# rostin79s/TFHE-AES

Measured on AMD Instinct MI355X. Metric: AES-128 CTR blocks/sec (FHE), higher is better.
Workload: dtype u64+f64; 1 GPU; configs[2]: 128 CTR blocks per GPU, Server::aes_encrypt 10 rounds (1280 bit-CBS/block), counters pre-incremented client-side; params=PARAM_OPT, blocks_per_gpu=128, total_blocks=128

## Files before the change

include/fheaes.h:

```cpp
#ifndef FHEAES_H
#define FHEAES_H

#include <stddef.h>
#include <stdint.h>

#ifdef __cplusplus
extern "C" {
#endif

#define FHEAES_OK 0
#define FHEAES_ERR_INVALID -1
#define FHEAES_ERR_NOKEYS -2
#define FHEAES_ERR_DEVICE -3
#define FHEAES_ERR_NOMEM -4

#define FHEAES_HOST 0
#define FHEAES_DEVICE 1

typedef struct fheaes_params {
    uint32_t lwe_dimension;
    uint32_t glwe_dimension;
    uint32_t polynomial_size;
    uint32_t pbs_base_log;
    uint32_t pbs_level;
// ... 77 lines not shown
int fheaes_aes_xts_decrypt_bits(fheaes_ctx *ctx, const uint64_t *dec_round_keys1, const uint64_t *round_keys2, uint32_t key_bits,
                                const uint64_t *tweaks_hi_lo, uint64_t n_units, uint64_t blocks_per_unit, uint64_t first_block,
                                const uint64_t *ct_hi_lo, uint64_t n_blocks, uint64_t *state_out, int memspace);
int fheaes_aes_xts_decrypt_packed(fheaes_ctx *ctx, const uint64_t *packed_dec_round_keys1, const uint64_t *packed_round_keys2, uint32_t key_bits,
                                  const uint64_t *tweaks_hi_lo, uint64_t n_units, uint64_t blocks_per_unit, uint64_t first_block,
                                  const uint64_t *ct_hi_lo, uint64_t n_blocks, uint64_t *state_out, int memspace);
int fheaes_xts_tweaks(fheaes_ctx *ctx, const uint64_t *anchor, uint64_t n_units, uint32_t first_offset, uint32_t n_offsets, uint64_t *out,
                      int memspace);
int fheaes_xts_tweak_row(uint32_t offset, uint32_t bit, uint32_t *sources_out , uint32_t *n_sources);
int fheaes_aes_xts_plan(uint64_t n_units, uint64_t blocks_per_unit, uint64_t first_block, uint64_t n_blocks, uint32_t key_bits,
                        uint64_t *segments, uint64_t *tweak_refresh_bytes, uint64_t *cipher_bytes, uint32_t *max_terms);

#define FHEAES_MAX_KEYS 65536
int fheaes_aes_key_expansion_batch(fheaes_ctx *ctx, const uint64_t *keys, uint32_t key_bits, uint64_t n_keys, uint64_t *round_keys, int memspace);
int fheaes_aes_decryption_round_keys_batch(fheaes_ctx *ctx, const uint64_t *round_keys, uint32_t key_bits, uint64_t n_keys,
                                           uint64_t *dec_round_keys, int memspace);
int fheaes_aes_encrypt_keyed(fheaes_ctx *ctx, const uint64_t *round_keys, uint32_t key_bits, uint64_t n_keys, const uint32_t *key_of_block,
                             uint64_t *state, uint64_t n_blocks, int memspace);
int fheaes_aes_decrypt_keyed(fheaes_ctx *ctx, const uint64_t *round_keys, uint32_t key_bits, uint64_t n_keys, const uint32_t *key_of_block,
                             uint64_t *state, uint64_t n_blocks, int memspace);
int fheaes_aes_decrypt_equivalent_keyed(fheaes_ctx *ctx, const uint64_t *dec_round_keys, uint32_t key_bits, uint64_t n_keys,
                                        const uint32_t *key_of_block, uint64_t *state, uint64_t n_blocks, int memspace);
int fheaes_aes_public_keyed(fheaes_ctx *ctx, const uint64_t *round_keys, uint32_t key_bits, uint64_t n_keys, const uint32_t *key_of_block,
                            const uint64_t *blocks_hi_lo, const uint64_t *data_hi_lo, uint64_t n_blocks, uint64_t *state_out, int memspace);
int fheaes_aes_public_plan_keyed(const uint64_t *blocks_hi_lo, const uint32_t *key_of_block, uint64_t n_blocks, uint64_t n_keys,
                                 uint32_t key_bits, uint64_t *unique_bytes_per_round);
int fheaes_aes_decrypt_public_keyed(fheaes_ctx *ctx, const uint64_t *dec_round_keys, uint32_t key_bits, uint64_t n_keys,
                                    const uint32_t *key_of_block, const uint64_t *blocks_hi_lo, const uint64_t *data_hi_lo, uint64_t n_blocks,
                                    uint64_t *state_out, int memspace);
int fheaes_aes_decrypt_public_plan_keyed(const uint64_t *blocks_hi_lo, const uint32_t *key_of_block, uint64_t n_blocks, uint64_t n_keys,
                                         uint32_t key_bits, uint64_t *unique_bytes_per_round);

size_t fheaes_packed_words(const fheaes_ctx *ctx, uint64_t m);
int fheaes_pack_bits(fheaes_ctx *ctx, const uint64_t *lwe_in, uint64_t m, uint64_t *glwe_out, int memspace);
int fheaes_unpack_bits(fheaes_ctx *ctx, const uint64_t *glwe_in, uint64_t m, uint64_t *lwe_out, int memspace);

int fheaes_expand_lwe_seeded(fheaes_ctx *ctx, const uint32_t *mask_key, uint64_t first_index, const uint64_t *bodies, uint64_t m,
                             uint64_t *lwe_out, int memspace);

size_t fheaes_packed_words_mod(const fheaes_ctx *ctx, uint64_t m, uint32_t width);
int fheaes_packed_mod_switch(fheaes_ctx *ctx, const uint64_t *glwe_in, uint64_t n_glwe, uint32_t width, uint64_t *out, int memspace);
int fheaes_pack_bits_mod(fheaes_ctx *ctx, const uint64_t *lwe_in, uint64_t m, uint32_t width, uint64_t *out, int memspace);
int fheaes_unpack_bits_mod(fheaes_ctx *ctx, const uint64_t *in, uint64_t m, uint32_t width, uint64_t *lwe_out, int memspace);

uint32_t fheaes_round_keys_packed_glwes(uint32_t key_bits);
int fheaes_pack_round_keys(fheaes_ctx *ctx, const uint64_t *round_keys, uint32_t key_bits, uint64_t n_keys, uint64_t *packed_out, int memspace);
int fheaes_unpack_round_keys(fheaes_ctx *ctx, const uint64_t *packed, uint32_t key_bits, uint64_t first_key, uint64_t n_keys,
                             uint64_t *round_keys_out, int memspace);
int fheaes_aes_encrypt_keyed_packed(fheaes_ctx *ctx, const uint64_t *packed_round_keys, uint32_t key_bits, uint64_t n_keys,
                                    const uint32_t *key_of_block, uint64_t *state, uint64_t n_blocks, int memspace);
int fheaes_aes_decrypt_keyed_packed(fheaes_ctx *ctx, const uint64_t *packed_round_keys, uint32_t key_bits, uint64_t n_keys,
                                    const uint32_t *key_of_block, uint64_t *state, uint64_t n_blocks, int memspace);
int fheaes_aes_decrypt_equivalent_keyed_packed(fheaes_ctx *ctx, const uint64_t *packed_dec_round_keys, uint32_t key_bits, uint64_t n_keys,
                                               const uint32_t *key_of_block, uint64_t *state, uint64_t n_blocks, int memspace);
int fheaes_aes_public_keyed_packed(fheaes_ctx *ctx, const uint64_t *packed_round_keys, uint32_t key_bits, uint64_t n_keys,
                                   const uint32_t *key_of_block, const uint64_t *blocks_hi_lo, const uint64_t *data_hi_lo, uint64_t n_blocks,
                                   uint64_t *state_out, int memspace);
int fheaes_aes_decrypt_public_keyed_packed(fheaes_ctx *ctx, const uint64_t *packed_dec_round_keys, uint32_t key_bits, uint64_t n_keys,
                                           const uint32_t *key_of_block, const uint64_t *blocks_hi_lo, const uint64_t *data_hi_lo,
                                           uint64_t n_blocks, uint64_t *state_out, int memspace);

#define FHEAES_MAC_MAX_STREAMS (1u << 20)
#define FHEAES_MAC_MAX_STREAM_BLOCKS (1u << 16)
#define FHEAES_MAC_NONE 0xFFFFFFFFu
int fheaes_aes_cbc_mac_keyed(fheaes_ctx *ctx, const uint64_t *round_keys, uint32_t key_bits, uint64_t n_keys, uint64_t n_streams,
                             const uint32_t *key_of_stream, const uint32_t *stream_blocks, const uint8_t *clear, const uint64_t *enc,
                             const uint8_t *enc_bytes, const uint64_t *init, uint64_t *mac_out, int memspace);
int fheaes_aes_cbc_mac_keyed_packed(fheaes_ctx *ctx, const uint64_t *packed_round_keys, uint32_t key_bits, uint64_t n_keys, uint64_t n_streams,
                                    const uint32_t *key_of_stream, const uint32_t *stream_blocks, const uint8_t *clear, const uint64_t *enc,
                                    const uint8_t *enc_bytes, const uint64_t *init, uint64_t *mac_out, int memspace);
int fheaes_aes_ccm_open_keyed(fheaes_ctx *ctx, const uint64_t *round_keys, uint32_t key_bits, uint64_t n_keys, uint64_t n_streams,
                              const uint32_t *key_of_stream, const uint32_t *head_blocks, const uint64_t *head_hi_lo, const uint64_t *ctr0_hi_lo,
                              const uint64_t *payload_bytes, const uint8_t *ciphertext, const uint8_t *tags, const uint32_t *tag_bytes,
                              uint64_t *plaintext_out, uint64_t *valid_out, int memspace);
int fheaes_aes_ccm_open_keyed_packed(fheaes_ctx *ctx, const uint64_t *packed_round_keys, uint32_t key_bits, uint64_t n_keys, uint64_t n_streams,
                                     const uint32_t *key_of_stream, const uint32_t *head_blocks, const uint64_t *head_hi_lo,
                                     const uint64_t *ctr0_hi_lo, const uint64_t *payload_bytes, const uint8_t *ciphertext, const uint8_t *tags,
                                     const uint32_t *tag_bytes, uint64_t *plaintext_out, uint64_t *valid_out, int memspace);
int fheaes_mac_link(fheaes_ctx *ctx, uint64_t *state, uint64_t n_slots, int first, const uint64_t *init, const uint64_t *enc, uint64_t n_enc,
                    const uint32_t *src_block, const uint8_t *enc_bytes, const uint8_t *clear, int memspace);
int fheaes_xts_whiten(fheaes_ctx *ctx, uint64_t *dst, const uint64_t *src, const uint64_t *tweaks, uint64_t n_tweaks, const uint32_t *tweak_of_block,
                      const uint8_t *clear, uint64_t n_blocks, int memspace);
int fheaes_aes_mac_plan(const uint32_t *stream_blocks, const uint32_t *payload_blocks, uint64_t n_streams, uint64_t *steps, uint64_t *n_active_out,
                        uint64_t n_active_cap, uint64_t *public_blocks, uint64_t *chained_blocks);

int fheaes_cmac_subkey_row(uint32_t which, uint32_t bit, uint32_t *sources_out, uint32_t *n_sources);
int fheaes_cmac_double(fheaes_ctx *ctx, const uint64_t *l, uint64_t n_keys, uint64_t *out, int memspace);
int fheaes_aes_cmac_subkeys_keyed(fheaes_ctx *ctx, const uint64_t *round_keys, uint32_t key_bits, uint64_t n_keys, uint64_t *subkeys_out,
                                  int memspace);
int fheaes_aes_cmac_subkeys_keyed_packed(fheaes_ctx *ctx, const uint64_t *packed_round_keys, uint32_t key_bits, uint64_t n_keys,
                                         uint64_t *subkeys_out, int memspace);
int fheaes_aes_cmac_keyed(fheaes_ctx *ctx, const uint64_t *round_keys, uint32_t key_bits, uint64_t n_keys, const uint64_t *subkeys,
                          uint64_t n_streams, const uint32_t *key_of_stream, const uint64_t *message_bytes, const uint8_t *data,
                          const uint8_t *tags, const uint32_t *tag_bytes, uint64_t *mac_out, uint64_t *valid_out, int memspace);
int fheaes_aes_cmac_keyed_packed(fheaes_ctx *ctx, const uint64_t *packed_round_keys, uint32_t key_bits, uint64_t n_keys, const uint64_t *subkeys,
                                 uint64_t n_streams, const uint32_t *key_of_stream, const uint64_t *message_bytes, const uint8_t *data,
                                 const uint8_t *tags, const uint32_t *tag_bytes, uint64_t *mac_out, uint64_t *valid_out, int memspace);
int fheaes_aes_cmac_plan(const uint64_t *message_bytes, uint64_t n_streams, uint64_t *steps, uint64_t *chained_blocks, uint64_t *padded_streams);

#define FHEAES_KW_MIN_SEMIBLOCKS 2
#define FHEAES_KW_MAX_SEMIBLOCKS 8
#define FHEAES_KW_MAX_KEYS 4096
int fheaes_aes_kw_unwrap_keyed(fheaes_ctx *ctx, const uint64_t *dec_round_keys, uint32_t key_bits, uint64_t n_keks, uint64_t n_keys,
                               const uint32_t *kek_of_key, uint32_t semiblocks, const uint8_t *wrapped, uint64_t *keys_out, uint64_t *valid_out,
                               int memspace);
int fheaes_aes_kw_unwrap_keyed_packed(fheaes_ctx *ctx, const uint64_t *packed_dec_round_keys, uint32_t key_bits, uint64_t n_keks, uint64_t n_keys,
                                      const uint32_t *kek_of_key, uint32_t semiblocks, const uint8_t *wrapped, uint64_t *keys_out,
                                      uint64_t *valid_out, int memspace);
int fheaes_kw_link(fheaes_ctx *ctx, uint64_t *state, uint64_t *regs, uint64_t n_keys, uint32_t semiblocks, uint32_t step, const uint8_t *wrapped,
                   int memspace);
int fheaes_aes_kw_plan(uint32_t key_bits, uint32_t semiblocks, uint64_t n_keys, uint64_t *steps, uint64_t *cipher_blocks, uint64_t *byte_wopbs);

#define FHEAES_GATE_LWE 0
#define FHEAES_GATE_GLWE 1
int fheaes_gate_ggsw(fheaes_ctx *ctx, const double *ggsw_fourier, uint64_t n_gates, const uint64_t *bits_of_gate, const uint64_t *in, uint64_t m,
                     int form, uint64_t *out, int memspace);
int fheaes_gate_bits(fheaes_ctx *ctx, const uint64_t *gates_lwe, uint64_t n_gates, const uint64_t *bits_of_gate, const uint64_t *lwe_in, uint64_t m,
                     uint64_t *lwe_out, int memspace);
int fheaes_gate_packed(fheaes_ctx *ctx, const uint64_t *gates_lwe, uint64_t n_gates, const uint64_t *glwes_of_gate, const uint64_t *glwe_in,
                       uint64_t n_glwe, uint64_t *glwe_out, int memspace);
int fheaes_gate_plan(const uint64_t *bits_of_gate, uint64_t n_gates, uint32_t k, uint64_t *workgroups, uint32_t *instances_per_workgroup);

#define FHEAES_AUDIT_MAX_ROWS 256
#define FHEAES_AUDIT_RECORDS 16
int fheaes_audit_set(fheaes_ctx *ctx, uint32_t rows, uint64_t min_bits, uint64_t seed);
int fheaes_audit_rows(uint64_t seed, uint64_t launch, uint64_t m, uint32_t rows, uint64_t *rows_out);
int fheaes_audit_read(fheaes_ctx *ctx, uint64_t *launches, uint64_t *rows_checked, uint64_t *rows_wrong, uint64_t *records_out, uint64_t record_cap,
                      uint64_t *record_n);
int fheaes_audit_debug(fheaes_ctx *ctx, uint64_t row, uint32_t word, uint64_t xor_mask);

#define FHEAES_STAGE_KEYSWITCH 0
#define FHEAES_STAGE_BLIND_ROTATE 1
#define FHEAES_STAGE_PFPKS 2
#define FHEAES_STAGE_GGSW_FFT 3
#define FHEAES_STAGE_VERTICAL_PACKING 4
#define FHEAES_STAGE_LINEAR 5
#define FHEAES_STAGE_COUNT 6
int fheaes_profile_enable(fheaes_ctx *ctx, int on);
int fheaes_profile_reset(fheaes_ctx *ctx);
int fheaes_profile_read(fheaes_ctx *ctx, int stage, double *total_ms, uint64_t *launches, uint64_t *units);

int fheaes_get_twiddles(double *psi_out);
int fheaes_read_bsk_fourier(fheaes_ctx *ctx, uint32_t i, double *out);
int fheaes_k2_launch_plan(uint64_t m, uint32_t cu_count, uint32_t k, int *form, uint64_t *units_main, uint32_t *r_main,
                          uint64_t *units_tail, uint32_t *r_tail);
int fheaes_k2_launch_plan_forms(uint64_t m, uint32_t cu_count, uint32_t k, int allow_pair, int *form, uint64_t *units_main, uint32_t *r_main,
                                uint64_t *units_tail, uint32_t *r_tail);
int fheaes_k2_context_plan(fheaes_ctx *ctx, uint64_t m, int *form, uint64_t *units_main, uint32_t *r_main, uint64_t *units_tail,
                           uint32_t *r_tail, char *kernel, size_t kernel_cap);
int fheaes_k2_set_parking(fheaes_ctx *ctx, int claimed);
int fheaes_k2_set_forms(fheaes_ctx *ctx, int allow_pair, int allow_home);
int fheaes_aes_window_plan(uint64_t n_blocks, uint32_t steps, uint32_t cu_count, uint32_t k, uint64_t *window_blocks, uint64_t *launches,
                           uint64_t *generations, uint64_t *generations_by_round);
int fheaes_aes_context_window(fheaes_ctx *ctx, uint64_t n_blocks, uint32_t steps, uint64_t *window_blocks);
#define FHEAES_AES_WINDOW_OFF 0xFFFFFFFFu
int fheaes_aes_set_window(fheaes_ctx *ctx, uint32_t window_blocks);
#define FHEAES_K2_PARK_SLOTS 1024
int fheaes_k2_park_debug(fheaes_ctx *ctx, const uint32_t *initial_owner, int record);
int fheaes_k2_park_read(fheaes_ctx *ctx, uint64_t *fallbacks, uint64_t *violations, uint32_t *owner_out, uint32_t *record_out,
                        uint64_t record_cap, uint64_t *record_n);
#define FHEAES_WS_BUFFERS 17
#define FHEAES_WS_F64 0
#define FHEAES_WS_WORDS 1
#define FHEAES_WS_TABLES 2
#define FHEAES_WS_PATTERN_F64_HALF 0x7FF87FF8u
#define FHEAES_WS_PATTERN_WORDS 0xA5
#define FHEAES_WS_PATTERN_TABLES 1u
#define FHEAES_WS_POISON_FILL 0
#define FHEAES_WS_POISON_RELEASE 1
int fheaes_workspace_info(fheaes_ctx *ctx, uint32_t index, char *name_out, size_t name_cap, uint64_t *bytes_out, int *class_out,
                          uint64_t *first_word_out, uint64_t *last_word_out);
int fheaes_workspace_poison(fheaes_ctx *ctx, int mode, uint64_t *bytes_out);
int fheaes_alloc_debug(fheaes_ctx *ctx, uint64_t fail_nth, uint64_t *seen_out);
const char *fheaes_version(void);

#ifdef __cplusplus
}
#endif
#endif
```

tfhe_aes_amd/_native.py:

```python
from __future__ import annotations

import ctypes
import os
import re
from pathlib import Path

import numpy as np

from . import _build
from .params import CParams, WopbsParameters

HOST, DEVICE = 0, 1
MAC_NONE = 0xFFFFFFFF
KW_MIN_SEMIBLOCKS, KW_MAX_SEMIBLOCKS, KW_MAX_KEYS = 2, 8, 4096
AES_WINDOW_OFF = 0xFFFFFFFF
GATE_LWE, GATE_GLWE = 0, 1
K2_PARK_SLOTS = 1024
AUDIT_MAX_ROWS, AUDIT_RECORDS = 256, 16
WS_BUFFERS = 17
WS_CLASSES = ("f64", "words", "tables")
WS_POISON_FILL, WS_POISON_RELEASE = 0, 1
STAGES = ("keyswitch", "blind_rotate", "pfpks", "ggsw_fft", "vertical_packing", "linear")

_u64p = ctypes.POINTER(ctypes.c_uint64)
_dp = ctypes.POINTER(ctypes.c_double)
_u32p = ctypes.POINTER(ctypes.c_uint32)
_u8p = ctypes.POINTER(ctypes.c_uint8)
_ctx = ctypes.c_void_p
_c = ctypes

SIGNATURES = {
    "fheaes_create": (_c.c_int, [_c.POINTER(CParams), _c.c_int, _c.POINTER(_ctx)]),
    "fheaes_destroy": (None, [_ctx]),
    "fheaes_last_error": (_c.c_char_p, [_ctx]),
    "fheaes_key_words": (_c.c_size_t, [_ctx, _c.c_int]),
    "fheaes_upload_keys": (_c.c_int, [_ctx, _c.c_void_p, _c.c_void_p, _c.c_void_p, _c.c_int]),
    "fheaes_key_body_words": (_c.c_size_t, [_ctx, _c.c_int]),
    "fheaes_upload_keys_seeded": (_c.c_int, [_ctx, _c.POINTER(_c.c_uint32), _c.c_void_p, _c.c_void_p, _c.c_void_p, _c.c_int]),
    "fheaes_clone_keys": (_c.c_int, [_ctx, _ctx]),
    "fheaes_clone_info": (_c.c_int, [_ctx, _c.POINTER(_c.c_int), _u64p, _dp]),
    "fheaes_noise_level_seen": (_c.c_int, [_ctx, _c.POINTER(_c.c_uint32), _c.POINTER(_c.c_uint32)]),
    "fheaes_set_stream": (_c.c_int, [_ctx, _c.c_void_p]),
    "fheaes_synchronize": (_c.c_int, [_ctx]),
    "fheaes_reserve": (_c.c_int, [_ctx, _c.c_uint64]),
    "fheaes_keyswitch_batch": (_c.c_int, [_ctx, _c.c_void_p, _c.c_uint64, _c.c_void_p, _c.c_int]),
    "fheaes_cbs_pbs_batch": (_c.c_int, [_ctx, _c.c_void_p, _c.c_uint64, _c.c_uint32, _c.c_void_p, _c.c_int]),
    "fheaes_pfpks_batch": (_c.c_int, [_ctx, _c.c_void_p, _c.c_uint64, _c.c_void_p, _c.c_int]),
    "fheaes_forward_fourier_batch": (_c.c_int, [_ctx, _c.c_void_p, _c.c_uint64, _c.c_void_p, _c.c_int]),
    "fheaes_vertical_packing_batch": (_c.c_int, [_ctx, _c.c_void_p, _c.c_uint64, _c.c_uint32, _c.c_void_p, _c.c_uint32,
                                                 _c.c_int, _c.c_void_p, _c.c_int]),
    "fheaes_inv_mix_columns_batch": (_c.c_int, [_ctx, _c.c_void_p, _c.c_uint64, _c.c_void_p, _c.c_int]),
    "fheaes_wopbs_batch": (_c.c_int, [_ctx, _c.c_void_p, _c.c_uint64, _c.c_uint32, _c.c_void_p, _c.c_uint32, _c.c_int,
                                      _c.c_void_p, _c.c_int]),
    "fheaes_gen_lut": (_c.c_int, [_c.c_uint32, _u64p, _u64p]),
    "fheaes_sbox": (_c.c_int, [_ctx, _c.c_void_p, _c.c_uint64, _c.c_int, _c.c_int]),
    "fheaes_many_sbox": (_c.c_int, [_ctx, _c.c_void_p, _c.c_uint64, _c.c_int, _c.c_void_p, _c.c_int]),
    "fheaes_aes_key_expansion": (_c.c_int, [_ctx, _c.c_void_p, _c.c_void_p, _c.c_int]),
    "fheaes_aes_encrypt": (_c.c_int, [_ctx, _c.c_void_p, _c.c_void_p, _c.c_uint64, _c.c_int]),
    "fheaes_aes_decrypt": (_c.c_int, [_ctx, _c.c_void_p, _c.c_void_p, _c.c_uint64, _c.c_int]),
    "fheaes_aes_decryption_round_keys": (_c.c_int, [_ctx, _c.c_void_p, _c.c_void_p, _c.c_int]),
    "fheaes_aes_decrypt_equivalent": (_c.c_int, [_ctx, _c.c_void_p, _c.c_void_p, _c.c_uint64, _c.c_int]),
    "fheaes_aes_key_expansion_bits": (_c.c_int, [_ctx, _c.c_void_p, _c.c_uint32, _c.c_void_p, _c.c_int]),
    "fheaes_aes_encrypt_bits": (_c.c_int, [_ctx, _c.c_void_p, _c.c_uint32, _c.c_void_p, _c.c_uint64, _c.c_int]),
    "fheaes_aes_decrypt_bits": (_c.c_int, [_ctx, _c.c_void_p, _c.c_uint32, _c.c_void_p, _c.c_uint64, _c.c_int]),
    "fheaes_aes_decryption_round_keys_bits": (_c.c_int, [_ctx, _c.c_void_p, _c.c_uint32, _c.c_void_p, _c.c_int]),
    "fheaes_aes_decrypt_equivalent_bits": (_c.c_int, [_ctx, _c.c_void_p, _c.c_uint32, _c.c_void_p, _c.c_uint64, _c.c_int]),
    "fheaes_add_scalar": (_c.c_int, [_ctx, _c.c_void_p, _c.c_uint64, _u64p, _c.c_int]),
    "fheaes_aes_encrypt_public_bits": (_c.c_int, [_ctx, _c.c_void_p, _c.c_uint32, _u64p, _c.c_uint64, _c.c_void_p, _c.c_int]),
    "fheaes_aes_ctr_bits": (_c.c_int, [_ctx, _c.c_void_p, _c.c_uint32, _u64p, _c.c_uint64, _u64p, _c.c_uint64, _c.c_void_p, _c.c_int]),
    "fheaes_aes_public_plan": (_c.c_int, [_u64p, _c.c_uint64, _c.c_uint32, _u64p]),
    "fheaes_aes_ctr32_bits": (_c.c_int, [_ctx, _c.c_void_p, _c.c_uint32, _u64p, _c.c_uint64, _u64p, _c.c_uint64, _c.c_void_p, _c.c_int]),
    "fheaes_aes_decrypt_public_bits": (_c.c_int, [_ctx, _c.c_void_p, _c.c_uint32, _u64p, _u64p, _c.c_uint64, _c.c_void_p, _c.c_int]),
    "fheaes_aes_cbc_decrypt_bits": (_c.c_int, [_ctx, _c.c_void_p, _c.c_uint32, _u64p, _u64p, _c.c_uint64, _c.c_void_p, _c.c_int]),
    "fheaes_aes_xts_decrypt_bits": (_c.c_int, [_ctx, _c.c_void_p, _c.c_void_p, _c.c_uint32, _u64p, _c.c_uint64, _c.c_uint64, _c.c_uint64, _u64p, _c.c_uint64,
                                               _c.c_void_p, _c.c_int]),
    "fheaes_aes_xts_decrypt_packed": (_c.c_int, [_ctx, _c.c_void_p, _c.c_void_p, _c.c_uint32, _u64p, _c.c_uint64, _c.c_uint64, _c.c_uint64, _u64p, _c.c_uint64,
                                                 _c.c_void_p, _c.c_int]),
    "fheaes_xts_tweaks": (_c.c_int, [_ctx, _c.c_void_p, _c.c_uint64, _c.c_uint32, _c.c_uint32, _c.c_void_p, _c.c_int]),
    "fheaes_xts_tweak_row": (_c.c_int, [_c.c_uint32, _c.c_uint32, _u32p, _u32p]),
    "fheaes_aes_xts_plan": (_c.c_int, [_c.c_uint64, _c.c_uint64, _c.c_uint64, _c.c_uint64, _c.c_uint32, _u64p, _u64p, _u64p, _u32p]),
    "fheaes_aes_key_expansion_batch": (_c.c_int, [_ctx, _c.c_void_p, _c.c_uint32, _c.c_uint64, _c.c_void_p, _c.c_int]),
    "fheaes_aes_decryption_round_keys_batch": (_c.c_int, [_ctx, _c.c_void_p, _c.c_uint32, _c.c_uint64, _c.c_void_p, _c.c_int]),
    "fheaes_aes_encrypt_keyed": (_c.c_int, [_ctx, _c.c_void_p, _c.c_uint32, _c.c_uint64, _u32p, _c.c_void_p, _c.c_uint64, _c.c_int]),
    "fheaes_aes_decrypt_keyed": (_c.c_int, [_ctx, _c.c_void_p, _c.c_uint32, _c.c_uint64, _u32p, _c.c_void_p, _c.c_uint64, _c.c_int]),
    "fheaes_aes_decrypt_equivalent_keyed": (_c.c_int, [_ctx, _c.c_void_p, _c.c_uint32, _c.c_uint64, _u32p, _c.c_void_p, _c.c_uint64, _c.c_int]),
    "fheaes_aes_public_keyed": (_c.c_int, [_ctx, _c.c_void_p, _c.c_uint32, _c.c_uint64, _u32p, _u64p, _u64p, _c.c_uint64, _c.c_void_p, _c.c_int]),
    "fheaes_aes_public_plan_keyed": (_c.c_int, [_u64p, _u32p, _c.c_uint64, _c.c_uint64, _c.c_uint32, _u64p]),
    "fheaes_aes_decrypt_public_keyed": (_c.c_int, [_ctx, _c.c_void_p, _c.c_uint32, _c.c_uint64, _u32p, _u64p, _u64p, _c.c_uint64, _c.c_void_p, _c.c_int]),
    "fheaes_aes_decrypt_public_plan_keyed": (_c.c_int, [_u64p, _u32p, _c.c_uint64, _c.c_uint64, _c.c_uint32, _u64p]),
    "fheaes_packed_words": (_c.c_size_t, [_ctx, _c.c_uint64]),
    "fheaes_pack_bits": (_c.c_int, [_ctx, _c.c_void_p, _c.c_uint64, _c.c_void_p, _c.c_int]),
    "fheaes_unpack_bits": (_c.c_int, [_ctx, _c.c_void_p, _c.c_uint64, _c.c_void_p, _c.c_int]),
    "fheaes_expand_lwe_seeded": (_c.c_int, [_ctx, _u32p, _c.c_uint64, _c.c_void_p, _c.c_uint64, _c.c_void_p, _c.c_int]),
    "fheaes_packed_words_mod": (_c.c_size_t, [_ctx, _c.c_uint64, _c.c_uint32]),
    "fheaes_packed_mod_switch": (_c.c_int, [_ctx, _c.c_void_p, _c.c_uint64, _c.c_uint32, _c.c_void_p, _c.c_int]),
    "fheaes_pack_bits_mod": (_c.c_int, [_ctx, _c.c_void_p, _c.c_uint64, _c.c_uint32, _c.c_void_p, _c.c_int]),
    "fheaes_unpack_bits_mod": (_c.c_int, [_ctx, _c.c_void_p, _c.c_uint64, _c.c_uint32, _c.c_void_p, _c.c_int]),
    "fheaes_round_keys_packed_glwes": (_c.c_uint32, [_c.c_uint32]),
    "fheaes_pack_round_keys": (_c.c_int, [_ctx, _c.c_void_p, _c.c_uint32, _c.c_uint64, _c.c_void_p, _c.c_int]),
    "fheaes_unpack_round_keys": (_c.c_int, [_ctx, _c.c_void_p, _c.c_uint32, _c.c_uint64, _c.c_uint64, _c.c_void_p, _c.c_int]),
    "fheaes_aes_encrypt_keyed_packed": (_c.c_int, [_ctx, _c.c_void_p, _c.c_uint32, _c.c_uint64, _u32p, _c.c_void_p, _c.c_uint64, _c.c_int]),
    "fheaes_aes_decrypt_keyed_packed": (_c.c_int, [_ctx, _c.c_void_p, _c.c_uint32, _c.c_uint64, _u32p, _c.c_void_p, _c.c_uint64, _c.c_int]),
    "fheaes_aes_decrypt_equivalent_keyed_packed": (_c.c_int, [_ctx, _c.c_void_p, _c.c_uint32, _c.c_uint64, _u32p, _c.c_void_p, _c.c_uint64, _c.c_int]),
    "fheaes_aes_public_keyed_packed": (_c.c_int, [_ctx, _c.c_void_p, _c.c_uint32, _c.c_uint64, _u32p, _u64p, _u64p, _c.c_uint64, _c.c_void_p, _c.c_int]),
    "fheaes_aes_decrypt_public_keyed_packed": (_c.c_int, [_ctx, _c.c_void_p, _c.c_uint32, _c.c_uint64, _u32p, _u64p, _u64p, _c.c_uint64, _c.c_void_p,
                                                          _c.c_int]),
    "fheaes_aes_cbc_mac_keyed": (_c.c_int, [_ctx, _c.c_void_p, _c.c_uint32, _c.c_uint64, _c.c_uint64, _u32p, _u32p, _u8p, _c.c_void_p, _u8p, _c.c_void_p,
                                            _c.c_void_p, _c.c_int]),
    "fheaes_aes_cbc_mac_keyed_packed": (_c.c_int, [_ctx, _c.c_void_p, _c.c_uint32, _c.c_uint64, _c.c_uint64, _u32p, _u32p, _u8p, _c.c_void_p, _u8p,
                                                   _c.c_void_p, _c.c_void_p, _c.c_int]),
    "fheaes_aes_ccm_open_keyed": (_c.c_int, [_ctx, _c.c_void_p, _c.c_uint32, _c.c_uint64, _c.c_uint64, _u32p, _u32p, _u64p, _u64p, _u64p, _u8p, _u8p, _u32p,
                                             _c.c_void_p, _c.c_void_p, _c.c_int]),
    "fheaes_aes_ccm_open_keyed_packed": (_c.c_int, [_ctx, _c.c_void_p, _c.c_uint32, _c.c_uint64, _c.c_uint64, _u32p, _u32p, _u64p, _u64p, _u64p, _u8p, _u8p,
                                                    _u32p, _c.c_void_p, _c.c_void_p, _c.c_int]),
    "fheaes_mac_link": (_c.c_int, [_ctx, _c.c_void_p, _c.c_uint64, _c.c_int, _c.c_void_p, _c.c_void_p, _c.c_uint64, _u32p, _u8p, _u8p, _c.c_int]),
    "fheaes_xts_whiten": (_c.c_int, [_ctx, _c.c_void_p, _c.c_void_p, _c.c_void_p, _c.c_uint64, _u32p, _u8p, _c.c_uint64, _c.c_int]),
    "fheaes_aes_mac_plan": (_c.c_int, [_u32p, _u32p, _c.c_uint64, _u64p, _u64p, _c.c_uint64, _u64p, _u64p]),
    "fheaes_cmac_subkey_row": (_c.c_int, [_c.c_uint32, _c.c_uint32, _u32p, _u32p]),
    "fheaes_cmac_double": (_c.c_int, [_ctx, _c.c_void_p, _c.c_uint64, _c.c_void_p, _c.c_int]),
    "fheaes_aes_cmac_subkeys_keyed": (_c.c_int, [_ctx, _c.c_void_p, _c.c_uint32, _c.c_uint64, _c.c_void_p, _c.c_int]),
    "fheaes_aes_cmac_subkeys_keyed_packed": (_c.c_int, [_ctx, _c.c_void_p, _c.c_uint32, _c.c_uint64, _c.c_void_p, _c.c_int]),
    "fheaes_aes_cmac_keyed": (_c.c_int, [_ctx, _c.c_void_p, _c.c_uint32, _c.c_uint64, _c.c_void_p, _c.c_uint64, _u32p, _u64p, _u8p, _u8p, _u32p, _c.c_void_p,
                                         _c.c_void_p, _c.c_int]),
    "fheaes_aes_cmac_keyed_packed": (_c.c_int, [_ctx, _c.c_void_p, _c.c_uint32, _c.c_uint64, _c.c_void_p, _c.c_uint64, _u32p, _u64p, _u8p, _u8p, _u32p,
                                                _c.c_void_p, _c.c_void_p, _c.c_int]),
    "fheaes_aes_cmac_plan": (_c.c_int, [_u64p, _c.c_uint64, _u64p, _u64p, _u64p]),
    "fheaes_aes_kw_unwrap_keyed": (_c.c_int, [_ctx, _c.c_void_p, _c.c_uint32, _c.c_uint64, _c.c_uint64, _u32p, _c.c_uint32, _u8p, _c.c_void_p, _c.c_void_p,
                                              _c.c_int]),
    "fheaes_aes_kw_unwrap_keyed_packed": (_c.c_int, [_ctx, _c.c_void_p, _c.c_uint32, _c.c_uint64, _c.c_uint64, _u32p, _c.c_uint32, _u8p, _c.c_void_p,
                                                     _c.c_void_p, _c.c_int]),
    "fheaes_kw_link": (_c.c_int, [_ctx, _c.c_void_p, _c.c_void_p, _c.c_uint64, _c.c_uint32, _c.c_uint32, _u8p, _c.c_int]),
    "fheaes_aes_kw_plan": (_c.c_int, [_c.c_uint32, _c.c_uint32, _c.c_uint64, _u64p, _u64p, _u64p]),
    "fheaes_gate_ggsw": (_c.c_int, [_ctx, _c.c_void_p, _c.c_uint64, _u64p, _c.c_void_p, _c.c_uint64, _c.c_int, _c.c_void_p, _c.c_int]),
    "fheaes_gate_bits": (_c.c_int, [_ctx, _c.c_void_p, _c.c_uint64, _u64p, _c.c_void_p, _c.c_uint64, _c.c_void_p, _c.c_int]),
    "fheaes_gate_packed": (_c.c_int, [_ctx, _c.c_void_p, _c.c_uint64, _u64p, _c.c_void_p, _c.c_uint64, _c.c_void_p, _c.c_int]),
    "fheaes_gate_plan": (_c.c_int, [_u64p, _c.c_uint64, _c.c_uint32, _u64p, _u32p]),
    "fheaes_profile_enable": (_c.c_int, [_ctx, _c.c_int]),
    "fheaes_profile_reset": (_c.c_int, [_ctx]),
    "fheaes_profile_read": (_c.c_int, [_ctx, _c.c_int, _dp, _u64p, _u64p]),
    "fheaes_get_twiddles": (_c.c_int, [_dp]),
    "fheaes_read_bsk_fourier": (_c.c_int, [_ctx, _c.c_uint32, _dp]),
    "fheaes_k2_launch_plan": (_c.c_int, [_c.c_uint64, _c.c_uint32, _c.c_uint32, _c.POINTER(_c.c_int), _c.POINTER(_c.c_uint64), _c.POINTER(_c.c_uint32),
                                       _c.POINTER(_c.c_uint64), _c.POINTER(_c.c_uint32)]),
    "fheaes_k2_launch_plan_forms": (_c.c_int, [_c.c_uint64, _c.c_uint32, _c.c_uint32, _c.c_int, _c.POINTER(_c.c_int), _c.POINTER(_c.c_uint64),
                                             _c.POINTER(_c.c_uint32), _c.POINTER(_c.c_uint64), _c.POINTER(_c.c_uint32)]),
    "fheaes_k2_context_plan": (_c.c_int, [_ctx, _c.c_uint64, _c.POINTER(_c.c_int), _c.POINTER(_c.c_uint64), _c.POINTER(_c.c_uint32),
                                        _c.POINTER(_c.c_uint64), _c.POINTER(_c.c_uint32), _c.c_char_p, _c.c_size_t]),
    "fheaes_k2_set_parking": (_c.c_int, [_ctx, _c.c_int]),
    "fheaes_k2_set_forms": (_c.c_int, [_ctx, _c.c_int, _c.c_int]),
    "fheaes_aes_window_plan": (_c.c_int, [_c.c_uint64, _c.c_uint32, _c.c_uint32, _c.c_uint32, _u64p, _u64p, _u64p, _u64p]),
    "fheaes_aes_context_window": (_c.c_int, [_ctx, _c.c_uint64, _c.c_uint32, _u64p]),
    "fheaes_aes_set_window": (_c.c_int, [_ctx, _c.c_uint32]),
    "fheaes_k2_park_debug": (_c.c_int, [_ctx, _c.POINTER(_c.c_uint32), _c.c_int]),
    "fheaes_k2_park_read": (_c.c_int, [_ctx, _u64p, _u64p, _c.POINTER(_c.c_uint32), _c.POINTER(_c.c_uint32), _c.c_uint64, _u64p]),
    "fheaes_audit_set": (_c.c_int, [_ctx, _c.c_uint32, _c.c_uint64, _c.c_uint64]),
    "fheaes_audit_rows": (_c.c_int, [_c.c_uint64, _c.c_uint64, _c.c_uint64, _c.c_uint32, _u64p]),
    "fheaes_audit_read": (_c.c_int, [_ctx, _u64p, _u64p, _u64p, _u64p, _c.c_uint64, _u64p]),
    "fheaes_audit_debug": (_c.c_int, [_ctx, _c.c_uint64, _c.c_uint32, _c.c_uint64]),
    "fheaes_workspace_info": (_c.c_int, [_ctx, _c.c_uint32, _c.c_char_p, _c.c_size_t, _u64p, _c.POINTER(_c.c_int), _u64p, _u64p]),
    "fheaes_workspace_poison": (_c.c_int, [_ctx, _c.c_int, _u64p]),
    "fheaes_alloc_debug": (_c.c_int, [_ctx, _c.c_uint64, _u64p]),
    "fheaes_version": (_c.c_char_p, []),
}

_libs = {}


def header_symbols() -> list[str]:
    text = (_build.ROOT / "include" / "fheaes.h").read_text()
    text = re.sub(r"/\*.*?\*/", "", text, flags=re.S)
    return sorted(set(re.findall(r"\b(fheaes_[a-z0-9_]+)\s*\(", text)))


def load_library(build: bool = True, path=None, partial: bool = False):
    if path is None:
        path = _build.build_engine() if build else _build.ENGINE_SO
    path = Path(path).resolve()
    if path in _libs:
        return _libs[path]
    try:
        import torch
    except ImportError:
        pass
    if not path.exists():
        raise RuntimeError("%s is missing: run __graft_entry__.build() (hipcc --offload-arch=gfx950)" % path.name)
    lib = ctypes.CDLL(str(path))
    for name, (res, args) in SIGNATURES.items():
        if partial and not hasattr(lib, name):
            continue
        fn = getattr(lib, name)
        fn.restype, fn.argtypes = res, args
    _libs[path] = lib
    return lib


class FheAesError(RuntimeError):
    def __init__(self, code: int, message: str):
        super().__init__("fheaes error %d: %s" % (code, message))
        self.code = code


def _ptr(x):
    if x is None:
        return None, None
    if isinstance(x, np.ndarray):
        assert x.flags["C_CONTIGUOUS"], "array must be C-contiguous"
        return x.ctypes.data, HOST
    if hasattr(x, "data_ptr"):
        assert x.is_contiguous()
        return x.data_ptr(), (DEVICE if x.is_cuda else HOST)
    raise TypeError("expected numpy array or torch tensor, got %r" % type(x))


class Engine:

    def __init__(self, params: WopbsParameters, device: int = 0, allow_dev_build: bool = False, library=None):
        self.params = params
        self._lib = load_library() if library is None else load_library(path=library, partial=True)
        self._h = _ctx()
        version = (self._lib.fheaes_version() or b"").decode()
        if version.endswith(" dev") and not (allow_dev_build or os.environ.get("FHEAES_ALLOW_DEV_BUILD") == "1"):
            raise RuntimeError("libfheaes.so is a developer build (%r): rebuild it with tfhe_aes_amd._build.build_engine(force=True), or pass "
                               "allow_dev_build=True / FHEAES_ALLOW_DEV_BUILD=1 if that is what you mean to run" % version)
        cp = params.c_struct()
        rc = self._lib.fheaes_create(ctypes.byref(cp), device, ctypes.byref(self._h))
        if rc != 0:
            raise FheAesError(rc, (self._lib.fheaes_last_error(None) or b"").decode())

    def close(self):
        if getattr(self, "_h", None):
            self._lib.fheaes_destroy(self._h)
            self._h = None

    def __del__(self):
        try:
            self.close()
        except Exception:
            pass

    def _check(self, rc: int):
        if rc != 0:
            raise FheAesError(rc, (self._lib.fheaes_last_error(self._h) or b"").decode())

    def _space(self, *arrays):
        spaces = {s for _, s in map(_ptr, arrays) if s is not None}
        if len(spaces) != 1:
            raise ValueError("all arrays of one call must live in the same memory space")
        return spaces.pop()

    def key_words(self, which: int) -> int:
        return self._lib.fheaes_key_words(self._h, which)

    def upload_keys(self, ksk, bsk, pfpksk):
        sp = self._space(ksk, bsk, pfpksk)
        for which, a in enumerate((ksk, bsk, pfpksk)):
            n = a.size if isinstance(a, np.ndarray) else a.numel()
            if n != self.key_words(which):
                raise ValueError("key %d has %d words, expected %d" % (which, n, self.key_words(which)))
        self._check(self._lib.fheaes_upload_keys(self._h, _ptr(ksk)[0], _ptr(bsk)[0], _ptr(pfpksk)[0], sp))

    def upload_keys_seeded(self, mask_key, ksk_body, bsk_body, pfpksk_body):
        mk = np.ascontiguousarray(np.asarray(mask_key, dtype=np.uint32).reshape(8))
        sp = self._space(ksk_body, bsk_body, pfpksk_body)
        for which, a in enumerate((ksk_body, bsk_body, pfpksk_body)):
            n = a.size if isinstance(a, np.ndarray) else a.numel()
            if n != self._lib.fheaes_key_body_words(self._h, which):
                raise ValueError("key body %d has %d words, expected %d" % (which, n, self._lib.fheaes_key_body_words(self._h, which)))
        self._check(self._lib.fheaes_upload_keys_seeded(self._h, mk.ctypes.data_as(_c.POINTER(_c.c_uint32)), _ptr(ksk_body)[0], _ptr(bsk_body)[0],
                                                        _ptr(pfpksk_body)[0], sp))

    def clone_keys_from(self, other: "Engine"):
        self._check(self._lib.fheaes_clone_keys(self._h, other._h))

    def clone_info(self) -> dict:
        path, nbytes, secs = ctypes.c_int(), ctypes.c_uint64(), ctypes.c_double()
        self._check(self._lib.fheaes_clone_info(self._h, ctypes.byref(path), ctypes.byref(nbytes), ctypes.byref(secs)))
        return {"path": ("none", "same_device", "peer", "staged")[path.value], "bytes": nbytes.value, "seconds": secs.value}

    def noise_level_seen(self) -> tuple[int, int]:
        seen, limit = ctypes.c_uint32(), ctypes.c_uint32()
        self._check(self._lib.fheaes_noise_level_seen(self._h, ctypes.byref(seen), ctypes.byref(limit)))
        return seen.value, limit.value

    def set_stream(self, stream_handle: int | None):
        self._check(self._lib.fheaes_set_stream(self._h, stream_handle))

    def synchronize(self):
        self._check(self._lib.fheaes_synchronize(self._h))

    def reserve(self, max_bits: int):
        self._check(self._lib.fheaes_reserve(self._h, max_bits))

    def keyswitch_batch(self, lwe_in, lwe_out, m: int):
        self._check(self._lib.fheaes_keyswitch_batch(self._h, _ptr(lwe_in)[0], m, _ptr(lwe_out)[0], self._space(lwe_in, lwe_out)))

    def cbs_pbs_batch(self, lwe_small, lwe_out, m: int, level: int = 1):
        self._check(self._lib.fheaes_cbs_pbs_batch(self._h, _ptr(lwe_small)[0], m, level, _ptr(lwe_out)[0], self._space(lwe_small, lwe_out)))

    def pfpks_batch(self, lwe_in, ggsw_out, m: int):
        self._check(self._lib.fheaes_pfpks_batch(self._h, _ptr(lwe_in)[0], m, _ptr(ggsw_out)[0], self._space(lwe_in, ggsw_out)))

    def forward_fourier_batch(self, polys_in, fourier_out, polys: int):
        self._check(self._lib.fheaes_forward_fourier_batch(self._h, _ptr(polys_in)[0], polys, _ptr(fourier_out)[0], self._space(polys_in, fourier_out)))
# ... 382 lines not shown
    out = np.zeros((len(values), 2), dtype=np.uint64)
    for i, v in enumerate(values):
        if isinstance(v, (bytes, bytearray)):
            if len(v) != 16:
                raise ValueError("an AES block has 16 bytes, got %d" % len(v))
            v = int.from_bytes(v, "big")
        v = int(v)
        if not 0 <= v < 1 << 128:
            raise ValueError("a block is a 128-bit value")
        out[i, 0], out[i, 1] = v >> 64, v & (2 ** 64 - 1)
    return out


def key_indices(key_of_block, n_blocks: int) -> np.ndarray:
    idx = [int(k) for k in key_of_block]
    if len(idx) != n_blocks:
        raise ValueError("one key index per block expected: %d for %d blocks" % (len(idx), n_blocks))
    if any(not 0 <= k < 1 << 32 for k in idx):
        raise ValueError("a key index is a uint32")
    out = np.zeros(max(n_blocks, 1), dtype=np.uint32)
    out[:n_blocks] = idx
    return out


def wrapped_bytes(wrapped, semiblocks: int) -> np.ndarray:
    size = 8 * (semiblocks + 1)
    if not isinstance(wrapped, np.ndarray):
        wrapped = [bytes(w) for w in wrapped]
        if any(len(w) != size for w in wrapped):
            raise ValueError("a wrapped key of %d semiblocks has %d bytes" % (semiblocks, size))
        wrapped = np.frombuffer(b"".join(wrapped), dtype=np.uint8)
    return np.ascontiguousarray(np.asarray(wrapped, dtype=np.uint8).reshape(-1, size))


def aes_public_plan_keyed(blocks, key_of_block, n_keys: int, key_bits: int = 128) -> list[int]:
    cnt = u128_pairs(blocks)
    kob = key_indices(key_of_block, len(cnt))
    out = np.zeros(14, dtype=np.uint64)
    rc = load_library().fheaes_aes_public_plan_keyed(cnt.ctypes.data_as(_u64p), kob.ctypes.data_as(_u32p), len(cnt), n_keys, key_bits, out.ctypes.data_as(_u64p))
    if rc != 0:
        raise FheAesError(rc, "fheaes_aes_public_plan_keyed: key_bits must be 128, 192 or 256, n_keys in 1..65536 and every key index below n_keys")
    return [int(x) for x in out[:{128: 10, 192: 12, 256: 14}[key_bits]]]


def aes_decrypt_public_plan_keyed(blocks, key_of_block, n_keys: int, key_bits: int = 128) -> list[int]:
    cnt = u128_pairs(blocks)
    kob = key_indices(key_of_block, len(cnt)) if key_of_block is not None else None
    out = np.zeros(14, dtype=np.uint64)
    rc = load_library().fheaes_aes_decrypt_public_plan_keyed(cnt.ctypes.data_as(_u64p), kob.ctypes.data_as(_u32p) if kob is not None else None, len(cnt),
                                                             n_keys, key_bits, out.ctypes.data_as(_u64p))
    if rc != 0:
        raise FheAesError(rc, "fheaes_aes_decrypt_public_plan_keyed: key_bits must be 128, 192 or 256, n_keys in 1..65536 and every key index below n_keys")
    return [int(x) for x in out[:{128: 10, 192: 12, 256: 14}[key_bits]]]


def aes_decrypt_public_plan(blocks, key_bits: int = 128) -> list[int]:
    return aes_decrypt_public_plan_keyed(blocks, None, 1, key_bits)


def xts_tweak_row(offset: int, bit: int) -> list[int]:
    src, n = (_c.c_uint32 * 4)(), _c.c_uint32()
    rc = load_library().fheaes_xts_tweak_row(offset, bit, src, _c.byref(n))
    if rc != 0:
        raise FheAesError(rc, "fheaes_xts_tweak_row: offset must be at most 121 and bit below 128")
    return [int(x) for x in src[:n.value]]


def aes_xts_plan(n_units: int, blocks_per_unit: int, first_block: int, n_blocks: int, key_bits: int = 128) -> dict:
    seg, ref, cip, terms = _c.c_uint64(), _c.c_uint64(), _c.c_uint64(), _c.c_uint32()
    rc = load_library().fheaes_aes_xts_plan(n_units, blocks_per_unit, first_block, n_blocks, key_bits, _c.byref(seg), _c.byref(ref), _c.byref(cip), _c.byref(terms))
    if rc != 0:
        raise FheAesError(rc, "fheaes_aes_xts_plan: key_bits must be 128 or 256, blocks_per_unit in 1..2^20, and n_units cover the blocks")
    return {"segments": seg.value, "tweak_refresh_bytes": ref.value, "cipher_bytes": cip.value, "max_terms": terms.value}


def aes_mac_plan(stream_blocks, payload_blocks=None) -> dict:
    sb = np.ascontiguousarray(np.asarray(stream_blocks, dtype=np.uint32).reshape(-1))
    pb = None if payload_blocks is None else np.ascontiguousarray(np.asarray(payload_blocks, dtype=np.uint32).reshape(-1))
    if pb is not None and len(pb) != len(sb):
        raise ValueError("one payload block count per stream expected")
    cap = int(sb.max()) if len(sb) else 0
    act = np.zeros(max(cap, 1), dtype=np.uint64)
    steps, pub, chained = _c.c_uint64(), _c.c_uint64(), _c.c_uint64()
    rc = load_library().fheaes_aes_mac_plan(sb.ctypes.data_as(_u32p), pb.ctypes.data_as(_u32p) if pb is not None else None, len(sb), _c.byref(steps),
                                            act.ctypes.data_as(_u64p), len(act), _c.byref(pub), _c.byref(chained))
    if rc != 0:
        raise FheAesError(rc, "fheaes_aes_mac_plan: at most 2^20 streams of at most 2^16 blocks, payload blocks within them")
    return {"steps": steps.value, "n_active": [int(x) for x in act[:steps.value]], "chained_blocks": chained.value, "public_blocks": pub.value}


def cmac_subkey_row(which: int, bit: int) -> list[int]:
    src, n = (_c.c_uint32 * 3)(), _c.c_uint32()
    rc = load_library().fheaes_cmac_subkey_row(which, bit, src, _c.byref(n))
    if rc != 0:
        raise FheAesError(rc, "fheaes_cmac_subkey_row: which must be 0 or 1 and bit below 128")
    return [int(x) for x in src[:n.value]]


def aes_cmac_plan(message_bytes) -> dict:
    mb = np.ascontiguousarray(np.asarray(message_bytes, dtype=np.uint64).reshape(-1))
    steps, chained, padded = _c.c_uint64(), _c.c_uint64(), _c.c_uint64()
    rc = load_library().fheaes_aes_cmac_plan(mb.ctypes.data_as(_u64p), len(mb), _c.byref(steps), _c.byref(chained), _c.byref(padded))
    if rc != 0:
        raise FheAesError(rc, "fheaes_aes_cmac_plan: at most 2^20 streams of at most 16 * 2^16 bytes")
    return {"steps": steps.value, "chained_blocks": chained.value, "padded_streams": padded.value}


def aes_kw_plan(key_bits: int, semiblocks: int, n_keys: int) -> dict:
    steps, blocks, wopbs = _c.c_uint64(), _c.c_uint64(), _c.c_uint64()
    rc = load_library().fheaes_aes_kw_plan(key_bits, semiblocks, n_keys, _c.byref(steps), _c.byref(blocks), _c.byref(wopbs))
    if rc != 0:
        raise FheAesError(rc, "fheaes_aes_kw_plan: key_bits 128 / 192 / 256, %d..%d semiblocks, at most %d keys" % (KW_MIN_SEMIBLOCKS, KW_MAX_SEMIBLOCKS, KW_MAX_KEYS))
    return {"steps": steps.value, "cipher_blocks": blocks.value, "byte_wopbs": wopbs.value}


def gate_plan(runs, k: int) -> dict:
    r = np.ascontiguousarray(np.asarray(runs, dtype=np.uint64).reshape(-1))
    wgs, per = _c.c_uint64(), _c.c_uint32()
    rc = load_library().fheaes_gate_plan(r.ctypes.data_as(_u64p), r.size, k, _c.byref(wgs), _c.byref(per))
    if rc != 0:
        raise FheAesError(rc, "fheaes_gate_plan: k must be 4 or 1")
    return {"workgroups": wgs.value, "instances_per_workgroup": per.value}


def audit_rows(seed: int, launch: int, m: int, rows: int) -> list[int]:
    out = np.zeros(max(min(int(rows), int(m)), 1), dtype=np.uint64)
    rc = load_library().fheaes_audit_rows(int(seed) & (2 ** 64 - 1), int(launch), int(m), int(rows), out.ctypes.data_as(_u64p))
    if rc != 0:
        raise FheAesError(rc, "fheaes_audit_rows: m at least 1 and rows in 1..%d" % AUDIT_MAX_ROWS)
    return [int(x) for x in out]


def round_keys_packed_glwes(key_bits: int) -> int:
    return int(load_library().fheaes_round_keys_packed_glwes(int(key_bits)))


def aes_public_plan(blocks, key_bits: int = 128) -> list[int]:
    cnt = u128_pairs(blocks)
    out = np.zeros(14, dtype=np.uint64)
    rc = load_library().fheaes_aes_public_plan(cnt.ctypes.data_as(_u64p), len(cnt), key_bits, out.ctypes.data_as(_u64p))
    if rc != 0:
        raise FheAesError(rc, "fheaes_aes_public_plan: key_bits must be 128, 192 or 256")
    return [int(x) for x in out[:{128: 10, 192: 12, 256: 14}[key_bits]]]


def aes_window_plan(n_blocks: int, steps: int, cu_count: int = 256, k: int = 4) -> dict:
    w, la, g, gr = _c.c_uint64(), _c.c_uint64(), _c.c_uint64(), _c.c_uint64()
    rc = load_library().fheaes_aes_window_plan(n_blocks, steps, cu_count, k, _c.byref(w), _c.byref(la), _c.byref(g), _c.byref(gr))
    if rc != 0:
        raise FheAesError(rc, "fheaes_aes_window_plan: n_blocks, steps and cu_count must be at least 1")
    return {"window": w.value, "launches": la.value, "generations": g.value, "generations_by_round": gr.value}


def get_twiddles() -> np.ndarray:
    out = np.empty((512, 2), dtype=np.float64)
    rc = load_library().fheaes_get_twiddles(out.ctypes.data_as(_dp))
    if rc != 0:
        raise FheAesError(rc, "fheaes_get_twiddles")
    return out


def gen_lut(nb_block: int, f_table) -> np.ndarray:
    f = np.ascontiguousarray(f_table, dtype=np.uint64)
    if f.size != 1 << nb_block:
        raise ValueError("f_table must have 2^nb_block entries")
    out = np.empty((nb_block, max(512, 1 << nb_block)), dtype=np.uint64)
    rc = load_library().fheaes_gen_lut(nb_block, f.ctypes.data_as(_u64p), out.ctypes.data_as(_u64p))
    if rc != 0:
        raise FheAesError(rc, "fheaes_gen_lut")
    return out
```

tfhe_aes_amd/csrc/aes_schedule.h:

```cpp
#pragma once

static int many_sbox_dev(fheaes_ctx *c, const uint64_t *bytes, uint64_t n_bytes, int set, uint64_t *out)
{
    return wopbs_dev(c, bytes, n_bytes, 8, c->lutset_d[set], (uint32_t)c->lutset_n[set], 0, out);
}

static int aes_rounds(uint32_t key_bits) { return key_bits == 128 ? 10 : key_bits == 192 ? 12 : key_bits == 256 ? 14 : 0; }

static int check_key_bits(fheaes_ctx *c, uint32_t key_bits)
{
    if (!aes_rounds(key_bits)) return c->fail(FHEAES_ERR_INVALID, "key_bits must be 128, 192 or 256, got %u", key_bits);
    return FHEAES_OK;
}

struct AesStep { int set; uint32_t n_luts; GatherTable table; int key_round; };
struct AesSchedule {
    int first_key_round = 0;
    uint32_t max_luts = 0;
    std::vector<AesStep> steps;
    void add(int set, uint32_t n_luts, const GatherTable &t, int key_round) { steps.push_back({set, n_luts, t, key_round}); max_luts = std::max(max_luts, n_luts); }
};

static AesSchedule aes_encrypt_schedule(int nr)
{
    AesSchedule s;
    s.first_key_round = 0;
    for (int round = 1; round < nr; ++round) s.add(LUTSET_ENC_ROUND, 3, table_enc_round(), round);
    s.add(LUTSET_SBOX, 1, table_shift_rows(false), nr);
    return s;
}

static AesSchedule aes_decrypt_schedule(int nr)
{
    AesSchedule s;
    s.first_key_round = nr;
    for (int round = nr; round >= 2; --round) {
        s.add(LUTSET_INV_SBOX, 1, table_shift_rows(true), round - 1);
        s.add(LUTSET_DEC_MUL, 4, table_dec_mix(), -1);
    }
    s.add(LUTSET_INV_SBOX, 1, table_shift_rows(true), 0);
    return s;
}

static AesSchedule aes_decrypt_eq_schedule(int nr)
{
    AesSchedule s;
    s.first_key_round = nr;
    for (int round = nr - 1; round >= 1; --round) s.add(LUTSET_DEC_EQ_ROUND, 4, table_dec_eq_round(), round);
    s.add(LUTSET_INV_SBOX, 1, table_shift_rows(true), 0);
    return s;
}

static int aes_run_dev(fheaes_ctx *c, const KeySets &rk, uint64_t *state, uint64_t n_blocks, const AesSchedule &sch)
{
    const uint64_t bw = 8ull * c->big1, sw = 16 * bw, steps = sch.steps.size();
    auto key_of = [&](const AesStep &st, uint64_t first_block) {
        if (st.key_round < 0) return KeySets{nullptr, nullptr, 0};
        return rk.round((uint64_t)st.key_round, sw, first_block);
    };
    const uint64_t w = aes_context_window(c, n_blocks, steps);
    TRY(ensure(c, c->ws_vp, (w ? w : n_blocks) * 16 * sch.max_luts * bw * 8));
    uint64_t *vp = (uint64_t *)c->ws_vp.p;
    TRY(launch_add_bcast(c, state, rk.round((uint64_t)sch.first_key_round, sw), sw, n_blocks));
    if (w == 0) {
        for (const AesStep &st : sch.steps) {
            TRY(many_sbox_dev(c, state, 16 * n_blocks, st.set, vp));
            TRY(launch_gather(c, vp, st.n_luts, key_of(st, 0), state, n_blocks, st.table));
        }
        return FHEAES_OK;
    }
    const uint64_t ggsw_words = (uint64_t)c->k1 * c->k1 * FHE_N, total = steps * n_blocks;
    TRY(ensure_wopbs_ws(c, w * AES_BLOCK_BITS));
    uint64_t *small = (uint64_t *)c->ws_small.p;
    const double2 *ggswf = (const double2 *)c->ws_ggswf.p;
    struct Segment { const AesStep *st; uint64_t first, blocks, row; uint64_t *vp; };
    for (uint64_t i0 = 0; i0 < total; i0 += w) {
        const uint64_t len = std::min<uint64_t>(w, total - i0), s = i0 / n_blocks, b0 = i0 % n_blocks, m = len * AES_BLOCK_BITS;
        Segment seg[2] = {{&sch.steps[s], b0, std::min<uint64_t>(len, n_blocks - b0), 0, vp}, {}};
        int n_seg = 1;
        if (seg[0].blocks < len) {
            seg[1] = {&sch.steps[s + 1], 0, len - seg[0].blocks, seg[0].blocks, vp + seg[0].blocks * 16 * seg[0].st->n_luts * bw};
            n_seg = 2;
        }
        for (int g = 0; g < n_seg; ++g)
            TRY(launch_keyswitch(c, state + seg[g].first * sw, seg[g].blocks * AES_BLOCK_BITS, small + seg[g].row * AES_BLOCK_BITS * (c->n + 1)));
        TRY(cbs_from_small(c, m));
        if (n_seg == 1 || seg[0].st->set == seg[1].st->set) {
            const int set = seg[0].st->set;
            TRY(launch_vertical_packing(c, ggswf, 16 * len, 8, c->lutset_d[set], (uint32_t)c->lutset_n[set], 0, vp));
        } else {
            for (int g = 0; g < n_seg; ++g) {
                const int set = seg[g].st->set;
                TRY(launch_vertical_packing(c, ggswf + seg[g].row * AES_BLOCK_BITS * (ggsw_words / 2), 16 * seg[g].blocks, 8, c->lutset_d[set],
                                            (uint32_t)c->lutset_n[set], 0, seg[g].vp));
            }
        }
        for (int g = 0; g < n_seg; ++g)
            TRY(launch_gather(c, seg[g].vp, seg[g].st->n_luts, key_of(*seg[g].st, seg[g].first), state + seg[g].first * sw, seg[g].blocks, seg[g].st->table));
    }
    return FHEAES_OK;
}

static int aes_encrypt_dev(fheaes_ctx *c, const KeySets &rk, uint64_t *state, uint64_t n_blocks, int nr) { return aes_run_dev(c, rk, state, n_blocks, aes_encrypt_schedule(nr)); }
static int aes_decrypt_dev(fheaes_ctx *c, const KeySets &rk, uint64_t *state, uint64_t n_blocks, int nr) { return aes_run_dev(c, rk, state, n_blocks, aes_decrypt_schedule(nr)); }
static int aes_decrypt_eq_dev(fheaes_ctx *c, const KeySets &dw, uint64_t *state, uint64_t n_blocks, int nr) { return aes_run_dev(c, dw, state, n_blocks, aes_decrypt_eq_schedule(nr)); }

typedef int (*AesDevFn)(fheaes_ctx *, const KeySets &, uint64_t *, uint64_t, int);

static int dec_round_keys_dev(fheaes_ctx *c, const uint64_t *w, uint64_t *dw, int nr, uint64_t n_keys)
{
    const uint64_t bw = 8ull * c->big1, sw = 16 * bw, ks = (uint64_t)(nr + 1) * sw, mid = (uint64_t)(nr - 1) * 16, nbytes = mid * n_keys;
    const bool strided = n_keys > 1;
    TRY(ensure(c, c->ws_vp, nbytes * 4 * bw * 8));
    TRY(ensure(c, c->ws_tmp_a, nbytes * bw * 8));
    if (strided) TRY(ensure(c, c->ws_tmp_b, nbytes * bw * 8));
    uint64_t *vp = (uint64_t *)c->ws_vp.p, *mix = (uint64_t *)c->ws_tmp_a.p, *flat = (uint64_t *)c->ws_tmp_b.p;
    TRY(launch_key_rows(c, dw, ks, w, ks, 0, nullptr, 0, 0, 16, n_keys, 1));
    TRY(launch_key_rows(c, dw + (uint64_t)nr * sw, ks, w + (uint64_t)nr * sw, ks, 0, nullptr, 0, 0, 16, n_keys, 1));
    if (strided) TRY(launch_key_rows(c, flat, mid * bw, w + sw, ks, 0, nullptr, 0, 0, (uint32_t)mid, n_keys, 1));
    TRY(many_sbox_dev(c, strided ? flat : w + sw, nbytes, LUTSET_DEC_MUL, vp));
    TRY(launch_gather(c, vp, 4, KeySets{nullptr, nullptr, 0}, mix, nbytes / 16, table_dec_mix()));
    TRY(many_sbox_dev(c, mix, nbytes, LUTSET_IDENTITY, strided ? flat : dw + sw));
    if (strided) TRY(launch_key_rows(c, dw + sw, ks, flat, mid * bw, 0, nullptr, 0, 0, (uint32_t)mid, n_keys, 1));
    return FHEAES_OK;
}

static int key_expansion_dev(fheaes_ctx *c, const uint64_t *key, uint64_t *w, int nr, uint64_t n_keys)
{
    static const uint8_t RCON[10] = {0x01, 0x02, 0x04, 0x08, 0x10, 0x20, 0x40, 0x80, 0x1B, 0x36};
    const uint64_t bw = 8ull * c->big1, ww = 4 * bw, ks = (uint64_t)(nr + 1) * 16 * bw;
    const int nk = nr - 6;
    const bool strided = n_keys > 1;
    TRY(ensure(c, c->ws_tmp_a, n_keys * ww * 8));
    TRY(ensure(c, c->ws_tmp_b, n_keys * ww * 8));
    if (strided) TRY(ensure(c, c->ws_tmp_c, n_keys * ww * 8));
    uint64_t *ta = (uint64_t *)c->ws_tmp_a.p, *tb = (uint64_t *)c->ws_tmp_b.p, *tc = (uint64_t *)c->ws_tmp_c.p;
    TRY(launch_key_rows(c, w, ks, key, (uint64_t)nk * ww, 0, nullptr, 0, 0, 4u * nk, n_keys, 1));
    for (int i = nk; i < 4 * (nr + 1); ++i) {
        const uint64_t *prev = w + (uint64_t)(i - 1) * ww, *back = w + (uint64_t)(i - nk) * ww;
        if (i % nk == 0) {
            TRY(launch_key_rows(c, ta, ww, prev, ks, 1, nullptr, 0, 0, 4, n_keys, 1));
            TRY(many_sbox_dev(c, ta, 4 * n_keys, LUTSET_SBOX, tb));
            TRY(launch_key_rows(c, ta, ww, tb, ww, 0, back, ks, RCON[i / nk - 1], 4, n_keys, 2));
        } else if (nk > 6 && i % nk == 4) {
            if (strided) TRY(launch_key_rows(c, ta, ww, prev, ks, 0, nullptr, 0, 0, 4, n_keys, 1));
            TRY(many_sbox_dev(c, strided ? ta : prev, 4 * n_keys, LUTSET_SBOX, tb));
            TRY(launch_key_rows(c, ta, ww, tb, ww, 0, back, ks, 0, 4, n_keys, 2));
        } else {
            TRY(launch_key_rows(c, ta, ww, prev, ks, 0, back, ks, 0, 4, n_keys, 2));
        }
        uint64_t *fresh = w + (uint64_t)i * ww;
        TRY(many_sbox_dev(c, ta, 4 * n_keys, LUTSET_IDENTITY, strided ? tc : fresh));
        if (strided) TRY(launch_key_rows(c, fresh, ks, tc, ww, 0, nullptr, 0, 0, 4, n_keys, 1));
    }
    return FHEAES_OK;
}

template <class Fill> static int upload_pinned(fheaes_ctx *c, size_t bytes, size_t ws_bytes, Fill fill)
{
    if (c->pin_ev) HIP_TRY(c, hipEventSynchronize(c->pin_ev));
    else HIP_TRY(c, hipEventCreateWithFlags(&c->pin_ev, hipEventDisableTiming));
    if (c->pin_bytes < bytes) {
        if (c->pin) { HIP_TRY(c, hipHostFree(c->pin)); c->pin = nullptr; c->pin_bytes = 0; }
        HIP_TRY(c, hipHostMalloc((void **)&c->pin, bytes, hipHostMallocDefault));
        c->pin_bytes = bytes;
    }
    fill(c->pin);
    TRY(ensure(c, c->ws_misc, ws_bytes));
    HIP_TRY(c, hipMemcpyAsync(c->ws_misc.p, c->pin, bytes, hipMemcpyHostToDevice, c->stream));
    HIP_TRY(c, hipEventRecord(c->pin_ev, c->stream));
    return FHEAES_OK;
}

static int add_scalar_dev(fheaes_ctx *c, uint64_t *state, uint64_t n_blocks, const uint64_t *counters)
{
    const uint32_t lw = c->big1;
    TRY(upload_pinned(c, 16 * n_blocks, 16 * n_blocks + n_blocks * lw * 8 + 64, [&](uint8_t *add) {
        for (uint64_t b = 0; b < n_blocks; ++b) {
            uint64_t hi = counters[2 * b], lo = counters[2 * b + 1];
            for (int j = 0; j < 8; ++j) { add[(15 - j) * n_blocks + b] = (uint8_t)(lo >> (8 * j)); add[(7 - j) * n_blocks + b] = (uint8_t)(hi >> (8 * j)); }
        }
    }));
    uint8_t *add_d = (uint8_t *)c->ws_misc.p;
    uint64_t *carry = (uint64_t *)((uint8_t *)c->ws_misc.p + ((16 * n_blocks + 63) / 64) * 64);
    TRY(ensure(c, c->ws_tmp_a, n_blocks * 9ull * lw * 8));
    TRY(ensure(c, c->ws_tmp_b, n_blocks * 2ull * 9 * lw * 8));
    TRY(ensure(c, c->ws_luts, n_blocks * 2ull * 9 * FHE_N * 8));
    uint64_t *in9 = (uint64_t *)c->ws_tmp_a.p, *res = (uint64_t *)c->ws_tmp_b.p, *luts = (uint64_t *)c->ws_luts.p;
    for (int byte = 15; byte >= 0; --byte) {
        const uint32_t bits = byte == 15 ? 8 : 9;
        dim3 g1((bits * lw + 255) / 256, (unsigned)n_blocks);
        hipLaunchKernelGGL(pack9_kernel, g1, dim3(256), 0, c->stream, (const uint64_t *)state, (const uint64_t *)carry, in9, (uint32_t)byte, lw, n_blocks, bits);
        hipLaunchKernelGGL(counter_lut_kernel, dim3((2 * bits * FHE_N + 255) / 256, (unsigned)n_blocks), dim3(256), 0, c->stream, luts,
                           (const uint8_t *)(add_d + (size_t)byte * n_blocks), bits, n_blocks);
        HIP_TRY(c, hipGetLastError());
        TRY(wopbs_dev(c, in9, n_blocks, bits, luts, 2, 1, res));
        hipLaunchKernelGGL(unpack_sum_carry_kernel, dim3((9 * lw + 255) / 256, (unsigned)n_blocks), dim3(256), 0, c->stream, (const uint64_t *)res, bits, state, carry,
                           (uint32_t)byte, lw, n_blocks);
        HIP_TRY(c, hipGetLastError());
    }
    return FHEAES_OK;
}

struct PublicPlan {
    struct Layer { size_t head, term; uint32_t n, terms; };
    std::vector<Layer> layers;
    std::vector<uint32_t> words;
    uint64_t max_vp_bytes_per_bw = 0;
};

static inline uint32_t u128_byte(const uint64_t *hi_lo, int p) { return (uint32_t)((p < 8 ? hi_lo[0] >> (8 * (7 - p)) : hi_lo[1] >> (8 * (15 - p))) & 0xFF); }

struct PublicKey5 {
    uint32_t v[5];
    bool operator==(const PublicKey5 &o) const { return !memcmp(v, o.v, sizeof v); }
};
struct PublicKey5Hash {
    size_t operator()(const PublicKey5 &k) const
    {
        uint64_t h = 0xCBF29CE484222325ull;
        for (uint32_t x : k.v) { h ^= x; h *= 0x100000001B3ull; }
        return (size_t)(h ^ (h >> 29));
    }
};

struct PublicDirection {
    GatherTable round, last;
    int round_set, last_set;
    uint32_t round_luts, last_luts;
    bool keys_descend;
    uint64_t key_round(int layer, int nr) const { return (uint64_t)(keys_descend ? nr - layer : layer); }
};

static PublicDirection public_forward() { return {table_enc_round(), table_shift_rows(false), LUTSET_ENC_ROUND, LUTSET_SBOX, 3, 1, false}; }
static PublicDirection public_inverse() { return {table_dec_eq_round(), table_shift_rows(true), LUTSET_DEC_EQ_ROUND, LUTSET_INV_SBOX, 4, 1, true}; }

static void public_plan(const PublicDirection &dir, const uint64_t *blocks, const uint64_t *data, const uint32_t *key_of_block, uint64_t n_blocks, int nr,
                        PublicPlan &pl)
{
    auto key_of = [&](uint64_t b) { return key_of_block ? key_of_block[b] : 0u; };
    const GatherTable &t_round = dir.round, &t_shift = dir.last;
    const uint64_t nbytes = 16 * n_blocks;
    std::vector<uint32_t> id(nbytes), next(nbytes);
    pl.layers.clear(); pl.words.clear();
    pl.layers.reserve((size_t)nr + 1);
    {
        std::unordered_map<uint32_t, uint32_t> seen;
// ... 362 lines not shown
```

tfhe_aes_amd/csrc/engine.hip:

```cpp
#include <hip/hip_runtime.h>
#include <algorithm>
#include <cmath>
#include <cstdarg>
#include <cstdio>
#include <atomic>
#include <chrono>
#include <cstring>
#include <functional>
#include <mutex>
#include <string>
#include <type_traits>
#include <unordered_map>
#include <vector>

#include "knobs.h"
#include "fheaes.h"
#include "fft_dev.h"
#include "kern_extprod.h"
#include "kern_gate.h"
#include "kern_blindrot_latency.h"
#include "kern_blindrot16.h"
#include "kern_blindrot_pair.h"
#include "kern_audit.h"
#include "ks_launch.h"
#include "kern_linear.h"

#define FHEAES_VERSION_STR "fheaes-mi355x 0.4 (gfx950)" FHEAES_BUILD_KIND

#include "host_tables.h"
#include "engine_ctx.h"
#include "engine_launch.h"
#include "aes_schedule.h"

namespace {

int supported(const fheaes_params *p, std::string &why)
{
    char buf[256];
    if (p->polynomial_size != FHE_N) { why = "polynomial_size must be 512"; return 0; }
    if (p->glwe_dimension != 4 && p->glwe_dimension != 1) { why = "glwe_dimension must be 4 (PARAM_OPT) or 1 (toy)"; return 0; }
    if (p->pbs_base_log != 8 || p->pbs_level != 5 || p->ks_base_log != 2 || p->ks_level != 6 || p->pfks_base_log != 12 ||
        p->pfks_level != 3 || p->cbs_base_log != 15 || p->cbs_level != 1) {
        snprintf(buf, sizeof buf, "unsupported gadget: kernels are instantiated for pbs(8,5) ks(2,6) pfks(12,3) cbs(15,1)");
        why = buf;
        return 0;
    }
    if (p->lwe_dimension < 1 || p->lwe_dimension > 4096) { why = "lwe_dimension out of range"; return 0; }
    return 1;
}

}

extern "C" {

int fheaes_k2_launch_plan(uint64_t m, uint32_t cu_count, uint32_t k, int *form, uint64_t *units_main, uint32_t *r_main,
                          uint64_t *units_tail, uint32_t *r_tail)
{
    if (!form || !units_main || !r_main || !units_tail || !r_tail || cu_count == 0 || m == 0) return FHEAES_ERR_INVALID;
    const K2Plan pl = k2_plan(m, cu_count, k + 1);
    *form = pl.form; *units_main = pl.units_main; *r_main = pl.r_main; *units_tail = pl.units_tail; *r_tail = pl.r_tail;
    return FHEAES_OK;
}
int fheaes_k2_launch_plan_forms(uint64_t m, uint32_t cu_count, uint32_t k, int allow_pair, int *form, uint64_t *units_main, uint32_t *r_main,
                                uint64_t *units_tail, uint32_t *r_tail)
{
    if (!form || !units_main || !r_main || !units_tail || !r_tail || cu_count == 0 || m == 0 || (allow_pair != 0 && allow_pair != 1)) return FHEAES_ERR_INVALID;
    const K2Plan pl = k2_plan(m, cu_count, k + 1, allow_pair == 1);
    *form = pl.form; *units_main = pl.units_main; *r_main = pl.r_main; *units_tail = pl.units_tail; *r_tail = pl.r_tail;
    return FHEAES_OK;
}
int fheaes_k2_context_plan(fheaes_ctx *ctx, uint64_t m, int *form, uint64_t *units_main, uint32_t *r_main, uint64_t *units_tail,
                           uint32_t *r_tail, char *kernel, size_t kernel_cap)
{
    if (!ctx) return FHEAES_ERR_INVALID;
    CtxLock lock__(ctx);
    if (!form || !units_main || !r_main || !units_tail || !r_tail || m == 0) return ctx->fail(FHEAES_ERR_INVALID, "k2_context_plan: null output or empty batch");
    const K2Launch L = k2_launch(ctx, m);
    const K2Plan &pl = L.pl;
    *form = pl.form; *units_main = pl.units_main; *r_main = pl.r_main; *units_tail = pl.units_tail; *r_tail = pl.r_tail;
    if (kernel && kernel_cap) { std::strncpy(kernel, L.name, kernel_cap - 1); kernel[kernel_cap - 1] = 0; }
    return FHEAES_OK;
}
int fheaes_k2_set_parking(fheaes_ctx *ctx, int claimed)
{
    if (!ctx) return FHEAES_ERR_INVALID;
    CtxLock lock__(ctx);
    if (claimed != 0 && claimed != 1) return ctx->fail(FHEAES_ERR_INVALID, "k2_set_parking: 1 = claimed slots, 0 = one private slot per workgroup (got %d)", claimed);
    HIP_TRY(ctx, hipStreamSynchronize(ctx->stream));
    ctx->k2_park_claim = claimed;
    return FHEAES_OK;
}
int fheaes_k2_set_forms(fheaes_ctx *ctx, int allow_pair, int allow_home)
{
    if (!ctx) return FHEAES_ERR_INVALID;
    CtxLock lock__(ctx);
    if ((allow_pair != 0 && allow_pair != 1) || (allow_home != 0 && allow_home != 1))
        return ctx->fail(FHEAES_ERR_INVALID, "k2_set_forms: each of allow_pair, allow_home is 0 or 1 (got %d, %d)", allow_pair, allow_home);
    HIP_TRY(ctx, hipStreamSynchronize(ctx->stream));
    ctx->k2_deny_pair = allow_pair == 0;
    ctx->k2_deny_home = allow_home == 0;
    return FHEAES_OK;
}
int fheaes_aes_window_plan(uint64_t n_blocks, uint32_t steps, uint32_t cu_count, uint32_t k, uint64_t *window_blocks, uint64_t *launches,
                           uint64_t *generations, uint64_t *generations_by_round)
{
    if (!window_blocks || !launches || !generations || !generations_by_round || n_blocks == 0 || steps == 0 || cu_count == 0) return FHEAES_ERR_INVALID;
    const AesWindowPlan pl = aes_window_plan(n_blocks, steps, cu_count, k + 1);
    *window_blocks = pl.window; *launches = pl.launches; *generations = pl.generations; *generations_by_round = pl.generations_by_round;
    return FHEAES_OK;
}
int fheaes_aes_context_window(fheaes_ctx *ctx, uint64_t n_blocks, uint32_t steps, uint64_t *window_blocks)
{
    if (!ctx) return FHEAES_ERR_INVALID;
    CtxLock lock__(ctx);
    if (!window_blocks) return ctx->fail(FHEAES_ERR_INVALID, "aes_context_window: null output");
    *window_blocks = aes_context_window(ctx, n_blocks, steps);
    return FHEAES_OK;
}
int fheaes_aes_set_window(fheaes_ctx *ctx, uint32_t window_blocks)
{
    if (!ctx) return FHEAES_ERR_INVALID;
    CtxLock lock__(ctx);
    HIP_TRY(ctx, hipStreamSynchronize(ctx->stream));
    ctx->aes_window = window_blocks;
    return FHEAES_OK;
}
int fheaes_k2_park_debug(fheaes_ctx *ctx, const uint32_t *initial_owner, int record)
{
    if (!ctx) return FHEAES_ERR_INVALID;
    CtxLock lock__(ctx);
    if (record != 0 && record != 1) return ctx->fail(FHEAES_ERR_INVALID, "k2_park_debug: record must be 0 or 1 (got %d)", record);
    HIP_TRY(ctx, hipSetDevice(ctx->device));
    HIP_TRY(ctx, hipStreamSynchronize(ctx->stream));
    if (initial_owner) {
        TRY(ensure(ctx, ctx->ws_park_pattern, BRP_PARK_SLOTS * sizeof(uint32_t)));
        HIP_TRY(ctx, hipMemcpy(ctx->ws_park_pattern.p, initial_owner, BRP_PARK_SLOTS * sizeof(uint32_t), hipMemcpyHostToDevice));
    }
    if (ctx->ws_park_owner.p)
        HIP_TRY(ctx, hipMemset((char *)ctx->ws_park_owner.p + PARK_RECORD_PTR_OFFSET, 0, sizeof(uint64_t)));
    ctx->k2_park_pattern = initial_owner != nullptr;
    ctx->k2_park_record = record == 1;
    ctx->k2_park_record_n = 0;
    return FHEAES_OK;
}
int fheaes_k2_park_read(fheaes_ctx *ctx, uint64_t *fallbacks, uint64_t *violations, uint32_t *owner_out, uint32_t *record_out,
                        uint64_t record_cap, uint64_t *record_n)
{
    if (!ctx) return FHEAES_ERR_INVALID;
    CtxLock lock__(ctx);
    if (record_out && record_cap < ctx->k2_park_record_n)
        return ctx->fail(FHEAES_ERR_INVALID, "k2_park_read: %llu records do not fit record_cap = %llu", (unsigned long long)ctx->k2_park_record_n,
                         (unsigned long long)record_cap);
    HIP_TRY(ctx, hipSetDevice(ctx->device));
    HIP_TRY(ctx, hipStreamSynchronize(ctx->stream));
    uint32_t words[PARK_OWNER_BYTES / sizeof(uint32_t)] = {};
    if (ctx->ws_park_owner.p) HIP_TRY(ctx, hipMemcpy(words, ctx->ws_park_owner.p, PARK_OWNER_BYTES, hipMemcpyDeviceToHost));
    uint64_t counters[2];
    std::memcpy(counters, words + BRP_PARK_SLOTS, sizeof counters);
    if (fallbacks) *fallbacks = counters[0];
    if (violations) *violations = counters[1];
    if (owner_out) std::memcpy(owner_out, words, BRP_PARK_SLOTS * sizeof(uint32_t));
    if (record_out && ctx->k2_park_record_n)
        HIP_TRY(ctx, hipMemcpy(record_out, ctx->ws_park_record.p, ctx->k2_park_record_n * 2 * sizeof(uint32_t), hipMemcpyDeviceToHost));
    if (record_n) *record_n = ctx->k2_park_record_n;
    return FHEAES_OK;
}
int fheaes_audit_set(fheaes_ctx *ctx, uint32_t rows, uint64_t min_bits, uint64_t seed)
{
    if (!ctx) return FHEAES_ERR_INVALID;
    CtxLock lock__(ctx);
    if (rows > AUDIT_MAX_ROWS) return ctx->fail(FHEAES_ERR_INVALID, "audit_set: at most %d rows per launch (got %u)", AUDIT_MAX_ROWS, rows);
    HIP_TRY(ctx, hipSetDevice(ctx->device));
    HIP_TRY(ctx, hipStreamSynchronize(ctx->stream));
    ctx->audit_rows = 0;
    ctx->audit_hook = false;
    ctx->audit_launch = 0;
    if (rows == 0) {
        for (DevBuf *b : {&ctx->audit_in, &ctx->audit_out, &ctx->audit_state})
            if (b->p) { HIP_TRY(ctx, hipFree(b->p)); b->p = nullptr; b->bytes = 0; }
        return FHEAES_OK;
    }
    TRY(ensure(ctx, ctx->audit_in, (size_t)AUDIT_MAX_ROWS * (ctx->n + 1) * 8));
    TRY(ensure(ctx, ctx->audit_out, (size_t)AUDIT_MAX_ROWS * ctx->big1 * 8));
    TRY(ensure(ctx, ctx->audit_state, AUDIT_STATE_WORDS * 8));
    HIP_TRY(ctx, hipMemset(ctx->audit_state.p, 0, AUDIT_STATE_WORDS * 8));
    ctx->audit_min_bits = min_bits;
    ctx->audit_seed = seed;
    ctx->audit_rows = rows;
    return FHEAES_OK;
}
int fheaes_audit_rows(uint64_t seed, uint64_t launch, uint64_t m, uint32_t rows, uint64_t *rows_out)
{
    if (!rows_out || m == 0 || rows == 0 || rows > AUDIT_MAX_ROWS) return FHEAES_ERR_INVALID;
    const uint32_t S = (uint32_t)std::min<uint64_t>(rows, m);
    for (uint32_t s = 0; s < S; ++s) rows_out[s] = audit_row(seed, launch, m, S, s);
    return FHEAES_OK;
}
int fheaes_audit_read(fheaes_ctx *ctx, uint64_t *launches, uint64_t *rows_checked, uint64_t *rows_wrong, uint64_t *records_out, uint64_t record_cap,
                      uint64_t *record_n)
{
    if (!ctx) return FHEAES_ERR_INVALID;
    CtxLock lock__(ctx);
    HIP_TRY(ctx, hipSetDevice(ctx->device));
    HIP_TRY(ctx, hipStreamSynchronize(ctx->stream));
    uint64_t st[AUDIT_STATE_WORDS] = {};
    if (ctx->audit_state.p) HIP_TRY(ctx, hipMemcpy(st, ctx->audit_state.p, sizeof st, hipMemcpyDeviceToHost));
    const uint64_t n = std::min<uint64_t>(st[AUDIT_ST_WRONG], AUDIT_RECORDS);
    if (records_out && record_cap < n)
        return ctx->fail(FHEAES_ERR_INVALID, "audit_read: %llu records do not fit record_cap = %llu", (unsigned long long)n, (unsigned long long)record_cap);
    if (launches) *launches = st[AUDIT_ST_LAUNCHES];
    if (rows_checked) *rows_checked = st[AUDIT_ST_CHECKED];
    if (rows_wrong) *rows_wrong = st[AUDIT_ST_WRONG];
    if (records_out && n) std::memcpy(records_out, st + AUDIT_ST_RECORDS, n * AUDIT_RECORD_WORDS * 8);
    if (record_n) *record_n = n;
    return FHEAES_OK;
}
int fheaes_audit_debug(fheaes_ctx *ctx, uint64_t row, uint32_t word, uint64_t xor_mask)
{
    if (!ctx) return FHEAES_ERR_INVALID;
    CtxLock lock__(ctx);
    if (xor_mask == 0 || word >= ctx->big1)
        return ctx->fail(FHEAES_ERR_INVALID, "audit_debug: a non-zero mask and a word in 0..%u (got mask %#llx, word %u)", ctx->big, (unsigned long long)xor_mask, word);
    ctx->audit_hook = true;
    ctx->audit_hook_row = row; ctx->audit_hook_word = word; ctx->audit_hook_mask = xor_mask;
    return FHEAES_OK;
}
const char *fheaes_version(void) { return FHEAES_VERSION_STR; }

const char *fheaes_last_error(const fheaes_ctx *ctx)
{
    if (!ctx) return g_create_error.c_str();
    if (tl_error_ctx_id != ctx->id) {
        CtxLock lock__(ctx);
        tl_error = ctx->err;
        tl_error_ctx_id = ctx->id;
    }
    return tl_error.c_str();
}

int fheaes_get_twiddles(double *psi_out)
{
    if (!psi_out) return FHEAES_ERR_INVALID;
    const HostTwiddles &t = twiddles();
    for (int j = 0; j < FHE_N; ++j) { psi_out[2 * j] = t.psi_re[j]; psi_out[2 * j + 1] = t.psi_im[j]; }
    return FHEAES_OK;
}

int fheaes_gen_lut(uint32_t nb_block, const uint64_t *f_table, uint64_t *lut_out)
{
    if (nb_block < 1 || nb_block > MAX_WOPBS_BITS || !f_table || !lut_out) return FHEAES_ERR_INVALID;
    gen_lut_host(nb_block, f_table, lut_out);
    return FHEAES_OK;
}

int fheaes_create(const fheaes_params *params, int device, fheaes_ctx **out)
{
    if (!params || !out) { g_create_error = "null argument"; return FHEAES_ERR_INVALID; }
    std::string why;
    if (!supported(params, why)) { g_create_error = why; return FHEAES_ERR_INVALID; }
    int ndev = 0;
    hipError_t e = hipGetDeviceCount(&ndev);
// ... 1345 lines not shown
                                 uint64_t *mac_out, uint64_t *valid_out, int memspace)
{
    return aes_cmac(c, {packed_round_keys, key_bits, n_keys, key_of_stream, n_streams, true}, subkeys, message_bytes, data, tags, tag_bytes, mac_out, valid_out, memspace);
}

int fheaes_aes_cmac_plan(const uint64_t *message_bytes, uint64_t n_streams, uint64_t *steps, uint64_t *chained_blocks, uint64_t *padded_streams)
{
    if ((n_streams && !message_bytes) || !steps || !chained_blocks || !padded_streams || n_streams > MAC_MAX_STREAMS) return FHEAES_ERR_INVALID;
    std::vector<uint32_t> len(n_streams);
    uint64_t padded = 0;
    for (uint64_t s = 0; s < n_streams; ++s) {
        if (message_bytes[s] > 16ull * MAC_MAX_STREAM_BLOCKS) return FHEAES_ERR_INVALID;
        len[s] = (uint32_t)cmac_blocks(message_bytes[s]);
        padded += message_bytes[s] == 0 || message_bytes[s] % 16 != 0;
    }
    MacPlan pl;
    mac_plan(len.data(), n_streams, pl);
    *steps = pl.n_active.size(); *chained_blocks = pl.chained; *padded_streams = padded;
    return FHEAES_OK;
}

static_assert(KW_MIN_SEMIBLOCKS == FHEAES_KW_MIN_SEMIBLOCKS && KW_MAX_SEMIBLOCKS == FHEAES_KW_MAX_SEMIBLOCKS, "fheaes.h's bounds on a wrapped key are the kernel's");

static int check_kw_shape(fheaes_ctx *c, uint32_t semiblocks, uint64_t n_keys)
{
    if (semiblocks < KW_MIN_SEMIBLOCKS || semiblocks > KW_MAX_SEMIBLOCKS)
        return c->fail(FHEAES_ERR_INVALID, "semiblocks must be in %u..%u (got %u)", KW_MIN_SEMIBLOCKS, KW_MAX_SEMIBLOCKS, semiblocks);
    if (n_keys > FHEAES_KW_MAX_KEYS) return c->fail(FHEAES_ERR_INVALID, "a call unwraps at most %u keys (got %llu)", (unsigned)FHEAES_KW_MAX_KEYS, (unsigned long long)n_keys);
    return FHEAES_OK;
}

int fheaes_kw_link(fheaes_ctx *c, uint64_t *state, uint64_t *regs, uint64_t n_keys, uint32_t semiblocks, uint32_t step, const uint8_t *wrapped, int memspace)
{
    if (!c) return FHEAES_ERR_INVALID;
    CtxLock lock__(c);
    TRY(check_kw_shape(c, semiblocks, n_keys));
    if (step > 6 * semiblocks) return c->fail(FHEAES_ERR_INVALID, "step must be in 0..%u for %u semiblocks (got %u)", 6 * semiblocks, semiblocks, step);
    if (!state || !regs || (step == 0 && !wrapped)) return c->fail(FHEAES_ERR_INVALID, "null pointer");
    if (n_keys == 0) return FHEAES_OK;
    const uint64_t bw = 8ull * c->big1, state_bytes = n_keys * 16 * bw * 8, regs_bytes = n_keys * 8 * semiblocks * bw * 8;
    if (overlap(state, state_bytes, regs, regs_bytes)) return c->fail(FHEAES_ERR_INVALID, "state and regs overlap");
    HIP_TRY(c, hipSetDevice(c->device));
    Staged st(c, memspace);
    if (step == 0) {
        TRY(st.out(state, state_bytes, &state));
        TRY(st.out(regs, regs_bytes, &regs));
        const size_t bytes = n_keys * 8 * (semiblocks + 1);
        TRY(upload_pinned(c, bytes, bytes, [&](uint8_t *pin) { memcpy(pin, wrapped, bytes); }));
    } else {
        TRY(st.inout(state, state_bytes, &state));
        TRY(st.inout(regs, regs_bytes, &regs));
    }
    TRY(launch_kw_link(c, state, regs, step == 0 ? (const uint8_t *)c->ws_misc.p : nullptr, n_keys, semiblocks, step));
    return st.finish();
}

static int aes_kw_unwrap(fheaes_ctx *c, RoundKeys k, uint32_t semiblocks, const uint8_t *wrapped, uint64_t *keys_out, uint64_t *valid_out, int memspace)
{
    if (!c) return FHEAES_ERR_INVALID;
    CtxLock lock__(c);
    TRY(check_keys(c));
    const uint64_t n_keys = k.n_of;
    if (!k.words || !wrapped || !keys_out || !valid_out || (!k.key_of && k.n_keys != 1)) return c->fail(FHEAES_ERR_INVALID, "null pointer");
    TRY(check_kw_shape(c, semiblocks, n_keys));
    TRY(resolve_keys(c, k));
    if (n_keys == 0) return FHEAES_OK;
    const uint64_t bw = 8ull * c->big1, out_bytes = n_keys * 8 * semiblocks * bw * 8, valid_bytes = n_keys * c->big1 * 8ull;
    if (k.overlaps(keys_out, out_bytes) || k.overlaps(valid_out, valid_bytes) || overlap(keys_out, out_bytes, valid_out, valid_bytes))
        return c->fail(FHEAES_ERR_INVALID, "keys_out, valid_out and the round keys overlap");
    HIP_TRY(c, hipSetDevice(c->device));
    Staged st(c, memspace);
    TRY(k.stage(st));
    TRY(st.out(keys_out, out_bytes, &keys_out));
    TRY(st.out(valid_out, valid_bytes, &valid_out));
    const bool table = k.n_keys > 1;
    const size_t tab_bytes = table ? (n_keys * sizeof(uint32_t) + 31) / 32 * 32 : 0, data_bytes = n_keys * 8 * (semiblocks + 1);
    TRY(upload_pinned(c, tab_bytes + data_bytes, tab_bytes + data_bytes, [&](uint8_t *pin) {
        if (table) memcpy(pin, k.key_of, n_keys * sizeof(uint32_t));
        memcpy(pin + tab_bytes, wrapped, data_bytes);
    }));
    const uint8_t *misc = (const uint8_t *)c->ws_misc.p;
    TRY(kw_unwrap_dev(c, k.sets(table ? (const uint32_t *)misc : nullptr), k.nr, misc + tab_bytes, semiblocks, n_keys, keys_out, valid_out));
    return st.finish();
}

int fheaes_aes_kw_unwrap_keyed(fheaes_ctx *c, const uint64_t *dec_round_keys, uint32_t key_bits, uint64_t n_keks, uint64_t n_keys, const uint32_t *kek_of_key,
                               uint32_t semiblocks, const uint8_t *wrapped, uint64_t *keys_out, uint64_t *valid_out, int memspace)
{
    return aes_kw_unwrap(c, {dec_round_keys, key_bits, n_keks, kek_of_key, n_keys, false}, semiblocks, wrapped, keys_out, valid_out, memspace);
}

int fheaes_aes_kw_unwrap_keyed_packed(fheaes_ctx *c, const uint64_t *packed_dec_round_keys, uint32_t key_bits, uint64_t n_keks, uint64_t n_keys,
                                      const uint32_t *kek_of_key, uint32_t semiblocks, const uint8_t *wrapped, uint64_t *keys_out, uint64_t *valid_out, int memspace)
{
    return aes_kw_unwrap(c, {packed_dec_round_keys, key_bits, n_keks, kek_of_key, n_keys, true}, semiblocks, wrapped, keys_out, valid_out, memspace);
}

int fheaes_aes_kw_plan(uint32_t key_bits, uint32_t semiblocks, uint64_t n_keys, uint64_t *steps, uint64_t *cipher_blocks, uint64_t *byte_wopbs)
{
    const uint64_t nr = (uint64_t)aes_rounds(key_bits), n = semiblocks;
    if (!nr || n < KW_MIN_SEMIBLOCKS || n > KW_MAX_SEMIBLOCKS || n_keys > FHEAES_KW_MAX_KEYS || !steps || !cipher_blocks || !byte_wopbs) return FHEAES_ERR_INVALID;
    *steps = 6 * n;
    *cipher_blocks = 6 * n * n_keys;
    *byte_wopbs = 16 * nr * 6 * n * n_keys + 8 * n * n_keys + 16 * n_keys;
    return FHEAES_OK;
}

static_assert(GATE_LWE == FHEAES_GATE_LWE && GATE_GLWE == FHEAES_GATE_GLWE, "fheaes.h's input forms are the kernel's");

static int gate_call(fheaes_ctx *c, bool boot, const double *ggsw_fourier, const uint64_t *gates_lwe, uint64_t n_gates, const uint64_t *bits_of_gate, const uint64_t *in,
                     uint64_t m, int form, uint64_t *out, int memspace)
{
    if (!c) return FHEAES_ERR_INVALID;
    CtxLock lock__(c);
    if (boot) TRY(check_keys(c));
    if (form != GATE_LWE && form != GATE_GLWE) return c->fail(FHEAES_ERR_INVALID, "form must be 0 (LWE) or 1 (GLWE), got %d", form);
    if (n_gates && !bits_of_gate) return c->fail(FHEAES_ERR_INVALID, "null pointer");
    if (n_gates > 0xFFFFFFFFull) return c->fail(FHEAES_ERR_INVALID, "a call takes at most 2^32 - 1 gates (got %llu)", (unsigned long long)n_gates);
    const uint32_t R = gate_r(c->k1);
    const uint64_t chunk = boot ? MAX_CHUNK_BITS : 0;
    std::vector<GateWg> wgs;
    std::vector<uint64_t> chunk_end;
    uint64_t n_wgs = 0, total = 0;
    for (uint64_t g = 0; g < n_gates; ++g) {
        if (bits_of_gate[g] > m - total) { total = ~0ull; break; }
        total += bits_of_gate[g];
    }
    if (total != m) return c->fail(FHEAES_ERR_INVALID, "the runs of bits_of_gate do not add up to m = %llu", (unsigned long long)m);
    if (m == 0) return FHEAES_OK;
    if (!in || !out || (boot ? !gates_lwe : !ggsw_fourier)) return c->fail(FHEAES_ERR_INVALID, "null pointer");
    const uint64_t ggsw_words = (uint64_t)c->k1 * c->k1 * FHE_N, inst_words = form == GATE_GLWE ? (uint64_t)c->k1 * FHE_N : c->big1;
    const uint64_t bytes = m * inst_words * 8, gate_bytes = n_gates * (boot ? c->big1 : ggsw_words) * 8;
    const void *gates = boot ? (const void *)gates_lwe : (const void *)ggsw_fourier;
    if (out != in && overlap(in, bytes, out, bytes)) return c->fail(FHEAES_ERR_INVALID, "in and out overlap without being the same buffer");
    if (overlap(gates, gate_bytes, out, bytes)) return c->fail(FHEAES_ERR_INVALID, "out overlaps the gates");
    gate_table(bits_of_gate, n_gates, R, chunk, &wgs, &chunk_end, &n_wgs);
    HIP_TRY(c, hipSetDevice(c->device));
    Staged s(c, memspace);
    if (boot) TRY(s.in(gates_lwe, gate_bytes, &gates_lwe));
    else TRY(s.in(ggsw_fourier, gate_bytes, &ggsw_fourier));
    if (out == in) { TRY(s.inout(out, bytes, &out)); in = out; }
    else { TRY(s.in(in, bytes, &in)); TRY(s.out(out, bytes, &out)); }
    const size_t tab_bytes = wgs.size() * sizeof(GateWg);
    TRY(upload_pinned(c, tab_bytes, tab_bytes, [&](uint8_t *pin) { memcpy(pin, wgs.data(), tab_bytes); }));
    const GateWg *tab = (const GateWg *)c->ws_misc.p;
    if (!boot) {
        TRY(launch_gate(c, (const double2 *)ggsw_fourier, tab, n_wgs, m, form, in, out));
        return s.finish();
    }
    TRY(ensure_wopbs_ws(c, std::min<uint64_t>(n_gates, chunk)));
    uint64_t wg0 = 0;
    for (uint64_t g0 = 0, ci = 0; g0 < n_gates; g0 += chunk, ++ci) {
        const uint64_t gc = std::min<uint64_t>(chunk, n_gates - g0);
        TRY(cbs_bits(c, gates_lwe + g0 * c->big1, gc));
        uint64_t units = 0;
        for (uint64_t g = g0; g < g0 + gc; ++g) units += bits_of_gate[g];
        TRY(launch_gate(c, (const double2 *)c->ws_ggswf.p, tab + wg0, chunk_end[ci] - wg0, units, form, in, out));
        wg0 = chunk_end[ci];
    }
    return s.finish();
}

int fheaes_gate_ggsw(fheaes_ctx *c, const double *ggsw_fourier, uint64_t n_gates, const uint64_t *bits_of_gate, const uint64_t *in, uint64_t m, int form,
                     uint64_t *out, int memspace)
{
    return gate_call(c, false, ggsw_fourier, nullptr, n_gates, bits_of_gate, in, m, form, out, memspace);
}

int fheaes_gate_bits(fheaes_ctx *c, const uint64_t *gates_lwe, uint64_t n_gates, const uint64_t *bits_of_gate, const uint64_t *lwe_in, uint64_t m,
                     uint64_t *lwe_out, int memspace)
{
    return gate_call(c, true, nullptr, gates_lwe, n_gates, bits_of_gate, lwe_in, m, GATE_LWE, lwe_out, memspace);
}

int fheaes_gate_packed(fheaes_ctx *c, const uint64_t *gates_lwe, uint64_t n_gates, const uint64_t *glwes_of_gate, const uint64_t *glwe_in, uint64_t n_glwe,
                       uint64_t *glwe_out, int memspace)
{
    return gate_call(c, true, nullptr, gates_lwe, n_gates, glwes_of_gate, glwe_in, n_glwe, GATE_GLWE, glwe_out, memspace);
}

int fheaes_gate_plan(const uint64_t *bits_of_gate, uint64_t n_gates, uint32_t k, uint64_t *workgroups, uint32_t *instances_per_workgroup)
{
    if ((n_gates && !bits_of_gate) || (k != 4 && k != 1) || !workgroups || !instances_per_workgroup) return FHEAES_ERR_INVALID;
    *instances_per_workgroup = gate_r(k + 1);
    gate_table(bits_of_gate, n_gates, *instances_per_workgroup, 0, nullptr, nullptr, workgroups);
    return FHEAES_OK;
}

size_t fheaes_packed_words(const fheaes_ctx *c, uint64_t m)
{
    if (!c) return 0;
    return (size_t)((m + FHE_N - 1) / FHE_N) * c->k1 * FHE_N;
}

int fheaes_pack_bits(fheaes_ctx *c, const uint64_t *lwe_in, uint64_t m, uint64_t *glwe_out, int memspace)
{
    if (!c) return FHEAES_ERR_INVALID;
    CtxLock lock__(c);
    TRY(check_keys(c));
    if (m == 0) return FHEAES_OK;
    if (!lwe_in || !glwe_out) return c->fail(FHEAES_ERR_INVALID, "null pointer");
    const uint64_t in_bytes = m * c->big1 * 8, out_bytes = (uint64_t)fheaes_packed_words(c, m) * 8;
    if (overlap(lwe_in, in_bytes, glwe_out, out_bytes)) return c->fail(FHEAES_ERR_INVALID, "lwe_in and glwe_out overlap (packing is not in place)");
    HIP_TRY(c, hipSetDevice(c->device));
    Staged s(c, memspace);
    TRY(s.in(lwe_in, in_bytes, &lwe_in));
    TRY(s.out(glwe_out, out_bytes, &glwe_out));
    TRY(pack_dev(c, lwe_in, m, glwe_out));
    return s.finish();
}

int fheaes_unpack_bits(fheaes_ctx *c, const uint64_t *glwe_in, uint64_t m, uint64_t *lwe_out, int memspace)
{
    if (!c) return FHEAES_ERR_INVALID;
    CtxLock lock__(c);
    if (m == 0) return FHEAES_OK;
    if (!glwe_in || !lwe_out) return c->fail(FHEAES_ERR_INVALID, "null pointer");
    const uint64_t in_bytes = (uint64_t)fheaes_packed_words(c, m) * 8, out_bytes = m * c->big1 * 8;
    if (overlap(glwe_in, in_bytes, lwe_out, out_bytes)) return c->fail(FHEAES_ERR_INVALID, "glwe_in and lwe_out overlap (unpacking is not in place)");
    HIP_TRY(c, hipSetDevice(c->device));
    Staged s(c, memspace);
    TRY(s.in(glwe_in, in_bytes, &glwe_in));
    TRY(s.out(lwe_out, out_bytes, &lwe_out));
    TRY(unpack_dev(c, glwe_in, m, lwe_out));
    return s.finish();
}

uint32_t fheaes_round_keys_packed_glwes(uint32_t key_bits) { return packed_key_glwes(key_bits); }

int fheaes_pack_round_keys(fheaes_ctx *c, const uint64_t *round_keys, uint32_t key_bits, uint64_t n_keys, uint64_t *packed_out, int memspace)
{
    CtxLock lock__(c);
    TRY(check_keys(c));
    if (!round_keys || !packed_out) return c->fail(FHEAES_ERR_INVALID, "null pointer");
    TRY(check_key_bits(c, key_bits));
    TRY(check_n_keys(c, n_keys));
    const uint64_t m = (uint64_t)(aes_rounds(key_bits) + 1) * AES_BLOCK_BITS, glwes = packed_key_glwes(key_bits);
    const uint64_t in_bytes = n_keys * m * c->big1 * 8, out_bytes = n_keys * glwes * c->k1 * FHE_N * 8;
    if (overlap(round_keys, in_bytes, packed_out, out_bytes)) return c->fail(FHEAES_ERR_INVALID, "round_keys and packed_out overlap (packing is not in place)");
    HIP_TRY(c, hipSetDevice(c->device));
    Staged s(c, memspace);
    TRY(s.in(round_keys, in_bytes, &round_keys));
    TRY(s.out(packed_out, out_bytes, &packed_out));
    TRY(pack_keys_dev(c, round_keys, m, n_keys, packed_out));
    return s.finish();
}

int fheaes_unpack_round_keys(fheaes_ctx *c, const uint64_t *packed, uint32_t key_bits, uint64_t first_key, uint64_t n_keys, uint64_t *round_keys_out,
                             int memspace)
{
    CtxLock lock__(c);
    if (!c) return FHEAES_ERR_INVALID;
    if (!packed || !round_keys_out) return c->fail(FHEAES_ERR_INVALID, "null pointer");
    TRY(check_key_bits(c, key_bits));
    TRY(check_n_keys(c, n_keys));
    if (first_key > FHEAES_MAX_KEYS - n_keys)
        return c->fail(FHEAES_ERR_INVALID, "keys %llu .. %llu lie beyond the %u a store can hold", (unsigned long long)first_key,
                       (unsigned long long)(first_key + n_keys), (unsigned)FHEAES_MAX_KEYS);
    const uint64_t m = (uint64_t)(aes_rounds(key_bits) + 1) * AES_BLOCK_BITS, key_words = (uint64_t)packed_key_glwes(key_bits) * c->k1 * FHE_N;
    packed += first_key * key_words;
    const uint64_t in_bytes = n_keys * key_words * 8, out_bytes = n_keys * m * c->big1 * 8;
    if (overlap(packed, in_bytes, round_keys_out, out_bytes)) return c->fail(FHEAES_ERR_INVALID, "packed and round_keys_out overlap (unpacking is not in place)");
    HIP_TRY(c, hipSetDevice(c->device));
    Staged s(c, memspace);
    TRY(s.in(packed, in_bytes, &packed));
    TRY(s.out(round_keys_out, out_bytes, &round_keys_out));
    TRY(unpack_keys_dev(c, packed, m, n_keys, round_keys_out));
    return s.finish();
}

static bool mod_width_ok(uint32_t width) { return (width >= 8 && width <= 32) || width == 64; }

static int check_mod_width(fheaes_ctx *c, uint32_t width)
{
    if (!mod_width_ok(width)) return c->fail(FHEAES_ERR_INVALID, "width must be in 8..32, or 64 for the words as they are (got %u)", width);
    return FHEAES_OK;
}

int fheaes_expand_lwe_seeded(fheaes_ctx *c, const uint32_t *mask_key, uint64_t first_index, const uint64_t *bodies, uint64_t m, uint64_t *lwe_out,
                             int memspace)
{
    CtxLock lock__(c);
    if (!c) return FHEAES_ERR_INVALID;
    if (m == 0) return FHEAES_OK;
    if (!mask_key || !bodies || !lwe_out) return c->fail(FHEAES_ERR_INVALID, "null pointer");
    const uint64_t in_bytes = m * 8, out_bytes = m * c->big1 * 8;
    if (overlap(bodies, in_bytes, lwe_out, out_bytes)) return c->fail(FHEAES_ERR_INVALID, "bodies and lwe_out overlap (expansion is not in place)");
    MaskKey mk;
    memcpy(mk.k, mask_key, 32);
    HIP_TRY(c, hipSetDevice(c->device));
    Staged s(c, memspace);
    TRY(s.in(bodies, in_bytes, &bodies));
    TRY(s.out(lwe_out, out_bytes, &lwe_out));
    TRY(expand_lwe_dev(c, mk, first_index, bodies, m, lwe_out));
    return s.finish();
}

size_t fheaes_packed_words_mod(const fheaes_ctx *c, uint64_t m, uint32_t width)
{
    if (!c || !mod_width_ok(width)) return 0;
    return (size_t)((m + FHE_N - 1) / FHE_N) * c->k1 * (FHE_N / 64) * width;
}

int fheaes_packed_mod_switch(fheaes_ctx *c, const uint64_t *glwe_in, uint64_t n_glwe, uint32_t width, uint64_t *out, int memspace)
{
    CtxLock lock__(c);
    if (!c) return FHEAES_ERR_INVALID;
// ... 82 lines not shown
```

tfhe_aes_amd/csrc/engine_launch.h:

```cpp
#pragma once

#define MAX_CHUNK_BITS 32768ull
#define K2_CALL_MAX_BITS 65536ull
#define MAX_WOPBS_BITS 16u

namespace {

#define LATENCY_BATCH_BITS 256ull
#define K2_PAIR_MIN_BITS 768ull
struct K2Plan { int form; uint64_t units_main; uint32_t r_main; uint64_t units_tail; uint32_t r_tail; };
K2Plan k2_plan(uint64_t m, uint32_t cu_count, uint32_t k1, bool allow_pair = true)
{
    K2Plan pl{};
    if (m <= LATENCY_BATCH_BITS) { pl.form = 0; pl.units_main = m; pl.r_main = 1; return pl; }
    if (allow_pair && k1 == 5 && m > K2_PAIR_MIN_BITS) {
        pl.form = 2; pl.r_main = 6; pl.r_tail = 4;
        const uint64_t gens = (m + 6ull * cu_count - 1) / (6ull * cu_count);
        uint64_t nu = gens * cu_count;
        uint64_t four = 6 * nu >= m ? (6 * nu - m) / 2 : 0;
        if (four > nu) four = nu;
        if (four == nu && 4 * nu > m) { nu = (m + 3) / 4; four = nu; }
        pl.units_tail = four; pl.units_main = nu - four;
        return pl;
    }
    pl.form = 1;
    pl.r_main = k1 == 5 ? 3 : 8;
    pl.units_main = (m + pl.r_main - 1) / pl.r_main;
    if (k1 == 5) {
        const uint64_t slots = 2ull * cu_count;
        pl.r_tail = 2;
        if ((m + 1) / 2 <= cu_count) {
            pl.units_main = 0;
            pl.units_tail = (m + 1) / 2;
        } else if (pl.units_main > slots) {
            const uint64_t nu = slots * ((m + 3 * slots - 1) / (3 * slots));
            if (2 * nu <= m) {
                pl.units_tail = 3 * nu - m;
                pl.units_main = nu - pl.units_tail;
            }
        }
    }
    return pl;
}

#define AES_BLOCK_BITS 128ull
#define AES_WINDOW_MAX_BLOCKS (MAX_CHUNK_BITS / AES_BLOCK_BITS)
struct AesWindowPlan { uint64_t window, launches, generations, generations_by_round; };

uint64_t k2_generations(uint64_t m, uint32_t cu_count, uint32_t k1)
{
    if (m == 0) return 0;
    if (m <= K2_PAIR_MIN_BITS) return 1;
    const K2Plan pl = k2_plan(m, cu_count, k1);
    return (pl.units_main + pl.units_tail + cu_count - 1) / cu_count;
}

void aes_window_count(uint64_t n, uint64_t steps, uint64_t w, uint32_t cu_count, uint32_t k1, uint64_t *launches, uint64_t *generations)
{
    const uint64_t total = steps * n, full = total / w, rest = total % w;
    *launches = full + (rest ? 1 : 0);
    *generations = full * k2_generations(w * AES_BLOCK_BITS, cu_count, k1) + k2_generations(rest * AES_BLOCK_BITS, cu_count, k1);
}

AesWindowPlan aes_window_plan(uint64_t n, uint64_t steps, uint32_t cu_count, uint32_t k1, bool allow_pair = true)
{
    AesWindowPlan pl{};
    const uint64_t chunks = n / AES_WINDOW_MAX_BLOCKS, last = n % AES_WINDOW_MAX_BLOCKS;
    pl.launches = steps * (chunks + (last ? 1 : 0));
    pl.generations_by_round = steps * (chunks * k2_generations(MAX_CHUNK_BITS, cu_count, k1) + k2_generations(last * AES_BLOCK_BITS, cu_count, k1));
    pl.generations = pl.generations_by_round;
    if (n == 0 || steps == 0) return pl;
    const uint64_t gen_bits = 6ull * cu_count;
    if (k2_plan(std::min<uint64_t>(n * AES_BLOCK_BITS, MAX_CHUNK_BITS), cu_count, k1, allow_pair).form != 2) return pl;
    if (n * AES_BLOCK_BITS % gen_bits == 0) return pl;
    uint64_t g = AES_BLOCK_BITS, r = gen_bits;
    while (r) { const uint64_t t = g % r; g = r; r = t; }
    const uint64_t base = gen_bits / g;
    const uint64_t w = std::min<uint64_t>(n, AES_WINDOW_MAX_BLOCKS) / base * base;
    if (w == 0) return pl;
    uint64_t launches, generations;
    aes_window_count(n, steps, w, cu_count, k1, &launches, &generations);
    if (generations >= pl.generations_by_round) return pl;
    pl.window = w; pl.launches = launches; pl.generations = generations;
    return pl;
}

int launch_keyswitch(fheaes_ctx *c, const uint64_t *in, uint64_t m, uint64_t *out)
{
    if (m == 0) return FHEAES_OK;
    StageScope sc(c, FHEAES_STAGE_KEYSWITCH, m);
    const uint64_t ct_tiles16 = ((m + KS_CT_TILE - 1) / KS_CT_TILE) * (KS_CT_TILE / 16);
    TRY(ensure(c, c->ws_digits, ct_tiles16 * c->ks_ksteps * 1024));
    int8_t *af = (int8_t *)c->ws_digits.p;
    const uint64_t threads = ct_tiles16 * c->ks_ksteps * 64;
    ks_launch_digits_k1(dim3((unsigned)((threads + 255) / 256)), c->stream, in, (uint64_t)c->big1, c->big, m, c->ks_ksteps, af);
    KeyswitchArgs a{};
    a.afrag = af; a.bfrag = c->ksk_frag; a.ksteps = c->ks_ksteps; a.coltiles = c->ks_coltiles;
    a.in = in; a.in_stride = c->big1; a.body_index = (int32_t)c->big; a.body_col = c->n; a.ncols = c->n + 1;
    a.out = out; a.out_stride = c->n + 1; a.out_z_stride = 0; a.m = m;
    dim3 grid((c->ks_coltiles + KSL_COL_TILES - 1) / KSL_COL_TILES, (unsigned)((m + 16 * KSL_CT_TILES - 1) / (16 * KSL_CT_TILES)), 1);
    ks_launch_mfma_lds(1, grid, c->stream, a);
    HIP_TRY(c, hipGetLastError());
    return FHEAES_OK;
}

int launch_pfpks(fheaes_ctx *c, const uint64_t *in, uint64_t m, uint64_t *out, uint64_t out_stride, int block = -1)
{
    if (m == 0) return FHEAES_OK;
    StageScope sc(c, FHEAES_STAGE_PFPKS, m);
    const uint32_t gsz = c->k1 * FHE_N;
    const uint64_t ct_tiles16 = ((m + KS_CT_TILE - 1) / KS_CT_TILE) * (KS_CT_TILE / 16);
    TRY(ensure(c, c->ws_digits, ct_tiles16 * c->pf_ksteps * 2 * 1024));
    int8_t *af = (int8_t *)c->ws_digits.p;
    const uint64_t threads = ct_tiles16 * c->pf_ksteps * 64;
    ks_launch_digits_k3(dim3((unsigned)((threads + 255) / 256)), c->stream, in, (uint64_t)c->big1, c->big1, m, c->pf_ksteps, af);
    KeyswitchArgs a{};
    a.afrag = af; a.bfrag = c->pfpksk_frag; a.ksteps = c->pf_ksteps; a.coltiles = c->pf_coltiles;
    if (block >= 0) a.bfrag += (size_t)block * c->pf_ksteps * c->pf_coltiles * 8 * 1024;
    a.in = in; a.in_stride = c->big1; a.body_index = -1; a.body_col = 0; a.ncols = gsz;
    a.out = out; a.out_stride = out_stride; a.out_z_stride = block >= 0 ? 0 : gsz; a.m = m;
    dim3 grid((c->pf_coltiles + KSL_COL_TILES - 1) / KSL_COL_TILES, (unsigned)((m + 16 * KSL_CT_TILES - 1) / (16 * KSL_CT_TILES)), block >= 0 ? 1 : c->k1);
    ks_launch_mfma_lds(2, grid, c->stream, a);
    HIP_TRY(c, hipGetLastError());
    return FHEAES_OK;
}

int launch_forward_fourier(fheaes_ctx *c, const uint64_t *in, uint64_t polys, double2 *out, int stage)
{
    if (polys == 0) return FHEAES_OK;
    StageScope sc(c, stage, polys);
    uint64_t wgs = (polys + EP_GROUPS - 1) / EP_GROUPS;
    if (wgs > 8192) wgs = 8192;
    hipLaunchKernelGGL(forward_fourier_kernel, dim3((unsigned)wgs), dim3(EP_THREADS), 0, c->stream, in, out, polys, c->tw_d);
    HIP_TRY(c, hipGetLastError());
    return FHEAES_OK;
}

bool k2_pair_allowed(fheaes_ctx *c)
{
    if (c->k2_deny_pair) return false;
    if (c->k2_pair_ok < 0) {
        int per_cu = 0;
        const hipError_t oe = hipOccupancyMaxActiveBlocksPerMultiprocessor(&per_cu, blind_rotate_pair_kernel<5, 5, 8, 3, 2>, BRP_THREADS, 0);
        c->k2_pair_ok = (oe == hipSuccess && per_cu >= 1) ? 1 : 0;
        (void)hipGetLastError();
    }
    return c->k2_pair_ok == 1;
}

bool k2_home_allowed(fheaes_ctx *c)
{
    if (c->k1 != 5 || c->k2_deny_home) return false;
    if (c->k2_home < 0) {
        int per_cu = 0;
        const hipError_t oe = hipOccupancyMaxActiveBlocksPerMultiprocessor(&per_cu, blind_rotate16_kernel<5, 5, 8, 3, 2, true>, EP_THREADS, 0);
        c->k2_home = (oe == hipSuccess && per_cu >= 2) ? 1 : 0;
        (void)hipGetLastError();
    }
    return c->k2_home == 1;
}

static_assert(FHEAES_K2_PARK_SLOTS == BRP_PARK_SLOTS, "include/fheaes.h and kern_blindrot_pair.h disagree on the number of parking slots");
constexpr size_t PARK_OWNER_BYTES = BRP_PARK_SLOTS * sizeof(uint32_t) + BRP_PARK_TAIL_WORDS * sizeof(uint64_t);
constexpr size_t PARK_RECORD_PTR_OFFSET = BRP_PARK_SLOTS * sizeof(uint32_t) + 2 * sizeof(uint64_t);

int ensure_park_owner(fheaes_ctx *c)
{
    if (c->ws_park_owner.p) return FHEAES_OK;
    TRY(ensure(c, c->ws_park_owner, PARK_OWNER_BYTES));
    HIP_TRY(c, hipMemsetAsync(c->ws_park_owner.p, 0, PARK_OWNER_BYTES, c->stream));
    return FHEAES_OK;
}

size_t k2_pair_park_bytes(const fheaes_ctx *c, uint64_t grid)
{
    return (size_t)((c->k2_park_claim ? BRP_PARK_SLOTS : 0) + grid) * 2 * BRP_PARK_WORDS_PER_HALF * 8;
}

struct K2Launch {
    K2Plan pl;
    void (*kernel)(ExtProdArgs);
    const char *name;
    unsigned grid, threads;
    size_t park_bytes;
    bool park_owner;
};
K2Launch k2_launch(fheaes_ctx *c, uint64_t m)
{
    K2Launch L{};
    L.pl = k2_plan(m, c->cu_count, c->k1, k2_pair_allowed(c));
    L.grid = (unsigned)(L.pl.units_main + L.pl.units_tail);
    if (L.pl.form == 0) {
        L.threads = BL_THREADS;
        if (c->k1 == 5) { L.kernel = blind_rotate_latency_kernel<5, 5, 8>; L.name = "blind_rotate_latency_kernel<5,5,8>"; }
        else { L.kernel = blind_rotate_latency_kernel<2, 5, 8>; L.name = "blind_rotate_latency_kernel<2,5,8>"; }
    } else if (L.pl.form == 2) {
        L.threads = BRP_THREADS;
        L.kernel = blind_rotate_pair_kernel<5, 5, 8, 3, 2>;
        L.name = c->k2_park_claim ? "blind_rotate_pair_kernel<5,5,8,3,2> parking=claimed" : "blind_rotate_pair_kernel<5,5,8,3,2> parking=private";
        L.park_bytes = k2_pair_park_bytes(c, L.grid);
        L.park_owner = c->k2_park_claim != 0;
    } else {
        L.threads = EP_THREADS;
        if (c->k1 == 5 && k2_home_allowed(c)) { L.kernel = blind_rotate16_kernel<5, 5, 8, 3, 2, true>; L.name = "blind_rotate16_kernel<5,5,8,3,2,true>"; }
        else if (c->k1 == 5) { L.kernel = blind_rotate16_kernel<5, 5, 8, 3, 2, false>; L.name = "blind_rotate16_kernel<5,5,8,3,2,false>"; }
        else { L.kernel = blind_rotate16_kernel<2, 5, 8, 8>; L.name = "blind_rotate16_kernel<2,5,8,8,0,false>"; }
        L.park_bytes = (size_t)L.grid * BR16_PARK_WORDS_PER_WG * 8;
    }
    return L;
}

uint64_t aes_context_window(fheaes_ctx *c, uint64_t n, uint64_t steps)
{
    if (n == 0 || steps == 0 || c->aes_window == FHEAES_AES_WINDOW_OFF) return 0;
    if (c->aes_window) return std::min<uint64_t>(c->aes_window, std::min<uint64_t>(n, AES_WINDOW_MAX_BLOCKS));
    const bool pair = k2_launch(c, std::min<uint64_t>(n * AES_BLOCK_BITS, MAX_CHUNK_BITS)).pl.form == 2;
    return aes_window_plan(n, steps, c->cu_count, c->k1, pair).window;
}

static_assert(FHEAES_AUDIT_MAX_ROWS == AUDIT_MAX_ROWS && FHEAES_AUDIT_RECORDS == AUDIT_RECORDS, "include/fheaes.h and kern_audit.h disagree");
static_assert(AUDIT_MAX_ROWS <= LATENCY_BATCH_BITS, "the audit's rows are one latency-form launch");
int launch_audit(fheaes_ctx *c, const ExtProdArgs &prod)
{
    const uint64_t m = prod.count, launch = c->audit_launch++;
    const uint32_t S = (uint32_t)std::min<uint64_t>(c->audit_rows, m);
    if (c->audit_hook) {
        c->audit_hook = false;
        if (c->audit_hook_row < m)
            hipLaunchKernelGGL(audit_tamper_kernel, dim3(1), dim3(1), 0, c->stream, prod.out, c->big1, c->audit_hook_row, c->audit_hook_word, c->audit_hook_mask);
    }
    uint64_t *const in = (uint64_t *)c->audit_in.p, *const out = (uint64_t *)c->audit_out.p;
    hipLaunchKernelGGL(audit_gather_kernel, dim3(S), dim3(AUDIT_THREADS), 0, c->stream, prod.lwe_in, c->n + 1, c->audit_seed, launch, m, S, in);
    ExtProdArgs a{};
    a.ggsw = prod.ggsw; a.tw = prod.tw; a.iters = prod.iters;
    a.tv_const = prod.tv_const; a.body_shift = prod.body_shift; a.post_add = prod.post_add;
    a.lwe_in = in; a.out = out; a.count = S;
    void (*const latency)(ExtProdArgs) = c->k1 == 5 ? blind_rotate_latency_kernel<5, 5, 8> : blind_rotate_latency_kernel<2, 5, 8>;
    hipLaunchKernelGGL(latency, dim3(S), dim3(BL_THREADS), 0, c->stream, a);
    hipLaunchKernelGGL(audit_compare_kernel, dim3(S), dim3(AUDIT_THREADS), 0, c->stream, prod.out, out, c->big1, c->audit_seed, launch, m, S,
                       (uint64_t *)c->audit_state.p);
    HIP_TRY(c, hipGetLastError());
    return FHEAES_OK;
}

int launch_cbs_pbs(fheaes_ctx *c, const uint64_t *lwe_small, uint64_t m, uint32_t level, uint64_t *out)
{
    if (m == 0) return FHEAES_OK;
    if ((uint64_t)c->n * c->p.pbs_level * c->k1 * c->k1 * FHE_H * 16 > 0x7FFFFFFFull)
        return c->fail(FHEAES_ERR_INVALID, "bootstrapping key larger than 2 GiB is not supported by the blind-rotation kernels");
    StageScope sc(c, FHEAES_STAGE_BLIND_ROTATE, m);
    ExtProdArgs a{};
    a.ggsw = c->bskf; a.tw = c->tw_d;
    a.out = out; a.count = m; a.iters = c->n; a.lwe_in = lwe_small;
    const uint64_t half_delta = 1ull << (64 - c->p.cbs_base_log * level - 1);
    a.tv_const = (uint64_t)0 - half_delta; a.body_shift = 1ull << 62; a.post_add = half_delta;
    const K2Launch L = k2_launch(c, m);
    if (L.pl.form != 0) a.units_main = (uint32_t)L.pl.units_main;
    if (L.park_bytes) {
        if (L.park_bytes > 0x7FFFFFFFull) return c->fail(FHEAES_ERR_INVALID, "internal: parking slab of %zu bytes exceeds one raw buffer", L.park_bytes);
        TRY(ensure(c, c->ws_park, L.park_bytes));
        a.park = (uint64_t *)c->ws_park.p; a.park_bytes = L.park_bytes;
    }
    if (L.park_owner) {
        TRY(ensure_park_owner(c));
        if (c->k2_park_pattern)
            HIP_TRY(c, hipMemcpyAsync(c->ws_park_owner.p, c->ws_park_pattern.p, BRP_PARK_SLOTS * sizeof(uint32_t), hipMemcpyDeviceToDevice, c->stream));
        else
            HIP_TRY(c, hipMemsetAsync(c->ws_park_owner.p, 0, BRP_PARK_SLOTS * sizeof(uint32_t), c->stream));
        a.park_owner = (uint32_t *)c->ws_park_owner.p;
        if (c->k2_park_record) {
            TRY(ensure(c, c->ws_park_record, (size_t)L.grid * 2 * sizeof(uint32_t)));
            HIP_TRY(c, hipMemsetAsync(c->ws_park_record.p, 0xFF, (size_t)L.grid * 2 * sizeof(uint32_t), c->stream));
            const uint64_t rp = (uint64_t)(uintptr_t)c->ws_park_record.p;
            uint32_t *const rp_word = (uint32_t *)((char *)c->ws_park_owner.p + PARK_RECORD_PTR_OFFSET);
            HIP_TRY(c, hipMemsetD32Async((hipDeviceptr_t)rp_word, (int)(uint32_t)rp, 1, c->stream));
            HIP_TRY(c, hipMemsetD32Async((hipDeviceptr_t)(rp_word + 1), (int)(uint32_t)(rp >> 32), 1, c->stream));
            c->k2_park_record_n = L.grid;
        }
    }
#ifdef EP_STAMPS
    static const char *namesL[EP_NPH] = {"barrier (result) + accumulate", "rotate+decompose (1 coeff x K1)", "read digits + forward fft", "digit stores", "barrier (digits)", "MAC", "barrier (MAC done)",
                                         "products store + next rows", "barrier (products)", "inverse fft -> doubles", "barrier (acc)", "barrier (decomposition)"};
    static const char *namesT[EP_NPH] = {"stage+rotate+decomp_first", "decomp_next", "fwd head", "pre-level barrier", "fwd tail (transpose+dft16)",
                                         "digit stores+late loads", "exchange barrier", "MAC", "products exchange", "inverse fft", "convert+add", "loop head"};
    StampReport rep(c, (size_t)L.grid * (L.threads / 64), L.pl.form == 0 ? namesL : namesT, L.pl.form == 0 ? 8 : 0);
    a.stamps = rep.d;
#endif
    hipLaunchKernelGGL(L.kernel, dim3(L.grid), dim3(L.threads), 0, c->stream, a);
    HIP_TRY(c, hipGetLastError());
    if (c->audit_rows && m >= c->audit_min_bits) TRY(launch_audit(c, a));
    return FHEAES_OK;
}

int launch_vertical_packing(fheaes_ctx *c, const double2 *ggswf, uint64_t n_inputs, uint32_t bits, const uint64_t *luts,
                            uint32_t n_luts, int per_input, uint64_t *out)
{
    if (n_inputs == 0) return FHEAES_OK;
    StageScope sc(c, FHEAES_STAGE_VERTICAL_PACKING, n_inputs * n_luts * bits);
    const bool k4 = c->k1 == 5;
    const uint32_t R = k4 ? 3 : 8;
    void (*const cmux_kernel)(CmuxArgs) = k4 ? cmux_level_kernel<5, 15, 3> : cmux_level_kernel<2, 15, 8>;
    void (*const vp_kernel)(VpArgs) = k4 ? vertical_packing_kernel<5, 15, 3> : vertical_packing_kernel<2, 15, 8>;
    const uint32_t inst_per_input = n_luts * bits;
    const uint64_t W = lut_row_words(bits);
    const uint64_t *glwe_root = nullptr;
    if (bits > 9) {
        const uint32_t tree_bits = bits - 9;
        const uint64_t instances = n_inputs * inst_per_input, gsz = (uint64_t)c->k1 * FHE_N;
        const uint64_t half_words = instances * (1ull << (tree_bits - 1)) * gsz;
        TRY(ensure(c, c->ws_tree, 2 * half_words * 8));
        uint64_t *buf[2] = {(uint64_t *)c->ws_tree.p, (uint64_t *)c->ws_tree.p + half_words};
        for (uint32_t t = 0; t < tree_bits; ++t) {
            CmuxArgs a{};
            a.ggsw = ggswf; a.tw = c->tw_d;
            a.luts = t == 0 ? luts : nullptr; a.in = t == 0 ? nullptr : buf[(t - 1) & 1]; a.out = buf[t & 1];
            a.bits = bits; a.bit = 9 + t; a.nodes_out = 1u << (tree_bits - 1 - t);
            a.inst_per_input = inst_per_input; a.lut_per_input = per_input ? 1 : 0; a.lut_words = W;
            const uint64_t jobs = (uint64_t)inst_per_input * a.nodes_out;
            a.wg_per_input = (uint32_t)((jobs + R - 1) / R);
            hipLaunchKernelGGL(cmux_kernel, dim3((unsigned)(n_inputs * a.wg_per_input)), dim3(EP_THREADS), 0, c->stream, a);
            HIP_TRY(c, hipGetLastError());
        }
        glwe_root = buf[(tree_bits - 1) & 1];
    }
    VpArgs a{};
    a.ggsw = ggswf; a.tw = c->tw_d;
    a.out = out; a.iters = bits < 9 ? bits : 9; a.ggsw_per_input = bits;
    a.luts = luts; a.lut_words = W; a.glwe_in = glwe_root;
    a.lut_per_input = per_input ? 1 : 0; a.inst_per_input = inst_per_input;
    a.wg_per_input = (inst_per_input + R - 1) / R;
    hipLaunchKernelGGL(vp_kernel, dim3((unsigned)(n_inputs * a.wg_per_input)), dim3(EP_THREADS), 0, c->stream, a);
    HIP_TRY(c, hipGetLastError());
    return FHEAES_OK;
}

#define GATE_MAX_GRID 65536ull
uint32_t gate_r(uint32_t k1) { return k1 == 5 ? 3 : 8; }

uint64_t gate_table(const uint64_t *bits_of_gate, uint64_t n_gates, uint32_t R, uint64_t chunk, std::vector<GateWg> *wgs, std::vector<uint64_t> *chunk_end,
                    uint64_t *n_wgs)
{
    uint64_t first = 0, count = 0;
    for (uint64_t g = 0; g < n_gates; ++g) {
        const uint64_t run = bits_of_gate[g];
        if (wgs)
            for (uint64_t i = 0; i < run; i += R)
                wgs->push_back({first + i, (uint32_t)(chunk ? g % chunk : g), (uint32_t)std::min<uint64_t>(R, run - i)});
        count += (run + R - 1) / R;
        first += run;
        if (chunk_end && chunk && ((g + 1) % chunk == 0 || g + 1 == n_gates)) chunk_end->push_back(count);
    }
    *n_wgs = count;
    return first;
}

int launch_gate(fheaes_ctx *c, const double2 *ggswf, const GateWg *wgs, uint64_t n_wgs, uint64_t units, int form, const uint64_t *in, uint64_t *out)
{
    if (n_wgs == 0) return FHEAES_OK;
    StageScope sc(c, FHEAES_STAGE_VERTICAL_PACKING, form == GATE_GLWE ? units * FHE_N : units);
    const bool k4 = c->k1 == 5;
    void (*const kernel)(GateArgs) = form == GATE_GLWE ? (k4 ? gate_kernel<5, 15, 3, GATE_GLWE> : gate_kernel<2, 15, 8, GATE_GLWE>)
                                                       : (k4 ? gate_kernel<5, 15, 3, GATE_LWE> : gate_kernel<2, 15, 8, GATE_LWE>);
    for (uint64_t w0 = 0; w0 < n_wgs; w0 += GATE_MAX_GRID) {
        GateArgs a{};
        a.ggsw = ggswf; a.tw = c->tw_d; a.wgs = wgs + w0; a.in = in; a.out = out;
        hipLaunchKernelGGL(kernel, dim3((unsigned)std::min<uint64_t>(GATE_MAX_GRID, n_wgs - w0)), dim3(EP_THREADS), 0, c->stream, a);
        HIP_TRY(c, hipGetLastError());
    }
    return FHEAES_OK;
}

int noise_guard(fheaes_ctx *c, uint32_t level, const char *what)
{
    if (level > c->noise_level_seen) c->noise_level_seen = level;
    if (level > FHEAES_MAX_NOISE_LEVEL)
        return c->fail(FHEAES_ERR_INVALID, "%s would sum %u nominal-noise ciphertexts; the parameter set allows %u (MaxNoiseLevel, client.rs:92)", what, level,
                       (unsigned)FHEAES_MAX_NOISE_LEVEL);
    return FHEAES_OK;
}

struct KeySets {
    const uint64_t *rk;
    const uint32_t *of_block;
    uint64_t stride;
    uint32_t packed_glwes = 0, bit0 = 0;
    KeySets round(uint64_t r, uint64_t sw, uint64_t first_block = 0) const
    {
        const uint32_t *of = of_block ? of_block + first_block : nullptr;
        if (packed_glwes) return {rk, of, stride, packed_glwes, bit0 + (uint32_t)(r * AES_BLOCK_BITS)};
        return {rk + r * sw, of, stride};
    }
};

template <class F>
static void with_keys(const fheaes_ctx *c, const KeySets &k, F &&f)
{
    if (k.packed_glwes) f(PackedKeys{k.rk, k.stride, k.bit0, c->k});
    else f(LweKeys{k.rk, k.stride});
}

int launch_gather(fheaes_ctx *c, const uint64_t *src, uint32_t n_luts, const KeySets &k, uint64_t *out, uint64_t n_blocks, const GatherTable &t)
{
    if (n_blocks == 0) return FHEAES_OK;
    TRY(noise_guard(c, (uint32_t)t.terms + (k.rk ? 1u : 0u), "the linear layer (MixColumns / ShiftRows + AddRoundKey)"));
    StageScope sc(c, FHEAES_STAGE_LINEAR, n_blocks);
    dim3 grid((8 * c->big1 + 1023) / 1024, 16, (unsigned)n_blocks);
    with_keys(c, k, [&](auto keys) {
        hipLaunchKernelGGL(gather_add_kernel<decltype(keys)>, grid, dim3(256), 0, c->stream, src, n_luts, keys, k.of_block, out, n_blocks, c->big1, t);
    });
    HIP_TRY(c, hipGetLastError());
    return FHEAES_OK;
}

dim3 block_rows_grid(uint64_t words_per_item, uint64_t n)
{
    const unsigned gx = (unsigned)std::min<uint64_t>((words_per_item + 255) / 256, 64);
    return dim3(gx, (unsigned)std::min<uint64_t>(n, std::max<uint64_t>(1, 16384 / gx)));
}

int launch_add_bcast(fheaes_ctx *c, uint64_t *dst, const KeySets &k, uint64_t words_per_block, uint64_t n_blocks)
{
    if (n_blocks == 0) return FHEAES_OK;
    TRY(noise_guard(c, 2, "the initial AddRoundKey"));
    StageScope sc(c, FHEAES_STAGE_LINEAR, n_blocks);
    const dim3 grid = block_rows_grid(words_per_block, n_blocks);
    with_keys(c, k, [&](auto keys) {
        hipLaunchKernelGGL(add_bcast_kernel<decltype(keys)>, grid, dim3(256), 0, c->stream, dst, keys, k.of_block, words_per_block, n_blocks, c->big1);
    });
    HIP_TRY(c, hipGetLastError());
    return FHEAES_OK;
}

int launch_key_rows(fheaes_ctx *c, uint64_t *dst, uint64_t dst_stride, const uint64_t *a, uint64_t a_stride, uint32_t rot, const uint64_t *b,
                    uint64_t b_stride, uint32_t rcon, uint32_t n_bytes, uint64_t n_keys, uint32_t level)
{
    if (level > 1) TRY(noise_guard(c, level, "a key-expansion word sum"));
    StageScope sc(c, FHEAES_STAGE_LINEAR, n_keys);
    dim3 grid((8 * c->big1 + 1023) / 1024, n_bytes, (unsigned)std::min<uint64_t>(n_keys, 65535));
    hipLaunchKernelGGL(key_rows_kernel, grid, dim3(256), 0, c->stream, dst, dst_stride, a, a_stride, rot, b, b_stride, rcon, c->big1, n_keys);
    HIP_TRY(c, hipGetLastError());
    return FHEAES_OK;
}

int launch_xts_tweaks(fheaes_ctx *c, const uint64_t *anchor, uint64_t anchor_stride, uint64_t n_units, uint32_t off0, uint32_t n_off, uint64_t *out)
{
    if (n_off == 0 || off0 > XTS_MAX_OFFSET || n_off > XTS_MAX_OFFSET + 1 - off0)
        return c->fail(FHEAES_ERR_INVALID, "XTS tweak offsets %u .. %u: one gather reaches offset %u at most", off0, off0 + n_off - 1, XTS_MAX_OFFSET);
    if (n_units == 0) return FHEAES_OK;
    uint32_t weight = 0, s[4];
    for (uint32_t j = off0; j < off0 + n_off; ++j)
        for (uint32_t i = 0; i < 128; ++i) weight = std::max(weight, xts_tweak_row(j, i, s));
    TRY(noise_guard(c, weight, "the XTS tweak layer (multiplication by alpha^j)"));
    StageScope sc(c, FHEAES_STAGE_LINEAR, n_units * n_off);
    const uint64_t rows = n_units * n_off * 128;
    hipLaunchKernelGGL(bit_rows_kernel<XtsRows>, dim3((unsigned)std::min<uint64_t>(rows, 1u << 20)), dim3(256), 0, c->stream,
                       XtsRows{anchor, anchor_stride, n_off, off0}, out, rows, c->big1);
    HIP_TRY(c, hipGetLastError());
    return FHEAES_OK;
}

int launch_xts_whiten(fheaes_ctx *c, uint64_t *dst, const uint64_t *src, const uint64_t *tweaks, const uint32_t *tweak_of_block, const uint8_t *clear,
                      uint64_t n_blocks, uint32_t level)
{
    if (n_blocks == 0) return FHEAES_OK;
    TRY(noise_guard(c, level, "the XTS whitening (tweak + block)"));
    StageScope sc(c, FHEAES_STAGE_LINEAR, n_blocks);
    const dim3 grid = block_rows_grid(128ull * c->big1, n_blocks);
    hipLaunchKernelGGL(xts_whiten_kernel, grid, dim3(256), 0, c->stream, dst, src, tweaks, tweak_of_block, clear, n_blocks, c->big1);
    HIP_TRY(c, hipGetLastError());
    return FHEAES_OK;
}

int launch_mac_link(fheaes_ctx *c, uint64_t *dst, const uint64_t *a, const uint64_t *b, const MacSlot *slots, uint64_t n_slots, uint32_t level, const char *what)
{
    if (n_slots == 0) return FHEAES_OK;
    TRY(noise_guard(c, level, what));
    StageScope sc(c, FHEAES_STAGE_LINEAR, n_slots);
    const dim3 grid = block_rows_grid(128ull * c->big1, n_slots);
    hipLaunchKernelGGL(mac_link_kernel, grid, dim3(256), 0, c->stream, dst, a, b, slots, n_slots, c->big1);
    HIP_TRY(c, hipGetLastError());
    return FHEAES_OK;
}

// ... 6 lines not shown
                                                           : "a key-unwrap link (cipher output + counter + the round key that follows)"));
    StageScope sc(c, FHEAES_STAGE_LINEAR, n_keys);
    const dim3 grid = block_rows_grid(128ull * c->big1, n_keys);
    hipLaunchKernelGGL(kw_link_kernel, grid, dim3(256), 0, c->stream, state, regs, wrapped, n_keys, n, step, c->big1);
    HIP_TRY(c, hipGetLastError());
    return FHEAES_OK;
}

int launch_cmac_double(fheaes_ctx *c, const uint64_t *l, uint64_t n_keys, uint64_t *out)
{
    if (n_keys == 0) return FHEAES_OK;
    static_assert(256ull * FHEAES_MAX_KEYS <= 0x7FFFFFFFull, "the rows of FHEAES_MAX_KEYS keys are one grid dimension");
    TRY(noise_guard(c, 3, "the CMAC subkey layer (multiplication by x and x^2)"));
    StageScope sc(c, FHEAES_STAGE_LINEAR, n_keys);
    hipLaunchKernelGGL(bit_rows_kernel<CmacRows>, dim3((unsigned)(n_keys * 256)), dim3(256), 0, c->stream, CmacRows{l, c->big1}, out, n_keys * 256, c->big1);
    HIP_TRY(c, hipGetLastError());
    return FHEAES_OK;
}

static_assert(PACK_N == FHE_N && PACK_N % PACK_FOLD_ROWS == 0, "kern_linear.h's packing kernels are written for N = 512");

static void launch_mod_switch(fheaes_ctx *c, const uint64_t *glwe, uint64_t n_glwe, uint32_t width, uint64_t *out)
{
    const uint32_t gsz = c->k1 * FHE_N;
    const uint64_t total = n_glwe * (gsz / 64 * width);
    hipLaunchKernelGGL(mod_switch_pack_kernel, dim3((unsigned)std::min<uint64_t>((total + 255) / 256, 65536)), dim3(256), 0, c->stream, glwe, n_glwe, gsz,
                       width, out);
}

int pack_dev(fheaes_ctx *c, const uint64_t *in, uint64_t m, uint64_t *out, uint32_t width = 64)
{
    if (m == 0) return FHEAES_OK;
    const uint64_t gsz = (uint64_t)c->k1 * FHE_N;
    uint64_t chunk = c->ws_ggsw.bytes / (gsz * 8) / FHE_N * FHE_N;
    if (chunk == 0) {
        chunk = std::min<uint64_t>((m + FHE_N - 1) / FHE_N * FHE_N, MAX_CHUNK_BITS);
        TRY(ensure(c, c->ws_ggsw, chunk * gsz * 8));
    }
    chunk = std::min<uint64_t>(chunk, MAX_CHUNK_BITS);
    if (width != 64) TRY(ensure(c, c->ws_tmp_a, (std::min<uint64_t>(chunk, m) + FHE_N - 1) / FHE_N * gsz * 8));
    uint64_t *ks = (uint64_t *)c->ws_ggsw.p;
    for (uint64_t t0 = 0; t0 < m; t0 += chunk) {
        const uint64_t mc = std::min<uint64_t>(chunk, m - t0), glwes = (mc + FHE_N - 1) / FHE_N;
        TRY(launch_pfpks(c, in + t0 * c->big1, mc, ks, gsz, (int)c->k));
        uint64_t *o = width == 64 ? out + t0 / FHE_N * gsz : (uint64_t *)c->ws_tmp_a.p;
        StageScope sc(c, FHEAES_STAGE_LINEAR, mc);
        HIP_TRY(c, hipMemsetAsync(o, 0, glwes * gsz * 8, c->stream));
        hipLaunchKernelGGL(pack_fold_kernel, dim3(FHE_N / PACK_FOLD_ROWS, c->k1, (unsigned)glwes), dim3(256), 0, c->stream, ks, mc, c->k1, o);
        HIP_TRY(c, hipGetLastError());
        if (width != 64) {
            launch_mod_switch(c, o, glwes, width, out + t0 / FHE_N * (gsz / 64 * width));
            HIP_TRY(c, hipGetLastError());
        }
    }
    return FHEAES_OK;
}

int unpack_dev(fheaes_ctx *c, const uint64_t *in, uint64_t m, uint64_t *out)
{
    for (uint64_t t0 = 0; t0 < m; t0 += MAX_CHUNK_BITS) {
        const uint64_t mc = std::min<uint64_t>(MAX_CHUNK_BITS, m - t0);
        StageScope sc(c, FHEAES_STAGE_LINEAR, mc);
        hipLaunchKernelGGL(sample_extract_kernel, dim3((unsigned)((mc + UNPACK_BITS_PER_WG - 1) / UNPACK_BITS_PER_WG)), dim3(256), 0, c->stream,
                           in + t0 / FHE_N * (uint64_t)c->k1 * FHE_N, mc, c->k, out + t0 * c->big1);
        HIP_TRY(c, hipGetLastError());
    }
    return FHEAES_OK;
}

int pack_keys_dev(fheaes_ctx *c, const uint64_t *in, uint64_t m, uint64_t n_keys, uint64_t *out)
{
    const uint64_t gsz = (uint64_t)c->k1 * FHE_N, glwes = (m + FHE_N - 1) / FHE_N, max_keys = MAX_CHUNK_BITS / m;
    uint64_t chunk = c->ws_ggsw.bytes / (gsz * 8) / m;
    if (chunk == 0) {
        chunk = std::min<uint64_t>(n_keys, max_keys);
        TRY(ensure(c, c->ws_ggsw, chunk * m * gsz * 8));
    }
    chunk = std::min<uint64_t>(chunk, max_keys);
    uint64_t *ks = (uint64_t *)c->ws_ggsw.p;
    for (uint64_t j0 = 0; j0 < n_keys; j0 += chunk) {
        const uint64_t kc = std::min<uint64_t>(chunk, n_keys - j0);
        TRY(launch_pfpks(c, in + j0 * m * c->big1, kc * m, ks, gsz, (int)c->k));
        uint64_t *o = out + j0 * glwes * gsz;
        StageScope sc(c, FHEAES_STAGE_LINEAR, kc * m);
        HIP_TRY(c, hipMemsetAsync(o, 0, kc * glwes * gsz * 8, c->stream));
        for (uint64_t j = 0; j < kc; ++j)
            hipLaunchKernelGGL(pack_fold_kernel, dim3(FHE_N / PACK_FOLD_ROWS, c->k1, (unsigned)glwes), dim3(256), 0, c->stream, ks + j * m * gsz, m, c->k1,
                               o + j * glwes * gsz);
        HIP_TRY(c, hipGetLastError());
    }
    return FHEAES_OK;
}

int unpack_keys_dev(fheaes_ctx *c, const uint64_t *in, uint64_t m, uint64_t n_keys, uint64_t *out)
{
    const uint64_t key_words = (m + FHE_N - 1) / FHE_N * c->k1 * FHE_N;
    for (uint64_t j = 0; j < n_keys; ++j) TRY(unpack_dev(c, in + j * key_words, m, out + j * m * c->big1));
    return FHEAES_OK;
}

int mod_switch_dev(fheaes_ctx *c, const uint64_t *in, uint64_t n_glwe, uint32_t width, uint64_t *out)
{
    const uint64_t gsz = (uint64_t)c->k1 * FHE_N, step = MAX_CHUNK_BITS / FHE_N;
    for (uint64_t g0 = 0; g0 < n_glwe; g0 += step) {
        const uint64_t gc = std::min<uint64_t>(step, n_glwe - g0);
        StageScope sc(c, FHEAES_STAGE_LINEAR, gc * FHE_N);
        launch_mod_switch(c, in + g0 * gsz, gc, width, out + g0 * (gsz / 64 * width));
        HIP_TRY(c, hipGetLastError());
    }
    return FHEAES_OK;
}

int unpack_mod_dev(fheaes_ctx *c, const uint64_t *in, uint64_t m, uint32_t width, uint64_t *out)
{
    for (uint64_t t0 = 0; t0 < m; t0 += MAX_CHUNK_BITS) {
        const uint64_t mc = std::min<uint64_t>(MAX_CHUNK_BITS, m - t0);
        StageScope sc(c, FHEAES_STAGE_LINEAR, mc);
        hipLaunchKernelGGL(sample_extract_mod_kernel, dim3((unsigned)((mc + UNPACK_BITS_PER_WG - 1) / UNPACK_BITS_PER_WG)), dim3(256), 0, c->stream,
                           in + t0 / FHE_N * (uint64_t)c->k1 * 8 * width, mc, c->k, width, out + t0 * c->big1);
        HIP_TRY(c, hipGetLastError());
    }
    return FHEAES_OK;
}

int expand_lwe_dev(fheaes_ctx *c, const MaskKey &key, uint64_t first_index, const uint64_t *bodies, uint64_t m, uint64_t *out)
{
    for (uint64_t t0 = 0; t0 < m; t0 += MAX_CHUNK_BITS) {
        const uint64_t mc = std::min<uint64_t>(MAX_CHUNK_BITS, m - t0);
        StageScope sc(c, FHEAES_STAGE_LINEAR, mc);
        hipLaunchKernelGGL(expand_lwe_kernel, dim3((unsigned)((mc * c->k + 3) / 4)), dim3(256), 0, c->stream, out + t0 * c->big1, bodies + t0, mc, c->k,
                           first_index + t0, key);
        HIP_TRY(c, hipGetLastError());
    }
    return FHEAES_OK;
}

int check_keys(fheaes_ctx *c)
{
    if (!c) return FHEAES_ERR_INVALID;
    if (!c->have_keys) return c->fail(FHEAES_ERR_NOKEYS, "evaluation keys have not been uploaded");
    return FHEAES_OK;
}

int ensure_wopbs_ws(fheaes_ctx *c, uint64_t bits)
{
    const uint64_t ggsw_words = (uint64_t)c->k1 * c->k1 * FHE_N;
    TRY(ensure(c, c->ws_small, bits * (c->n + 1) * 8));
    TRY(ensure(c, c->ws_pbs, bits * c->big1 * 8));
    TRY(ensure(c, c->ws_ggsw, bits * ggsw_words * 8));
    TRY(ensure(c, c->ws_ggswf, bits * ggsw_words * 8));
    return FHEAES_OK;
}

int cbs_from_small(fheaes_ctx *c, uint64_t m)
{
    const uint64_t ggsw_words = (uint64_t)c->k1 * c->k1 * FHE_N;
    TRY(launch_cbs_pbs(c, (const uint64_t *)c->ws_small.p, m, 1, (uint64_t *)c->ws_pbs.p));
    TRY(launch_pfpks(c, (const uint64_t *)c->ws_pbs.p, m, (uint64_t *)c->ws_ggsw.p, ggsw_words));
    TRY(launch_forward_fourier(c, (const uint64_t *)c->ws_ggsw.p, m * c->k1 * c->k1, (double2 *)c->ws_ggswf.p, FHEAES_STAGE_GGSW_FFT));
    return FHEAES_OK;
}

int cbs_bits(fheaes_ctx *c, const uint64_t *in, uint64_t m)
{
    TRY(launch_keyswitch(c, in, m, (uint64_t *)c->ws_small.p));
    return cbs_from_small(c, m);
}

int wopbs_dev(fheaes_ctx *c, const uint64_t *lwe_in, uint64_t n_inputs, uint32_t bits, const uint64_t *luts, uint32_t n_luts,
              int per_input, uint64_t *lwe_out)
{
    if (bits < 1 || bits > MAX_WOPBS_BITS) return c->fail(FHEAES_ERR_INVALID, "bits_per_input must be in 1..%u (got %u)", MAX_WOPBS_BITS, bits);
    if (n_luts < 1) return c->fail(FHEAES_ERR_INVALID, "n_luts must be >= 1");
    if (n_inputs == 0) return FHEAES_OK;
    uint64_t chunk_inputs = std::max<uint64_t>(1, MAX_CHUNK_BITS / bits);
    if (bits > 9) {
        const uint64_t per_input = (uint64_t)n_luts * bits * (1ull << (bits - 9)) * c->k1 * FHE_N * 8;
        chunk_inputs = std::max<uint64_t>(1, std::min<uint64_t>(chunk_inputs, (2ull << 30) / per_input));
    }
    const uint64_t W = lut_row_words(bits);
    TRY(ensure_wopbs_ws(c, std::min<uint64_t>(n_inputs, chunk_inputs) * bits));
    for (uint64_t i0 = 0; i0 < n_inputs; i0 += chunk_inputs) {
        const uint64_t ni = std::min<uint64_t>(chunk_inputs, n_inputs - i0);
        TRY(cbs_bits(c, lwe_in + i0 * bits * c->big1, ni * bits));
        const uint64_t *l = per_input ? luts + i0 * n_luts * bits * W : luts;
        TRY(launch_vertical_packing(c, (const double2 *)c->ws_ggswf.p, ni, bits, l, n_luts, per_input, lwe_out + i0 * n_luts * bits * c->big1));
    }
    return FHEAES_OK;
}

}
```

tfhe_aes_amd/csrc/kern_extprod.h:

```cpp
#pragma once
#include "fft_dev.h"

#define EP_THREADS 256
#define EP_EARLY_LOAD 2
#define EP_MAC_PRIO 1
#define EP_ROT_CHUNK 4
#define EP_PREFETCH 2
#define EP_MIN_WAVES 2
#define EP_GROUPS 16
#define EP_LDS_DOUBLES (EP_GROUPS * GROUP_TILE_DOUBLES + 2 * FHE_TW_ENTRIES)

__device__ __forceinline__ void ep_load_table(double2 *tw_lds, const double2 *tw_g)
{
    for (int i = threadIdx.x; i < FHE_TW_ENTRIES; i += blockDim.x) tw_lds[i] = tw_g[i];
}

struct ExtProdArgs {
    const double2 *ggsw;
    const double2 *tw;
    uint64_t *out;
    uint64_t count;
    uint32_t iters;
    const uint64_t *lwe_in;
    uint64_t tv_const;
    uint64_t body_shift;
    uint64_t post_add;
    uint64_t *park;
    uint64_t park_bytes;
    uint32_t *park_owner;
    uint32_t units_main;
#ifdef EP_STAMPS
    unsigned long long *stamps;
#endif
};

typedef unsigned ep_u32x4 __attribute__((ext_vector_type(4)));
#define EP_KEY_AUX 0
__device__ __forceinline__ double2 ep_key_load(__amdgpu_buffer_rsrc_t rsrc, unsigned lane_bytes, unsigned row_bytes)
{
    ep_u32x4 v = __builtin_amdgcn_raw_buffer_load_b128(rsrc, lane_bytes, row_bytes, EP_KEY_AUX);
    double2 d;
    d.x = __longlong_as_double((long long)(((unsigned long long)v[1] << 32) | v[0]));
    d.y = __longlong_as_double((long long)(((unsigned long long)v[3] << 32) | v[2]));
    return d;
}

template <int K1, int R>
__device__ __forceinline__ void ep_product_once(double (&xr)[16], double (&xi)[16], const double2 *ggsws, const uint32_t which, double *lds,
                                                const double2 *tw, double *tile, const int tid, const int b)
{
    nega_fwd(xr, xi, tw, tile, b);
#pragma unroll
    for (int k2 = 0; k2 < 16; ++k2) {
        double2 v; v.x = xr[k2]; v.y = xi[k2];
        *reinterpret_cast<double2 *>(tile + 2 * (b + 16 * k2)) = v;
    }
    __syncthreads();
    double fr[R][K1], fi[R][K1];
#pragma unroll
    for (int r = 0; r < R; ++r)
#pragma unroll
        for (int c = 0; c < K1; ++c) { fr[r][c] = 0.0; fi[r][c] = 0.0; }
    const double2 *G = ggsws + (size_t)which * (size_t)(K1 * K1 * FHE_H) + tid;
#pragma unroll
    for (int p = 0; p < K1; ++p) {
        double2 bv[K1];
#pragma unroll
        for (int c = 0; c < K1; ++c) bv[c] = G[(size_t)(p * K1 + c) * FHE_H];
#pragma unroll
        for (int r = 0; r < R; ++r) {
            const double2 d = *reinterpret_cast<const double2 *>(lds + (r * K1 + p) * GROUP_TILE_DOUBLES + 2 * tid);
#pragma unroll
            for (int c = 0; c < K1; ++c) {
                fr[r][c] = __builtin_fma(d.x, bv[c].x, fr[r][c]);
                fr[r][c] = __builtin_fma(-d.y, bv[c].y, fr[r][c]);
                fi[r][c] = __builtin_fma(d.x, bv[c].y, fi[r][c]);
                fi[r][c] = __builtin_fma(d.y, bv[c].x, fi[r][c]);
            }
        }
    }
    __syncthreads();
#pragma unroll
    for (int r = 0; r < R; ++r)
#pragma unroll
        for (int c = 0; c < K1; ++c) {
            double2 v; v.x = fr[r][c]; v.y = fi[r][c];
            *reinterpret_cast<double2 *>(lds + (r * K1 + c) * GROUP_TILE_DOUBLES + 2 * tid) = v;
        }
    __syncthreads();
#pragma unroll
    for (int k2 = 0; k2 < 16; ++k2) {
        double2 v = *reinterpret_cast<const double2 *>(tile + 2 * (b + 16 * k2));
        xr[k2] = v.x; xi[k2] = v.y;
    }
    wave_lds_sync();
    nega_inv(xr, xi, tw, tile, b);
}

#ifdef EP_STAMPS
#define EP_NPH 12
#define EP_STAMP(ph) do { unsigned long long t__ = __builtin_readcyclecounter(); ph_cyc[ph] += t__ - t_last; t_last = t__; } while (0)
#else
#define EP_STAMP(ph) do { } while (0)
#endif

struct VpArgs {
    const double2 *ggsw;
    const double2 *tw;
    uint64_t *out;
    uint32_t iters;
    const uint64_t *luts;
    uint32_t lut_per_input;
    uint32_t inst_per_input;
    uint32_t wg_per_input;
    uint32_t ggsw_per_input;
    uint64_t lut_words;
    const uint64_t *glwe_in;
};

template <int K1, int BASE_LOG, int R>
__global__ __launch_bounds__(EP_THREADS, EP_MIN_WAVES) void vertical_packing_kernel(const VpArgs A)
{
    static_assert(R * K1 <= EP_GROUPS, "too many polynomials for 16 lane groups");
    __shared__ __attribute__((aligned(16))) double lds[EP_LDS_DOUBLES];
    double2 *tw = reinterpret_cast<double2 *>(lds + EP_GROUPS * GROUP_TILE_DOUBLES);

    const int tid = threadIdx.x;
    const int g = tid >> 4, b = tid & 15;
    const bool owner = g < R * K1;
    const int r_own = owner ? g / K1 : R - 1;
    const int p_own = owner ? g % K1 : K1 - 1;
    double *tile = lds + g * GROUP_TILE_DOUBLES;

    ep_load_table(tw, A.tw);

    const uint64_t input = blockIdx.x / A.wg_per_input;
    uint32_t local = (blockIdx.x % A.wg_per_input) * R + r_own;
    const bool valid = local < A.inst_per_input;
    if (!valid) local = A.inst_per_input - 1;
    const uint64_t inst = input * A.inst_per_input + local;

    uint64_t lo[16], hi[16];
    if (A.glwe_in) {
        const uint64_t *src = A.glwe_in + (inst * K1 + p_own) * FHE_N;
#pragma unroll
        for (int a = 0; a < 16; ++a) { lo[a] = src[16 * a + b]; hi[a] = src[256 + 16 * a + b]; }
    } else {
        const uint64_t set = A.lut_per_input ? input : 0;
        const uint64_t *lut = A.luts + (set * A.inst_per_input + inst % A.inst_per_input) * A.lut_words;
#pragma unroll
        for (int a = 0; a < 16; ++a) {
            lo[a] = (p_own == K1 - 1) ? lut[16 * a + b] : 0;
            hi[a] = (p_own == K1 - 1) ? lut[256 + 16 * a + b] : 0;
        }
    }
    __syncthreads();

    const size_t ggsw_stride = (size_t)K1 * K1 * FHE_H;

    for (uint32_t it = 0; it < A.iters; ++it) {
        const int t = (1024 - (1 << it)) & 1023;
        const double2 *G = A.ggsw + ((size_t)input * A.ggsw_per_input + it) * ggsw_stride;

        uint64_t *stage = reinterpret_cast<uint64_t *>(tile);
#pragma unroll
        for (int a = 0; a < 16; ++a) {
            stage[16 * a + b] = lo[a];
            stage[256 + 16 * a + b] = hi[a];
        }
        wave_lds_sync();
        double xr[16], xi[16];
#pragma unroll
        for (int a = 0; a < 16; ++a) {
            int j0 = 16 * a + b, j1 = j0 + 256;
            int s0 = (j0 - t) & 511, s1 = (j1 - t) & 511;
            uint64_t v0 = stage[s0], v1 = stage[s1];
            if (((s0 + t) >> 9) & 1) v0 = (uint64_t)0 - v0;
            if (((s1 + t) >> 9) & 1) v1 = (uint64_t)0 - v1;
            v0 -= lo[a]; v1 -= hi[a];
            uint32_t st;
            xr[a] = (double)decompose_first<BASE_LOG, 1>(v0, st);
            xi[a] = (double)decompose_first<BASE_LOG, 1>(v1, st);
            if ((a & (EP_ROT_CHUNK - 1)) == EP_ROT_CHUNK - 1) __builtin_amdgcn_sched_barrier(0);
        }
        wave_lds_sync();

        double fr[R][K1], fi[R][K1];
#pragma unroll
        for (int r = 0; r < R; ++r)
#pragma unroll
            for (int c = 0; c < K1; ++c) { fr[r][c] = 0.0; fi[r][c] = 0.0; }

        auto level_body = [&]() {
            {
                double2 w0[8], w1[8];
                fft_fwd_table(w0, w1, tw, b);
                nega_fwd_head(xr, xi, w0, w1);
            }
            nega_fwd_tail(xr, xi, tile, b);
            const double2 *Gl = G + tid;
            constexpr int PF = (K1 < EP_PREFETCH) ? K1 : EP_PREFETCH;
            constexpr int EARLY = (EP_EARLY_LOAD < PF) ? EP_EARLY_LOAD : PF;
            constexpr int CHUNK = (K1 * 2 * 2 + 3) / 4;
            double2 bq[PF][K1];
#pragma unroll
            for (int e = 0; e < EARLY; ++e) {
#pragma unroll
                for (int k2 = e * CHUNK; k2 < (e + 1) * CHUNK && k2 < 16; ++k2) {
                    double2 v; v.x = xr[k2]; v.y = xi[k2];
                    *reinterpret_cast<double2 *>(tile + 2 * (b + 16 * k2)) = v;
                }
                __builtin_amdgcn_sched_barrier(0);
#pragma unroll
                for (int c = 0; c < K1; ++c) bq[e][c] = Gl[(size_t)(e * K1 + c) * FHE_H];
                __builtin_amdgcn_sched_barrier(0);
            }
#pragma unroll
            for (int k2 = (EARLY * CHUNK < 16 ? EARLY * CHUNK : 16); k2 < 16; ++k2) {
                double2 v; v.x = xr[k2]; v.y = xi[k2];
                *reinterpret_cast<double2 *>(tile + 2 * (b + 16 * k2)) = v;
            }
            __builtin_amdgcn_sched_barrier(0);
            wg_barrier_lds_only();
            __builtin_amdgcn_s_setprio(EP_MAC_PRIO);
            __builtin_amdgcn_sched_barrier(0);
#pragma unroll
            for (int p = EARLY; p < PF; ++p)
#pragma unroll
                for (int c = 0; c < K1; ++c) bq[p][c] = Gl[(size_t)(p * K1 + c) * FHE_H];
            __builtin_amdgcn_sched_barrier(0);
#pragma unroll
            for (int p = 0; p < K1; ++p) {
                double2 bv[K1];
#pragma unroll
                for (int c = 0; c < K1; ++c) bv[c] = bq[p % PF][c];
                if (p + PF < K1) {
#pragma unroll
                    for (int c = 0; c < K1; ++c) bq[p % PF][c] = Gl[(size_t)((p + PF) * K1 + c) * FHE_H];
                }
                __builtin_amdgcn_sched_barrier(0);
#pragma unroll
                for (int r = 0; r < R; ++r) {
                    double2 d = *reinterpret_cast<const double2 *>(lds + (r * K1 + p) * GROUP_TILE_DOUBLES + 2 * tid);
#pragma unroll
                    for (int c = 0; c < K1; ++c) {
                        fr[r][c] = __builtin_fma(d.x, bv[c].x, fr[r][c]);
                        fr[r][c] = __builtin_fma(-d.y, bv[c].y, fr[r][c]);
                        fi[r][c] = __builtin_fma(d.x, bv[c].y, fi[r][c]);
                        fi[r][c] = __builtin_fma(d.y, bv[c].x, fi[r][c]);
                    }
                }
                __builtin_amdgcn_sched_barrier(0);
            }
            __builtin_amdgcn_s_setprio(0);
        };
        level_body();

        __syncthreads();
#pragma unroll
        for (int r = 0; r < R; ++r)
#pragma unroll
            for (int c = 0; c < K1; ++c) {
                double2 v; v.x = fr[r][c]; v.y = fi[r][c];
                *reinterpret_cast<double2 *>(lds + (r * K1 + c) * GROUP_TILE_DOUBLES + 2 * tid) = v;
            }
        __syncthreads();
#pragma unroll
        for (int k2 = 0; k2 < 16; ++k2) {
            double2 v = *reinterpret_cast<const double2 *>(tile + 2 * (b + 16 * k2));
            xr[k2] = v.x; xi[k2] = v.y;
        }
        wave_lds_sync();
        nega_inv(xr, xi, tw, tile, b);
#pragma unroll
        for (int a = 0; a < 16; ++a) {
            lo[a] += torus_from_double(xr[a]);
            hi[a] += torus_from_double(xi[a]);
        }
    }

    if (owner && valid) {
        const uint64_t big = (uint64_t)(K1 - 1) * FHE_N;
        uint64_t *o = A.out + inst * (big + 1);
        if (p_own < K1 - 1) {
            uint64_t *om = o + (uint64_t)p_own * FHE_N;
#pragma unroll
            for (int a = 0; a < 16; ++a) {
                int j0 = 16 * a + b, j1 = j0 + 256;
                if (j0 == 0) om[0] = lo[a]; else om[FHE_N - j0] = (uint64_t)0 - lo[a];
                om[FHE_N - j1] = (uint64_t)0 - hi[a];
            }
        } else if (b == 0) {
            o[big] = lo[0];
        }
    }
}

struct CmuxArgs {
    const double2 *ggsw;
    const double2 *tw;
    const uint64_t *luts;
    const uint64_t *in;
    uint64_t *out;
    uint32_t bits, bit;
    uint32_t nodes_out;
    uint32_t inst_per_input;
    uint32_t lut_per_input;
    uint32_t wg_per_input;
    uint64_t lut_words;
};

template <int K1, int BASE_LOG, int R>
__global__ __launch_bounds__(EP_THREADS, 2) void cmux_level_kernel(const CmuxArgs A)
{
    static_assert(R * K1 <= EP_GROUPS, "too many polynomials for 16 lane groups");
    __shared__ __attribute__((aligned(16))) double lds[EP_LDS_DOUBLES];
    double2 *tw = reinterpret_cast<double2 *>(lds + EP_GROUPS * GROUP_TILE_DOUBLES);
    const int tid = threadIdx.x;
    const int g = tid >> 4, b = tid & 15;
    const bool owner = g < R * K1;
    const int r_own = owner ? g / K1 : R - 1;
    const int p_own = owner ? g % K1 : K1 - 1;
    double *tile = lds + g * GROUP_TILE_DOUBLES;
    ep_load_table(tw, A.tw);

    const uint64_t input = blockIdx.x / A.wg_per_input;
    const uint32_t jobs_per_input = A.inst_per_input * A.nodes_out;
    uint32_t local = (blockIdx.x % A.wg_per_input) * R + r_own;
    const bool valid = owner && local < jobs_per_input;
    if (local >= jobs_per_input) local = jobs_per_input - 1;
    const uint32_t instl = local / A.nodes_out, node = local % A.nodes_out;
    const uint64_t inst = input * A.inst_per_input + instl;

    uint64_t c0lo[16], c0hi[16];
    double xr[16], xi[16];
    {
        const uint64_t *p0, *p1;
        bool zero = false;
        if (A.luts) {
            const uint64_t set = A.lut_per_input ? input : 0;
            const uint64_t *lut = A.luts + (set * A.inst_per_input + instl) * A.lut_words;
            p0 = lut + (uint64_t)(2 * node) * FHE_N;
            p1 = p0 + FHE_N;
            zero = p_own != K1 - 1;
        } else {
            p0 = A.in + ((inst * (2 * A.nodes_out) + 2 * node) * K1 + p_own) * FHE_N;
            p1 = p0 + (uint64_t)K1 * FHE_N;
        }
#pragma unroll
        for (int a = 0; a < 16; ++a) {
            const uint64_t a0 = zero ? 0 : p0[16 * a + b], a1 = zero ? 0 : p0[256 + 16 * a + b];
            const uint64_t b0 = zero ? 0 : p1[16 * a + b], b1 = zero ? 0 : p1[256 + 16 * a + b];
            c0lo[a] = a0; c0hi[a] = a1;
            uint32_t st;
            xr[a] = (double)decompose_first<BASE_LOG, 1>(b0 - a0, st);
            xi[a] = (double)decompose_first<BASE_LOG, 1>(b1 - a1, st);
        }
    }
    __syncthreads();
    ep_product_once<K1, R>(xr, xi, A.ggsw, (uint32_t)(input * A.bits + A.bit), lds, tw, tile, tid, b);
    if (valid) {
        uint64_t *o = A.out + ((inst * A.nodes_out + node) * K1 + p_own) * FHE_N;
#pragma unroll
        for (int a = 0; a < 16; ++a) {
            o[16 * a + b] = c0lo[a] + torus_from_double(xr[a]);
            o[256 + 16 * a + b] = c0hi[a] + torus_from_double(xi[a]);
        }
    }
}

__global__ __launch_bounds__(EP_THREADS) void forward_fourier_kernel(const uint64_t *in, double2 *out, uint64_t polys, const double2 *tw_g)
{
    __shared__ __attribute__((aligned(16))) double lds[EP_LDS_DOUBLES];
    double2 *tw = reinterpret_cast<double2 *>(lds + EP_GROUPS * GROUP_TILE_DOUBLES);
    const int tid = threadIdx.x, g = tid >> 4, b = tid & 15;
    double *tile = lds + g * GROUP_TILE_DOUBLES;
    ep_load_table(tw, tw_g);
    __syncthreads();
    for (uint64_t base = (uint64_t)blockIdx.x * EP_GROUPS; base < polys; base += (uint64_t)gridDim.x * EP_GROUPS) {
        uint64_t q = base + g;
        bool valid = q < polys;
        if (!valid) q = polys - 1;
        const uint64_t *p = in + q * FHE_N;
        double xr[16], xi[16];
#pragma unroll
        for (int a = 0; a < 16; ++a) {
            xr[a] = double_from_torus(p[16 * a + b]);
            xi[a] = double_from_torus(p[256 + 16 * a + b]);
        }
        nega_fwd(xr, xi, tw, tile, b);
        if (valid) {
            double2 *o = out + q * FHE_H;
#pragma unroll
            for (int k2 = 0; k2 < 16; ++k2) { double2 v; v.x = xr[k2]; v.y = xi[k2]; o[b + 16 * k2] = v; }
        }
    }
}
```

tfhe_aes_amd/csrc/kern_keyswitch.h:

```cpp
#pragma once
#include <hip/hip_runtime.h>
#include <stdint.h>
#include "fft_dev.h"

#define KS_CT_TILE 64
#define KS_KSTEP 64

typedef int ks_int4 __attribute__((ext_vector_type(4)));

struct KeyswitchArgs {
    const int8_t *afrag;
    const int8_t *bfrag;
    uint32_t ksteps, coltiles;
    const uint64_t *in;
    uint64_t in_stride;
    int32_t body_index;
    uint32_t body_col;
    uint32_t ncols;
    uint64_t *out;
    uint64_t out_stride, out_z_stride;
    uint64_t m;
};

#define KSL_CT_TILES 8
#define KSL_THREADS (64 * KSL_CT_TILES)
#define KSL_COL_TILES 4

#ifndef FHEAES_KS_DECLS_ONLY
__global__ __launch_bounds__(256) void keybytes_kernel(const uint64_t *key, uint64_t key_z_stride, uint32_t rows, uint32_t ncols,
                                                       uint32_t ksteps, uint32_t coltiles, int8_t *frag)
{
    const uint64_t gid = (uint64_t)blockIdx.x * blockDim.x + threadIdx.x;
    const uint32_t lane = gid & 63;
    const uint64_t t = gid >> 6;
    const uint32_t C = t % coltiles;
    const uint32_t ks = (uint32_t)(t / coltiles);
    const uint32_t z = blockIdx.y;
    if (ks >= ksteps) return;
    const uint32_t col = C * 16 + (lane & 15);
    const uint32_t row0 = ks * KS_KSTEP + (lane >> 4) * 16;
    int8_t b[8][16];
#pragma unroll
    for (int e = 0; e < 16; ++e) {
        uint64_t x = 0;
        if (col < ncols && row0 + e < rows) x = key[(uint64_t)z * key_z_stride + (uint64_t)(row0 + e) * ncols + col];
        uint32_t carry = 0;
#pragma unroll
        for (int j = 0; j < 8; ++j) {
            uint32_t v = (uint32_t)((x >> (8 * j)) & 0xFF) + carry;
            carry = v >= 128 ? 1u : 0u;
            b[j][e] = (int8_t)(v & 0xFF);
        }
    }
    int8_t *o = frag + ((((uint64_t)z * ksteps + ks) * coltiles + C) * 8) * 1024 + (uint64_t)lane * 16;
#pragma unroll
    for (int j = 0; j < 8; ++j) {
        ks_int4 w;
        memcpy(&w, b[j], 16);
        *reinterpret_cast<ks_int4 *>(o + (uint64_t)j * 1024) = w;
    }
}

template <int BASE_LOG, int LEVELS, int PLANES>
__global__ __launch_bounds__(256) void digits_kernel(const uint64_t *in, uint64_t in_stride, uint32_t n_in, uint64_t m,
                                                     uint32_t ksteps, int8_t *frag)
{
    const uint64_t gid = (uint64_t)blockIdx.x * blockDim.x + threadIdx.x;
    const uint32_t lane = gid & 63;
    const uint64_t t = gid >> 6;
    const uint32_t ks = t % ksteps;
    const uint64_t T = t / ksteps;
    const uint64_t ct = T * 16 + (lane & 15);
    const uint32_t q0 = ks * KS_KSTEP + (lane >> 4) * 16;
    int8_t lo[16], hi[16];
#pragma unroll
    for (int e = 0; e < 16; ++e) { lo[e] = 0; hi[e] = 0; }
    if (ct < m) {
        const uint32_t i0 = q0 / LEVELS;
        constexpr int NI = (16 + LEVELS - 1) / LEVELS + 1;
#pragma unroll
        for (int ii = 0; ii < NI; ++ii) {
            const uint32_t i = i0 + ii;
            if (i >= n_in) break;
            int d[LEVELS];
            decompose_all<BASE_LOG, LEVELS>(in[ct * in_stride + i], d);
#pragma unroll
            for (int l = 0; l < LEVELS; ++l) {
                const int e = (int)(i * LEVELS + l) - (int)q0;
                if (e >= 0 && e < 16) {
                    const int dl = ((d[l] + 128) & 255) - 128;
#pragma unroll
                    for (int ee = 0; ee < 16; ++ee) if (ee == e) { lo[ee] = (int8_t)dl; hi[ee] = (int8_t)((d[l] - dl) >> 8); }
                }
            }
        }
    }
    int8_t *o = frag + ((T * ksteps + ks) * PLANES) * 1024 + (uint64_t)lane * 16;
    ks_int4 w;
    memcpy(&w, lo, 16);
    *reinterpret_cast<ks_int4 *>(o) = w;
    if (PLANES == 2) {
        memcpy(&w, hi, 16);
        *reinterpret_cast<ks_int4 *>(o + 1024) = w;
    }
}

template <int PLANES>
__global__ __launch_bounds__(KSL_THREADS, 2) void keyswitch_mfma_lds_kernel(const KeyswitchArgs A)
{
    constexpr int A_FRAGS = KSL_CT_TILES * PLANES;
    constexpr int B_FRAGS = KSL_COL_TILES * 8;
    constexpr int FRAGS = A_FRAGS + B_FRAGS;
    __shared__ __attribute__((aligned(16))) int8_t lds[2 * FRAGS * 1024];
    const int lane = threadIdx.x & 63, wave = threadIdx.x >> 6;
    const int wc = wave & 3, wt = wave >> 2;
    const uint32_t C0 = blockIdx.x * KSL_COL_TILES;
    const uint64_t T0 = (uint64_t)blockIdx.y * KSL_CT_TILES;
    const uint32_t z = blockIdx.z;
    const uint64_t ct_tiles_total = (A.m + 15) / 16;

    ks_int4 acc[4][8];
#pragma unroll
    for (int t = 0; t < 4; ++t)
#pragma unroll
        for (int s = 0; s < 8; ++s) acc[t][s] = (ks_int4){0, 0, 0, 0};

    auto issue = [&](uint32_t ks, int buf) {
        constexpr int WAVES = KSL_THREADS / 64;
#pragma unroll
        for (int i = 0; i < (FRAGS + WAVES - 1) / WAVES; ++i) {
            const int f = wave + WAVES * i;
            if (f < FRAGS) {
                const int8_t *src;
                if (f < A_FRAGS) {
                    uint64_t T = T0 + f / PLANES;
                    if (T >= ct_tiles_total) T = ct_tiles_total - 1;
                    src = A.afrag + ((T * A.ksteps + ks) * PLANES + (f % PLANES)) * 1024;
                } else {
                    const int g = f - A_FRAGS;
                    uint32_t C = C0 + g / 8;
                    if (C >= A.coltiles) C = A.coltiles - 1;
                    src = A.bfrag + ((((uint64_t)z * A.ksteps + ks) * A.coltiles + C) * 8 + (g % 8)) * 1024;
                }
                __builtin_amdgcn_global_load_lds((const __attribute__((address_space(1))) void *)(src + lane * 16),
                                                 (__attribute__((address_space(3))) void *)(lds + ((size_t)buf * FRAGS + f) * 1024), 16, 0, 0);
            }
        }
    };

    issue(0, 0);
    for (uint32_t ks = 0; ks < A.ksteps; ++ks) {
        const int buf = ks & 1;
        asm volatile("s_waitcnt vmcnt(0)" ::: "memory");
        __syncthreads();
        if (ks + 1 < A.ksteps) issue(ks + 1, buf ^ 1);
        const int8_t *base = lds + (size_t)buf * FRAGS * 1024 + lane * 16;
        ks_int4 a[4][PLANES], b[8];
#pragma unroll
        for (int s = 0; s < 8; ++s) b[s] = *reinterpret_cast<const ks_int4 *>(base + (A_FRAGS + wc * 8 + s) * 1024);
#pragma unroll
        for (int t = 0; t < 4; ++t)
#pragma unroll
            for (int pl = 0; pl < PLANES; ++pl) a[t][pl] = *reinterpret_cast<const ks_int4 *>(base + ((wt * 4 + t) * PLANES + pl) * 1024);
#pragma unroll
        for (int s = 0; s < 8; ++s) {
#pragma unroll
            for (int t = 0; t < 4; ++t) acc[t][s] = __builtin_amdgcn_mfma_i32_16x16x64_i8(a[t][0], b[s], acc[t][s], 0, 0, 0);
            if (PLANES == 2 && s >= 1) {
#pragma unroll
                for (int t = 0; t < 4; ++t) acc[t][s] = __builtin_amdgcn_mfma_i32_16x16x64_i8(a[t][1], b[s - 1], acc[t][s], 0, 0, 0);
            }
        }
    }

    const uint32_t C = C0 + wc;
    const uint32_t col = C * 16 + (lane & 15);
    if (C >= A.coltiles || col >= A.ncols) return;
#pragma unroll
    for (int t = 0; t < 4; ++t)
#pragma unroll
        for (int r = 0; r < 4; ++r) {
            const uint64_t ct = (T0 + wt * 4 + t) * 16 + (uint64_t)(lane >> 4) * 4 + r;
            if (ct >= A.m) continue;
            uint64_t v = 0;
#pragma unroll
            for (int s = 0; s < 8; ++s) v += (uint64_t)(int64_t)acc[t][s][r] << (8 * s);
            v = (uint64_t)0 - v;
            if (A.body_index >= 0 && col == A.body_col) v += A.in[ct * A.in_stride + (uint32_t)A.body_index];
            A.out[ct * A.out_stride + (uint64_t)z * A.out_z_stride + col] = v;
        }
}
#endif
```

tfhe_aes_amd/csrc/ks_launch.h:

```cpp
#pragma once
#ifdef FHEAES_SPLIT_KS
#ifndef FHEAES_KS_TU
#define FHEAES_KS_DECLS_ONLY
#endif
#endif
#include "kern_keyswitch.h"

#if defined(FHEAES_SPLIT_KS) && !defined(FHEAES_KS_TU)
#define FHEAES_KS_LAUNCH_DECL
#else
#define FHEAES_KS_LAUNCH_DEFINE
#ifdef FHEAES_SPLIT_KS
#define FHEAES_KS_LAUNCH_LINKAGE
#else
#define FHEAES_KS_LAUNCH_LINKAGE static inline
#endif
#endif

#ifdef FHEAES_KS_LAUNCH_DECL
void ks_launch_digits_k1(dim3 grid, hipStream_t s, const uint64_t *in, uint64_t in_stride, uint32_t n_in, uint64_t m, uint32_t ksteps, int8_t *frag);
void ks_launch_digits_k3(dim3 grid, hipStream_t s, const uint64_t *in, uint64_t in_stride, uint32_t n_in, uint64_t m, uint32_t ksteps, int8_t *frag);
void ks_launch_mfma_lds(int planes, dim3 grid, hipStream_t s, const KeyswitchArgs &a);
void ks_launch_keybytes(dim3 grid, hipStream_t s, const uint64_t *key, uint64_t key_z_stride, uint32_t rows, uint32_t ncols, uint32_t ksteps,
                        uint32_t coltiles, int8_t *frag);
#endif

#ifdef FHEAES_KS_LAUNCH_DEFINE
FHEAES_KS_LAUNCH_LINKAGE void ks_launch_digits_k1(dim3 grid, hipStream_t s, const uint64_t *in, uint64_t in_stride, uint32_t n_in, uint64_t m, uint32_t ksteps, int8_t *frag)
{
    hipLaunchKernelGGL((digits_kernel<2, 6, 1>), grid, dim3(256), 0, s, in, in_stride, n_in, m, ksteps, frag);
}
FHEAES_KS_LAUNCH_LINKAGE void ks_launch_digits_k3(dim3 grid, hipStream_t s, const uint64_t *in, uint64_t in_stride, uint32_t n_in, uint64_t m, uint32_t ksteps, int8_t *frag)
{
    hipLaunchKernelGGL((digits_kernel<12, 3, 2>), grid, dim3(256), 0, s, in, in_stride, n_in, m, ksteps, frag);
}
FHEAES_KS_LAUNCH_LINKAGE void ks_launch_mfma_lds(int planes, dim3 grid, hipStream_t s, const KeyswitchArgs &a)
{
    if (planes == 1) hipLaunchKernelGGL((keyswitch_mfma_lds_kernel<1>), grid, dim3(KSL_THREADS), 0, s, a);
    else hipLaunchKernelGGL((keyswitch_mfma_lds_kernel<2>), grid, dim3(KSL_THREADS), 0, s, a);
}
FHEAES_KS_LAUNCH_LINKAGE void ks_launch_keybytes(dim3 grid, hipStream_t s, const uint64_t *key, uint64_t key_z_stride, uint32_t rows, uint32_t ncols, uint32_t ksteps,
                                          uint32_t coltiles, int8_t *frag)
{
    hipLaunchKernelGGL(keybytes_kernel, grid, dim3(256), 0, s, key, key_z_stride, rows, ncols, ksteps, coltiles, frag);
}
#endif
```

Baseline: 60.98 blocks/s.

## Skip unused GGSW rows for the first vertical-packing bit

The circuit bootstrap now computes only the last GLWE row (k1 polys) of the GGSW for the first bit of each input. That row is used in a special first CMUX iteration, where the accumulator is the trivial LUT GLWE and only its body term contributes. A new row layout places these partial GGSWs after the full ones, and pfpks, the forward FFT and vertical packing index rows through it. This removes pfpks and FFT work for k of the k1 GGSW rows on one bit in eight, and makes the first external product cheaper. In exchange it adds index remapping in several kernels and an extra launch per stage.

```diff
diff --git a/include/fheaes.h b/include/fheaes.h
--- a/include/fheaes.h
+++ b/include/fheaes.h
@@ -253,6 +253,7 @@
 int fheaes_k2_set_forms(fheaes_ctx *ctx, int allow_pair, int allow_home);
 int fheaes_aes_window_plan(uint64_t n_blocks, uint32_t steps, uint32_t cu_count, uint32_t k, uint64_t *window_blocks, uint64_t *launches,
                            uint64_t *generations, uint64_t *generations_by_round);
+int fheaes_cbs_row(uint64_t n_inputs, uint32_t bits, uint64_t input, uint32_t bit, uint64_t *row);
 int fheaes_aes_context_window(fheaes_ctx *ctx, uint64_t n_blocks, uint32_t steps, uint64_t *window_blocks);
 #define FHEAES_AES_WINDOW_OFF 0xFFFFFFFFu
 int fheaes_aes_set_window(fheaes_ctx *ctx, uint32_t window_blocks);
diff --git a/tfhe_aes_amd/_native.py b/tfhe_aes_amd/_native.py
--- a/tfhe_aes_amd/_native.py
+++ b/tfhe_aes_amd/_native.py
@@ -149,6 +149,7 @@
     "fheaes_k2_set_parking": (_c.c_int, [_ctx, _c.c_int]),
     "fheaes_k2_set_forms": (_c.c_int, [_ctx, _c.c_int, _c.c_int]),
     "fheaes_aes_window_plan": (_c.c_int, [_c.c_uint64, _c.c_uint32, _c.c_uint32, _c.c_uint32, _u64p, _u64p, _u64p, _u64p]),
+    "fheaes_cbs_row": (_c.c_int, [_c.c_uint64, _c.c_uint32, _c.c_uint64, _c.c_uint32, _u64p]),
     "fheaes_aes_context_window": (_c.c_int, [_ctx, _c.c_uint64, _c.c_uint32, _u64p]),
     "fheaes_aes_set_window": (_c.c_int, [_ctx, _c.c_uint32]),
     "fheaes_k2_park_debug": (_c.c_int, [_ctx, _c.POINTER(_c.c_uint32), _c.c_int]),
@@ -837,6 +838,14 @@
     return {"window": w.value, "launches": la.value, "generations": g.value, "generations_by_round": gr.value}
 
 
+def cbs_row(n_inputs: int, bits: int, input: int, bit: int) -> int:
+    row = _c.c_uint64()
+    rc = load_library().fheaes_cbs_row(n_inputs, bits, input, bit, _c.byref(row))
+    if rc != 0:
+        raise FheAesError(rc, "fheaes_cbs_row: bits in 1..16, input < n_inputs, bit < bits")
+    return row.value
+
+
 def get_twiddles() -> np.ndarray:
     out = np.empty((512, 2), dtype=np.float64)
     rc = load_library().fheaes_get_twiddles(out.ctypes.data_as(_dp))
diff --git a/tfhe_aes_amd/csrc/aes_schedule.h b/tfhe_aes_amd/csrc/aes_schedule.h
--- a/tfhe_aes_amd/csrc/aes_schedule.h
+++ b/tfhe_aes_amd/csrc/aes_schedule.h
@@ -69,13 +69,13 @@
         }
         return FHEAES_OK;
     }
-    const uint64_t ggsw_words = (uint64_t)c->k1 * c->k1 * FHE_N, total = steps * n_blocks;
+    const uint64_t total = steps * n_blocks;
     TRY(ensure_wopbs_ws(c, w * AES_BLOCK_BITS));
     uint64_t *small = (uint64_t *)c->ws_small.p;
     const double2 *ggswf = (const double2 *)c->ws_ggswf.p;
     struct Segment { const AesStep *st; uint64_t first, blocks, row; uint64_t *vp; };
     for (uint64_t i0 = 0; i0 < total; i0 += w) {
-        const uint64_t len = std::min<uint64_t>(w, total - i0), s = i0 / n_blocks, b0 = i0 % n_blocks, m = len * AES_BLOCK_BITS;
+        const uint64_t len = std::min<uint64_t>(w, total - i0), s = i0 / n_blocks, b0 = i0 % n_blocks;
         Segment seg[2] = {{&sch.steps[s], b0, std::min<uint64_t>(len, n_blocks - b0), 0, vp}, {}};
         int n_seg = 1;
         if (seg[0].blocks < len) {
@@ -84,15 +84,15 @@
         }
         for (int g = 0; g < n_seg; ++g)
             TRY(launch_keyswitch(c, state + seg[g].first * sw, seg[g].blocks * AES_BLOCK_BITS, small + seg[g].row * AES_BLOCK_BITS * (c->n + 1)));
-        TRY(cbs_from_small(c, m));
+        const CbsRows rows{16 * len, 8};
+        TRY(cbs_from_small(c, rows));
         if (n_seg == 1 || seg[0].st->set == seg[1].st->set) {
             const int set = seg[0].st->set;
-            TRY(launch_vertical_packing(c, ggswf, 16 * len, 8, c->lutset_d[set], (uint32_t)c->lutset_n[set], 0, vp));
+            TRY(launch_vertical_packing(c, ggswf, 16 * len, 8, c->lutset_d[set], (uint32_t)c->lutset_n[set], 0, vp, rows));
         } else {
             for (int g = 0; g < n_seg; ++g) {
                 const int set = seg[g].st->set;
-                TRY(launch_vertical_packing(c, ggswf + seg[g].row * AES_BLOCK_BITS * (ggsw_words / 2), 16 * seg[g].blocks, 8, c->lutset_d[set],
-                                            (uint32_t)c->lutset_n[set], 0, seg[g].vp));
+                TRY(launch_vertical_packing(c, ggswf, 16 * seg[g].blocks, 8, c->lutset_d[set], (uint32_t)c->lutset_n[set], 0, seg[g].vp, rows, 16 * seg[g].row));
             }
         }
         for (int g = 0; g < n_seg; ++g)
diff --git a/tfhe_aes_amd/csrc/engine.hip b/tfhe_aes_amd/csrc/engine.hip
--- a/tfhe_aes_amd/csrc/engine.hip
+++ b/tfhe_aes_amd/csrc/engine.hip
@@ -107,6 +107,12 @@
     if (!window_blocks || !launches || !generations || !generations_by_round || n_blocks == 0 || steps == 0 || cu_count == 0) return FHEAES_ERR_INVALID;
     const AesWindowPlan pl = aes_window_plan(n_blocks, steps, cu_count, k + 1);
     *window_blocks = pl.window; *launches = pl.launches; *generations = pl.generations; *generations_by_round = pl.generations_by_round;
+    return FHEAES_OK;
+}
+int fheaes_cbs_row(uint64_t n_inputs, uint32_t bits, uint64_t input, uint32_t bit, uint64_t *row)
+{
+    if (!row || bits < 1 || bits > MAX_WOPBS_BITS || input >= n_inputs || bit >= bits) return FHEAES_ERR_INVALID;
+    *row = CbsRows{n_inputs, bits}.row(input, bit);
     return FHEAES_OK;
 }
 int fheaes_aes_context_window(fheaes_ctx *ctx, uint64_t n_blocks, uint32_t steps, uint64_t *window_blocks)
@@ -1758,7 +1764,7 @@
     uint64_t wg0 = 0;
     for (uint64_t g0 = 0, ci = 0; g0 < n_gates; g0 += chunk, ++ci) {
         const uint64_t gc = std::min<uint64_t>(chunk, n_gates - g0);
-        TRY(cbs_bits(c, gates_lwe + g0 * c->big1, gc));
+        TRY(cbs_bits(c, gates_lwe + g0 * c->big1, CbsRows{gc, 1, false}));
         uint64_t units = 0;
         for (uint64_t g = g0; g < g0 + gc; ++g) units += bits_of_gate[g];
         TRY(launch_gate(c, (const double2 *)c->ws_ggswf.p, tab + wg0, chunk_end[ci] - wg0, units, form, in, out));
diff --git a/tfhe_aes_amd/csrc/engine_launch.h b/tfhe_aes_amd/csrc/engine_launch.h
--- a/tfhe_aes_amd/csrc/engine_launch.h
+++ b/tfhe_aes_amd/csrc/engine_launch.h
@@ -42,6 +42,19 @@
     }
     return pl;
 }
+
+struct CbsRows {
+    uint64_t n_inputs = 0;
+    uint32_t bits = 0;
+    bool packed = true;
+    bool ruled() const { return packed && bits >= 1 && bits <= 9; }
+    uint64_t tail() const { return ruled() ? n_inputs * (bits - 1) : n_inputs * bits; }
+    uint64_t row(uint64_t input, uint32_t bit) const
+    {
+        if (!ruled()) return input * bits + bit;
+        return bit ? input * (bits - 1) + bit - 1 : tail() + input;
+    }
+};
 
 #define AES_BLOCK_BITS 128ull
 #define AES_WINDOW_MAX_BLOCKS (MAX_CHUNK_BITS / AES_BLOCK_BITS)
@@ -104,16 +117,16 @@
     return FHEAES_OK;
 }
 
-int launch_pfpks(fheaes_ctx *c, const uint64_t *in, uint64_t m, uint64_t *out, uint64_t out_stride, int block = -1)
+int pfpks_rows(fheaes_ctx *c, const uint64_t *in, uint64_t m, uint64_t *out, uint64_t out_stride, int block, uint32_t group = 0, uint32_t stride = 0,
+               uint32_t first = 0)
 {
     if (m == 0) return FHEAES_OK;
-    StageScope sc(c, FHEAES_STAGE_PFPKS, m);
     const uint32_t gsz = c->k1 * FHE_N;
     const uint64_t ct_tiles16 = ((m + KS_CT_TILE - 1) / KS_CT_TILE) * (KS_CT_TILE / 16);
     TRY(ensure(c, c->ws_digits, ct_tiles16 * c->pf_ksteps * 2 * 1024));
     int8_t *af = (int8_t *)c->ws_digits.p;
     const uint64_t threads = ct_tiles16 * c->pf_ksteps * 64;
-    ks_launch_digits_k3(dim3((unsigned)((threads + 255) / 256)), c->stream, in, (uint64_t)c->big1, c->big1, m, c->pf_ksteps, af);
+    ks_launch_digits_k3(dim3((unsigned)((threads + 255) / 256)), c->stream, in, (uint64_t)c->big1, c->big1, m, c->pf_ksteps, af, group, stride, first);
     KeyswitchArgs a{};
     a.afrag = af; a.bfrag = c->pfpksk_frag; a.ksteps = c->pf_ksteps; a.coltiles = c->pf_coltiles;
     if (block >= 0) a.bfrag += (size_t)block * c->pf_ksteps * c->pf_coltiles * 8 * 1024;
@@ -125,13 +138,49 @@
     return FHEAES_OK;
 }
 
+int launch_pfpks(fheaes_ctx *c, const uint64_t *in, uint64_t m, uint64_t *out, uint64_t out_stride, int block = -1)
+{
+    if (m == 0) return FHEAES_OK;
+    StageScope sc(c, FHEAES_STAGE_PFPKS, m);
+    return pfpks_rows(c, in, m, out, out_stride, block);
+}
+
+int launch_pfpks_cbs(fheaes_ctx *c, const uint64_t *in, const CbsRows &rows, uint64_t *out)
+{
+    const uint64_t m = rows.n_inputs * rows.bits, full = rows.tail();
+    if (m == 0) return FHEAES_OK;
+    const uint64_t gsz = (uint64_t)c->k1 * FHE_N, ggsw_words = c->k1 * gsz;
+    StageScope sc(c, FHEAES_STAGE_PFPKS, m);
+    TRY(ensure(c, c->ws_digits, ((m + KS_CT_TILE - 1) / KS_CT_TILE) * (KS_CT_TILE / 16) * c->pf_ksteps * 2 * 1024));
+    if (!rows.ruled()) return pfpks_rows(c, in, m, out, ggsw_words, -1);
+    TRY(pfpks_rows(c, in, full, out, ggsw_words, -1, rows.bits - 1, rows.bits, 1));
+    return pfpks_rows(c, in, m - full, out + full * ggsw_words + c->k * gsz, ggsw_words, (int)c->k, 1, rows.bits, 0);
+}
+
+void forward_fourier_polys(fheaes_ctx *c, const uint64_t *in, uint64_t polys, double2 *out, uint32_t group = 0, uint32_t stride = 0, uint32_t first = 0)
+{
+    if (polys == 0) return;
+    uint64_t wgs = (polys + EP_GROUPS - 1) / EP_GROUPS;
+    if (wgs > 8192) wgs = 8192;
+    hipLaunchKernelGGL(forward_fourier_kernel, dim3((unsigned)wgs), dim3(EP_THREADS), 0, c->stream, in, out, polys, c->tw_d, group, stride, first);
+}
+
 int launch_forward_fourier(fheaes_ctx *c, const uint64_t *in, uint64_t polys, double2 *out, int stage)
 {
     if (polys == 0) return FHEAES_OK;
     StageScope sc(c, stage, polys);
-    uint64_t wgs = (polys + EP_GROUPS - 1) / EP_GROUPS;
-    if (wgs > 8192) wgs = 8192;
-    hipLaunchKernelGGL(forward_fourier_kernel, dim3((unsigned)wgs), dim3(EP_THREADS), 0, c->stream, in, out, polys, c->tw_d);
+    forward_fourier_polys(c, in, polys, out);
+    HIP_TRY(c, hipGetLastError());
+    return FHEAES_OK;
+}
+
+int launch_forward_fourier_cbs(fheaes_ctx *c, const uint64_t *in, const CbsRows &rows, double2 *out)
+{
+    const uint64_t m = rows.n_inputs * rows.bits, full = rows.tail(), per = (uint64_t)c->k1 * c->k1;
+    if (m == 0) return FHEAES_OK;
+    StageScope sc(c, FHEAES_STAGE_GGSW_FFT, m * per);
+    forward_fourier_polys(c, in, full * per, out);
+    forward_fourier_polys(c, in + full * per * FHE_N, (m - full) * c->k1, out + full * per * FHE_H, c->k1, (uint32_t)per, c->k * c->k1);
     HIP_TRY(c, hipGetLastError());
     return FHEAES_OK;
 }
@@ -293,7 +342,7 @@
 }
 
 int launch_vertical_packing(fheaes_ctx *c, const double2 *ggswf, uint64_t n_inputs, uint32_t bits, const uint64_t *luts,
-                            uint32_t n_luts, int per_input, uint64_t *out)
+                            uint32_t n_luts, int per_input, uint64_t *out, const CbsRows &rows = CbsRows{}, uint64_t input0 = 0)
 {
     if (n_inputs == 0) return FHEAES_OK;
     StageScope sc(c, FHEAES_STAGE_VERTICAL_PACKING, n_inputs * n_luts * bits);
@@ -329,6 +378,8 @@
     a.luts = luts; a.lut_words = W; a.glwe_in = glwe_root;
     a.lut_per_input = per_input ? 1 : 0; a.inst_per_input = inst_per_input;
     a.wg_per_input = (inst_per_input + R - 1) / R;
+    a.input0 = input0;
+    if (rows.ruled()) { a.ruled = 1; a.tail = rows.tail(); }
     hipLaunchKernelGGL(vp_kernel, dim3((unsigned)(n_inputs * a.wg_per_input)), dim3(EP_THREADS), 0, c->stream, a);
     HIP_TRY(c, hipGetLastError());
     return FHEAES_OK;
@@ -641,19 +692,18 @@
     return FHEAES_OK;
 }
 
-int cbs_from_small(fheaes_ctx *c, uint64_t m)
-{
-    const uint64_t ggsw_words = (uint64_t)c->k1 * c->k1 * FHE_N;
-    TRY(launch_cbs_pbs(c, (const uint64_t *)c->ws_small.p, m, 1, (uint64_t *)c->ws_pbs.p));
-    TRY(launch_pfpks(c, (const uint64_t *)c->ws_pbs.p, m, (uint64_t *)c->ws_ggsw.p, ggsw_words));
-    TRY(launch_forward_fourier(c, (const uint64_t *)c->ws_ggsw.p, m * c->k1 * c->k1, (double2 *)c->ws_ggswf.p, FHEAES_STAGE_GGSW_FFT));
-    return FHEAES_OK;
-}
-
-int cbs_bits(fheaes_ctx *c, const uint64_t *in, uint64_t m)
-{
-    TRY(launch_keyswitch(c, in, m, (uint64_t *)c->ws_small.p));
-    return cbs_from_small(c, m);
+int cbs_from_small(fheaes_ctx *c, const CbsRows &rows)
+{
+    TRY(launch_cbs_pbs(c, (const uint64_t *)c->ws_small.p, rows.n_inputs * rows.bits, 1, (uint64_t *)c->ws_pbs.p));
+    TRY(launch_pfpks_cbs(c, (const uint64_t *)c->ws_pbs.p, rows, (uint64_t *)c->ws_ggsw.p));
+    TRY(launch_forward_fourier_cbs(c, (const uint64_t *)c->ws_ggsw.p, rows, (double2 *)c->ws_ggswf.p));
+    return FHEAES_OK;
+}
+
+int cbs_bits(fheaes_ctx *c, const uint64_t *in, const CbsRows &rows)
+{
+    TRY(launch_keyswitch(c, in, rows.n_inputs * rows.bits, (uint64_t *)c->ws_small.p));
+    return cbs_from_small(c, rows);
 }
 
 int wopbs_dev(fheaes_ctx *c, const uint64_t *lwe_in, uint64_t n_inputs, uint32_t bits, const uint64_t *luts, uint32_t n_luts,
@@ -671,11 +721,12 @@
     TRY(ensure_wopbs_ws(c, std::min<uint64_t>(n_inputs, chunk_inputs) * bits));
     for (uint64_t i0 = 0; i0 < n_inputs; i0 += chunk_inputs) {
         const uint64_t ni = std::min<uint64_t>(chunk_inputs, n_inputs - i0);
-        TRY(cbs_bits(c, lwe_in + i0 * bits * c->big1, ni * bits));
+        const CbsRows rows{ni, bits};
+        TRY(cbs_bits(c, lwe_in + i0 * bits * c->big1, rows));
         const uint64_t *l = per_input ? luts + i0 * n_luts * bits * W : luts;
-        TRY(launch_vertical_packing(c, (const double2 *)c->ws_ggswf.p, ni, bits, l, n_luts, per_input, lwe_out + i0 * n_luts * bits * c->big1));
-    }
-    return FHEAES_OK;
-}
-
-}
+        TRY(launch_vertical_packing(c, (const double2 *)c->ws_ggswf.p, ni, bits, l, n_luts, per_input, lwe_out + i0 * n_luts * bits * c->big1, rows));
+    }
+    return FHEAES_OK;
+}
+
+}
diff --git a/tfhe_aes_amd/csrc/kern_extprod.h b/tfhe_aes_amd/csrc/kern_extprod.h
--- a/tfhe_aes_amd/csrc/kern_extprod.h
+++ b/tfhe_aes_amd/csrc/kern_extprod.h
@@ -116,6 +116,8 @@
     uint32_t ggsw_per_input;
     uint64_t lut_words;
     const uint64_t *glwe_in;
+    uint64_t input0, tail;
+    uint32_t ruled;
 };
 
 template <int K1, int BASE_LOG, int R>
@@ -157,11 +159,14 @@
     __syncthreads();
 
     const size_t ggsw_stride = (size_t)K1 * K1 * FHE_H;
-
-    for (uint32_t it = 0; it < A.iters; ++it) {
-        const int t = (1024 - (1 << it)) & 1023;
-        const double2 *G = A.ggsw + ((size_t)input * A.ggsw_per_input + it) * ggsw_stride;
-
+    const uint64_t batch_input = A.input0 + input;
+    auto ggsw_of = [&](const uint32_t it) {
+        uint64_t row = batch_input * A.ggsw_per_input + it;
+        if (A.ruled) row = it ? batch_input * (A.ggsw_per_input - 1) + it - 1 : A.tail + batch_input;
+        return A.ggsw + (size_t)row * ggsw_stride;
+    };
+
+    auto rotate_decompose = [&](const int t, double (&xr)[16], double (&xi)[16]) {
         uint64_t *stage = reinterpret_cast<uint64_t *>(tile);
 #pragma unroll
         for (int a = 0; a < 16; ++a) {
@@ -169,7 +174,6 @@
             stage[256 + 16 * a + b] = hi[a];
         }
         wave_lds_sync();
-        double xr[16], xi[16];
 #pragma unroll
         for (int a = 0; a < 16; ++a) {
             int j0 = 16 * a + b, j1 = j0 + 256;
@@ -184,6 +188,70 @@
             if ((a & (EP_ROT_CHUNK - 1)) == EP_ROT_CHUNK - 1) __builtin_amdgcn_sched_barrier(0);
         }
         wave_lds_sync();
+    };
+
+    auto accumulate_products = [&](const double (&fr)[R][K1], const double (&fi)[R][K1], double (&xr)[16], double (&xi)[16]) {
+        __syncthreads();
+#pragma unroll
+        for (int r = 0; r < R; ++r)
+#pragma unroll
+            for (int c = 0; c < K1; ++c) {
+                double2 v; v.x = fr[r][c]; v.y = fi[r][c];
+                *reinterpret_cast<double2 *>(lds + (r * K1 + c) * GROUP_TILE_DOUBLES + 2 * tid) = v;
+            }
+        __syncthreads();
+#pragma unroll
+        for (int k2 = 0; k2 < 16; ++k2) {
+            double2 v = *reinterpret_cast<const double2 *>(tile + 2 * (b + 16 * k2));
+            xr[k2] = v.x; xi[k2] = v.y;
+        }
+        wave_lds_sync();
+        nega_inv(xr, xi, tw, tile, b);
+#pragma unroll
+        for (int a = 0; a < 16; ++a) {
+            lo[a] += torus_from_double(xr[a]);
+            hi[a] += torus_from_double(xi[a]);
+        }
+    };
+
+    uint32_t it = 0;
+    if (!A.glwe_in && A.iters) {
+        const double2 *Gl = ggsw_of(0) + (size_t)(K1 - 1) * K1 * FHE_H + tid;
+        double2 bv[K1];
+#pragma unroll
+        for (int c = 0; c < K1; ++c) bv[c] = Gl[(size_t)c * FHE_H];
+        double xr[16], xi[16];
+        if (p_own == K1 - 1) {
+            rotate_decompose(1023, xr, xi);
+            nega_fwd(xr, xi, tw, tile, b);
+#pragma unroll
+            for (int k2 = 0; k2 < 16; ++k2) {
+                double2 v; v.x = xr[k2]; v.y = xi[k2];
+                *reinterpret_cast<double2 *>(tile + 2 * (b + 16 * k2)) = v;
+            }
+        }
+        __syncthreads();
+        double fr[R][K1], fi[R][K1];
+#pragma unroll
+        for (int r = 0; r < R; ++r) {
+            const double2 d = *reinterpret_cast<const double2 *>(lds + (r * K1 + K1 - 1) * GROUP_TILE_DOUBLES + 2 * tid);
+#pragma unroll
+            for (int c = 0; c < K1; ++c) {
+                fr[r][c] = __builtin_fma(d.x, bv[c].x, 0.0);
+                fr[r][c] = __builtin_fma(-d.y, bv[c].y, fr[r][c]);
+                fi[r][c] = __builtin_fma(d.x, bv[c].y, 0.0);
+                fi[r][c] = __builtin_fma(d.y, bv[c].x, fi[r][c]);
+            }
+        }
+        accumulate_products(fr, fi, xr, xi);
+        it = 1;
+    }
+
+    for (; it < A.iters; ++it) {
+        const int t = (1024 - (1 << it)) & 1023;
+        const double2 *G = ggsw_of(it);
+        double xr[16], xi[16];
+        rotate_decompose(t, xr, xi);
 
         double fr[R][K1], fi[R][K1];
 #pragma unroll
@@ -255,28 +323,7 @@
             __builtin_amdgcn_s_setprio(0);
         };
         level_body();
-
-        __syncthreads();
-#pragma unroll
-        for (int r = 0; r < R; ++r)
-#pragma unroll
-            for (int c = 0; c < K1; ++c) {
-                double2 v; v.x = fr[r][c]; v.y = fi[r][c];
-                *reinterpret_cast<double2 *>(lds + (r * K1 + c) * GROUP_TILE_DOUBLES + 2 * tid) = v;
-            }
-        __syncthreads();
-#pragma unroll
-        for (int k2 = 0; k2 < 16; ++k2) {
-            double2 v = *reinterpret_cast<const double2 *>(tile + 2 * (b + 16 * k2));
-            xr[k2] = v.x; xi[k2] = v.y;
-        }
-        wave_lds_sync();
-        nega_inv(xr, xi, tw, tile, b);
-#pragma unroll
-        for (int a = 0; a < 16; ++a) {
-            lo[a] += torus_from_double(xr[a]);
-            hi[a] += torus_from_double(xi[a]);
-        }
+        accumulate_products(fr, fi, xr, xi);
     }
 
     if (owner && valid) {
@@ -369,7 +416,8 @@
     }
 }
 
-__global__ __launch_bounds__(EP_THREADS) void forward_fourier_kernel(const uint64_t *in, double2 *out, uint64_t polys, const double2 *tw_g)
+__global__ __launch_bounds__(EP_THREADS) void forward_fourier_kernel(const uint64_t *in, double2 *out, uint64_t polys, const double2 *tw_g,
+                                                                     uint32_t group, uint32_t stride, uint32_t first)
 {
     __shared__ __attribute__((aligned(16))) double lds[EP_LDS_DOUBLES];
     double2 *tw = reinterpret_cast<double2 *>(lds + EP_GROUPS * GROUP_TILE_DOUBLES);
@@ -381,6 +429,7 @@
         uint64_t q = base + g;
         bool valid = q < polys;
         if (!valid) q = polys - 1;
+        if (group) q = (q / group) * stride + first + q % group;
         const uint64_t *p = in + q * FHE_N;
         double xr[16], xi[16];
 #pragma unroll
diff --git a/tfhe_aes_amd/csrc/kern_keyswitch.h b/tfhe_aes_amd/csrc/kern_keyswitch.h
--- a/tfhe_aes_amd/csrc/kern_keyswitch.h
+++ b/tfhe_aes_amd/csrc/kern_keyswitch.h
@@ -63,7 +63,7 @@
 
 template <int BASE_LOG, int LEVELS, int PLANES>
 __global__ __launch_bounds__(256) void digits_kernel(const uint64_t *in, uint64_t in_stride, uint32_t n_in, uint64_t m,
-                                                     uint32_t ksteps, int8_t *frag)
+                                                     uint32_t ksteps, int8_t *frag, uint32_t group, uint32_t stride, uint32_t first)
 {
     const uint64_t gid = (uint64_t)blockIdx.x * blockDim.x + threadIdx.x;
     const uint32_t lane = gid & 63;
@@ -76,6 +76,7 @@
 #pragma unroll
     for (int e = 0; e < 16; ++e) { lo[e] = 0; hi[e] = 0; }
     if (ct < m) {
+        const uint64_t row = group ? (ct / group) * stride + first + ct % group : ct;
         const uint32_t i0 = q0 / LEVELS;
         constexpr int NI = (16 + LEVELS - 1) / LEVELS + 1;
 #pragma unroll
@@ -83,7 +84,7 @@
             const uint32_t i = i0 + ii;
             if (i >= n_in) break;
             int d[LEVELS];
-            decompose_all<BASE_LOG, LEVELS>(in[ct * in_stride + i], d);
+            decompose_all<BASE_LOG, LEVELS>(in[row * in_stride + i], d);
 #pragma unroll
             for (int l = 0; l < LEVELS; ++l) {
                 const int e = (int)(i * LEVELS + l) - (int)q0;
diff --git a/tfhe_aes_amd/csrc/ks_launch.h b/tfhe_aes_amd/csrc/ks_launch.h
--- a/tfhe_aes_amd/csrc/ks_launch.h
+++ b/tfhe_aes_amd/csrc/ks_launch.h
@@ -18,21 +18,25 @@
 #endif
 
 #ifdef FHEAES_KS_LAUNCH_DECL
-void ks_launch_digits_k1(dim3 grid, hipStream_t s, const uint64_t *in, uint64_t in_stride, uint32_t n_in, uint64_t m, uint32_t ksteps, int8_t *frag);
-void ks_launch_digits_k3(dim3 grid, hipStream_t s, const uint64_t *in, uint64_t in_stride, uint32_t n_in, uint64_t m, uint32_t ksteps, int8_t *frag);
+void ks_launch_digits_k1(dim3 grid, hipStream_t s, const uint64_t *in, uint64_t in_stride, uint32_t n_in, uint64_t m, uint32_t ksteps, int8_t *frag,
+                         uint32_t group = 0, uint32_t stride = 0, uint32_t first = 0);
+void ks_launch_digits_k3(dim3 grid, hipStream_t s, const uint64_t *in, uint64_t in_stride, uint32_t n_in, uint64_t m, uint32_t ksteps, int8_t *frag,
+                         uint32_t group = 0, uint32_t stride = 0, uint32_t first = 0);
 void ks_launch_mfma_lds(int planes, dim3 grid, hipStream_t s, const KeyswitchArgs &a);
 void ks_launch_keybytes(dim3 grid, hipStream_t s, const uint64_t *key, uint64_t key_z_stride, uint32_t rows, uint32_t ncols, uint32_t ksteps,
                         uint32_t coltiles, int8_t *frag);
 #endif
 
 #ifdef FHEAES_KS_LAUNCH_DEFINE
-FHEAES_KS_LAUNCH_LINKAGE void ks_launch_digits_k1(dim3 grid, hipStream_t s, const uint64_t *in, uint64_t in_stride, uint32_t n_in, uint64_t m, uint32_t ksteps, int8_t *frag)
+FHEAES_KS_LAUNCH_LINKAGE void ks_launch_digits_k1(dim3 grid, hipStream_t s, const uint64_t *in, uint64_t in_stride, uint32_t n_in, uint64_t m, uint32_t ksteps, int8_t *frag,
+                         uint32_t group = 0, uint32_t stride = 0, uint32_t first = 0)
 {
-    hipLaunchKernelGGL((digits_kernel<2, 6, 1>), grid, dim3(256), 0, s, in, in_stride, n_in, m, ksteps, frag);
+    hipLaunchKernelGGL((digits_kernel<2, 6, 1>), grid, dim3(256), 0, s, in, in_stride, n_in, m, ksteps, frag, group, stride, first);
 }
-FHEAES_KS_LAUNCH_LINKAGE void ks_launch_digits_k3(dim3 grid, hipStream_t s, const uint64_t *in, uint64_t in_stride, uint32_t n_in, uint64_t m, uint32_t ksteps, int8_t *frag)
+FHEAES_KS_LAUNCH_LINKAGE void ks_launch_digits_k3(dim3 grid, hipStream_t s, const uint64_t *in, uint64_t in_stride, uint32_t n_in, uint64_t m, uint32_t ksteps, int8_t *frag,
+                         uint32_t group = 0, uint32_t stride = 0, uint32_t first = 0)
 {
-    hipLaunchKernelGGL((digits_kernel<12, 3, 2>), grid, dim3(256), 0, s, in, in_stride, n_in, m, ksteps, frag);
+    hipLaunchKernelGGL((digits_kernel<12, 3, 2>), grid, dim3(256), 0, s, in, in_stride, n_in, m, ksteps, frag, group, stride, first);
 }
 FHEAES_KS_LAUNCH_LINKAGE void ks_launch_mfma_lds(int planes, dim3 grid, hipStream_t s, const KeyswitchArgs &a)
 {
```

Measured after the change: 61.47 blocks/s, median of 6. About the same (+0.8%).
